# Vegeta2020/SE-SSD

Measured on NVIDIA H100. Metric: frames_per_sec, higher is better.
Workload: dtype f32

## Files before the change

### include/sessd_b200.h

```cpp
#ifndef SESSD_B200_H
#define SESSD_B200_H

#include <stddef.h>
#include <stdint.h>

#ifdef __cplusplus
extern "C" {
#endif

#define SESSD_OK 0
#define SESSD_EINVAL (-1)
#define SESSD_ECAPACITY (-2)
#define SESSD_EWORKSPACE (-3)

const char *sessd_version(void);
long long sessd_launch_count(void);

typedef struct {
    float voxel_size[3];
    float range_min[3];
    float range_max[3];
    int grid[3];
    int max_points;
    int max_voxels;
    int num_feat;
} sessd_voxel_cfg;

size_t sessd_voxelize_workspace_bytes(int max_total_points, int batch, const sessd_voxel_cfg *cfg);

int sessd_voxelize(const float *d_points, const int *d_frame_off, int batch, int max_total_points,
                   const sessd_voxel_cfg *cfg, float *d_voxels, int *d_coors, int *d_num_points, float *d_mean,
                   int *d_num_voxels, void *workspace, size_t workspace_bytes, void *stream);

int sessd_voxelize_host(const float *h_points, int num_points, const sessd_voxel_cfg *cfg, float *h_voxels,
                        int *h_coors_zyx , int *h_num_points);

typedef struct {
    int batch;
    int shape[3];
} sessd_grid;

size_t sessd_hash_bytes(int max_rows, int *capacity_out);
int sessd_hash_build(const int *d_coors , const int *d_n, int max_rows, sessd_grid grid,
                     uint64_t *d_table, int capacity, void *stream);

size_t sessd_bitmap_words(sessd_grid grid);
size_t sessd_scan_scratch_bytes(size_t n_items);

int sessd_subm_rulebook(const int *d_coors, const int *d_n, int max_rows, sessd_grid grid, const int ksize[3],
                        int index_kind , const void *d_index, int hash_capacity,
                        int *d_nbr, void *stream);

int sessd_strided_rulebook(const int *d_in_coors, const int *d_n_in, int max_in, sessd_grid in_grid,
                           int in_index_kind, const void *d_in_index, int in_hash_capacity,
                           const int ksize[3], const int stride[3], const int padding[3],
                           sessd_grid out_grid, void *d_out_bitmap , void *d_scan_scratch,
                           int *d_out_coors, int *d_n_out, int max_out, int *d_nbr, int *d_status, void *stream);

int sessd_tile_list_stride(int kvol);
int sessd_rulebook_tile_lists(const int *d_nbr, int kvol, const int *d_n_out, int max_out, void *d_tiles, void *stream);

int sessd_spconv_forward(const float *d_in_feat, int cin, const int *d_nbr, int kvol, const int *d_n_out,
                         int max_out, const float *d_weight, int cout, const float *d_scale, const float *d_shift,
                         int relu, float *d_out_feat, void *stream);

int sessd_sparse_to_dense(const float *d_feat, const int *d_coors, const int *d_n, int max_rows, int channels,
                          sessd_grid grid, float *d_out, void *stream);
int sessd_sparse_to_dense_indexed(const float *d_feat, int max_rows, const void *d_bitmap_index, int channels, sessd_grid grid,
                                  float *d_out, void *stream);

int sessd_spconv_forward_rows(const float *d_in_feat, int cin, const int *d_nbr, int kvol, const int *d_n_out, int max_out,
                              const float *d_weight, int cout, const float *d_scale, const float *d_shift, int relu,
                              float *d_out_feat, float *d_amax_out, void *stream);
int sessd_spconv_forward_rows_planes(const float *d_in_feat, int cin, const int *d_nbr, int kvol, const int *d_n_out, int max_out,
                                     const float *d_weight, int cout, const float *d_scale, const float *d_shift, int relu,
                                     const float *d_amax_in, float gain, float shift_max, float *d_out_feat, void *d_out_planes, int cpo,
                                     float *d_out_info, void *stream);
int sessd_spconv_forward_cg(const void *d_in_planes, int cp, int plane_rows, const float *d_in_info, const void *d_tiles, int kvol,
                            const int *d_n_out, int max_out, const void *d_weight_h2, int cout, const float *d_scale, const float *d_shift,
                            int relu, float gain, float shift_max, float *d_out_f32, void *d_out_planes, float *d_out_info, void *stream);
void sessd_set_sp_cg_deep(int on);
int sessd_spconv_cg_blocks_per_sm(int cp, int cout, int deep);
int sessd_absmax_rows(const float *d_feat, const int *d_n, int max_rows, int channels, float *d_amax, void *stream);

int sessd_rulebook_transpose(const int *d_nbr, int kvol, const int *d_n_out, int max_out, int max_in, int *d_nbr_t, void *stream);
int sessd_sparse_split_planes(const float *d_x, const int *d_n, int max_rows, int channels, float *d_info, void *d_planes, int cp, void *stream);
int sessd_dense_grad_gather(const float *d_grad, const int *d_coors, const int *d_n, int max_rows, int channels, sessd_grid grid,
                            float *d_out, void *stream);
int sessd_spconv_wgrad_items(int max_out, int kvol);
size_t sessd_spconv_wgrad_workspace_bytes(int max_out, int kvol, int cin, int cout);
int sessd_spconv_wgrad_rows(const float *d_in_feat, int cin, const float *d_gout, int cout, const void *d_tiles, int kvol,
                            const int *d_n_out, int max_out, float *d_gw, void *d_ws, size_t ws_bytes, void *stream);
int sessd_spconv_wgrad_cg(const void *d_in_planes, int cp, const float *d_in_info, const void *d_g_planes, int cout, const float *d_g_info,
                          const void *d_tiles, int kvol, const int *d_n_out, int max_out, float *d_gw, void *d_ws, size_t ws_bytes,
                          void *stream);

typedef struct {
    int batch, in_h, in_w, cin;
    int out_h, out_w, cout;
    int grid_h, grid_w;
    int in_stride;
    int out_stride, out_off_y, out_off_x;
    int ntaps;
    int tap_dy[16], tap_dx[16];
    int relu;
} sessd_conv_desc;

int sessd_bev_conv_p2(const void *d_in_planes, const float *d_in_info, const void *d_weight_h2, int cout_pad, const float *d_scale,
                      const float *d_shift, const float *d_residual, const float *d_resid_info, float gain, float shift_max,
                      float *d_out_f32, void *d_out_planes, float *d_out_info, const sessd_conv_desc *desc, const int *d_items,
                      void *stream);
int sessd_bev_deconv_p2(const void *d_in_planes, const float *d_in_info, const void *d_weight_h2, int cout_pad, const float *d_scale,
                        const float *d_shift, const float *d_residual, const float *d_resid_info, float gain, float shift_max,
                        float *d_out_f32, void *d_out_planes, float *d_out_info, int batch, int in_h, int in_w, int cin, int cout,
                        int relu, const int *d_items, void *stream);
long long sessd_bev_skip_plan_words(int batch, int h, int w, int *offsets);
int sessd_bev_skip_plan(const void *d_bitmap_index, sessd_grid grid, int *d_plan, void *stream);
int sessd_bev_skip_fill(const int *d_record, float *d_out_f32, void *d_out_planes, int cout, void *stream);
int sessd_bev_wgrad_items(const sessd_conv_desc *desc);
size_t sessd_bev_wgrad_workspace_bytes(const sessd_conv_desc *desc);
int sessd_bev_wgrad(const void *d_in_planes, const float *d_in_info, const void *d_g_planes, const float *d_g_info,
                    const sessd_conv_desc *desc, float *d_gw, void *d_ws, size_t ws_bytes, void *stream);
int sessd_bev_split_planes(const float *d_x, long long n, float *d_info, void *d_planes, void *stream);
int sessd_sparse_to_dense_planes(const float *d_feat, int max_rows, const void *d_bitmap_index, int channels, sessd_grid grid,
                                 const float *d_amax, float *d_info, void *d_planes, void *stream);
int sessd_ssfa_fuse_planes(const float *d_x0, const float *d_x1, const float *d_w0, const float *d_w1, float s0, float t0, float s1,
                           float t1, int num_pixels, int channels, float *d_out, const float *d_info0, const float *d_info1,
                           float *d_out_info, void *d_planes, void *stream);

int sessd_absmax(const float *d_x, long long n, float *d_amax, void *stream);


typedef struct {
    float cnt_thresh;
    float dist_edge[4];
    float sigma2[3];
    float suppressed_thresh;
    float centerness_pow;
    int centerness;
} sessd_dinms_cfg;

#define SESSD_DINMS_MAX_PRE 4096

typedef struct {
    int batch;
    int num_anchors;
    int anchors_per_loc;
    int head_stride;
    float score_thresh;
    int nms_pre_max;
    int nms_post_max;
    float nms_iou_thresh;
    int nms_ge;
    float post_range[6];
    float direction_offset;
    int use_frustum;
    int nms_mode;
    sessd_dinms_cfg dinms;
} sessd_post_cfg;

size_t sessd_postprocess_workspace_bytes(const sessd_post_cfg *cfg);

int sessd_postprocess(const float *d_head, const float *d_anchors, const float *d_frustum,
                      const sessd_post_cfg *cfg, float *d_boxes, float *d_scores, int *d_labels, int *d_count,
                      int *d_aux, int *d_sel_anchor, void *workspace, size_t workspace_bytes, void *stream);

int sessd_postprocess_packed(const float *d_head, const float *d_anchors, const float *d_frustum,
                             const sessd_post_cfg *cfg, float *d_boxes, float *d_scores, int *d_labels, int *d_count,
                             int *d_aux, int *d_sel_anchor, float *d_packed, int *d_meta, const int *d_num_voxels,
                             const int *d_status, void *workspace, size_t workspace_bytes, void *stream);

size_t sessd_rotate_nms_workspace_bytes(int max_boxes, int pre_max);
int sessd_rotate_nms(const float *d_boxes5, const float *d_scores, const int *d_n, int max_boxes, int pre_max,
                     int post_max, float iou_thresh, int ge, int *d_keep, int *d_num_keep, void *workspace,
                     size_t workspace_bytes, void *stream);

size_t sessd_rotate_weighted_nms_workspace_bytes(int max_boxes, int pre_max);
int sessd_rotate_weighted_nms(const float *d_boxes7, const float *d_boxes5, const float *d_scores, const float *d_iou_preds,
                              const int *d_labels, const int *d_dirs, const float *d_anchors, const int *d_n, int max_boxes,
                              int pre_max, const sessd_dinms_cfg *cfg, float *d_out_boxes, float *d_out_scores, int *d_out_labels,
                              int *d_out_dirs, int *d_keep, int *d_selected, int *d_count, void *workspace, size_t workspace_bytes,
                              void *stream);

int sessd_boxes_overlap_bev(const float *d_a, int n, const float *d_b, int m, float *d_out, void *stream);
int sessd_boxes_aligned_overlap_bev(const float *d_a, const float *d_b, int n, float *d_out, void *stream);
int sessd_boxes_iou_bev(const float *d_a, int n, const float *d_b, int m, float *d_out, void *stream);
int sessd_boxes_iou3d(const float *d_a, int n, const float *d_b, int m, float *d_out, void *stream);
size_t sessd_nms_workspace_bytes(int n);
int sessd_nms_sorted(const float *d_boxes, int n, float thresh, int mode, long long *d_keep, int *d_num_keep,
                     void *workspace, size_t workspace_bytes, void *stream);

size_t sessd_assign_workspace_bytes(int num_anchors, int batch, int max_gt);
int sessd_assign_targets(const float *d_anchors, int num_anchors, const float *d_gt_boxes, const int *d_num_gt, int batch,
                         int max_gt, float matched_thr, float unmatched_thr, int *d_labels, float *d_bbox_targets,
                         float *d_bbox_outside_weights, int *d_pos_anchor, int *d_pos_gt_id, int *d_num_pos,
                         void *workspace, size_t workspace_bytes, void *stream);

#define SESSD_AUGMENT_MAX_GT 256
#define SESSD_AUGMENT_MAX_TRY 128
int sessd_box_collision(const double *d_boxes, int n, const double *d_qboxes, int k, uint8_t *d_out, void *stream);
int sessd_noise_per_box(const float *d_gt_boxes, const int *d_num_gt, const uint8_t *d_valid, int batch, int max_gt,
                        const double *d_loc_noise, const double *d_rot_noise, int num_try, double context, int *d_selected,
                        void *stream);
int sessd_points_in_boxes(const float *d_points, int n, int point_stride, const float *d_boxes, int m, double context, uint8_t *d_mask,
                          void *stream);
int sessd_augment_points(const float *d_points, const int *d_frame_off, int batch, int max_frame_points, const float *d_gt_boxes,
                         const int *d_num_gt, const uint8_t *d_valid, int max_gt, const double *d_loc_noise, const double *d_rot_noise,
                         int num_try, const int *d_selected, double context, const float *d_global, const int *d_perm,
                         const uint8_t *d_labeled, float *d_points_raw, float *d_points_out, void *stream);
int sessd_augment_boxes(const float *d_gt_boxes, const int *d_num_gt, const uint8_t *d_valid, const uint8_t *d_target, int batch,
                        int max_gt, const double *d_loc_noise, const double *d_rot_noise, int num_try, const int *d_selected,
                        const float *d_global, const float *range_bev, float *d_boxes_raw, int *d_num_raw, float *d_boxes_out,
                        int *d_num_out, float *d_boxes_global, int *d_num_global, void *stream);

int sessd_gtaug_select_host(const double *h_corners, int num_boxes, int num_cand, uint8_t *h_accepted);
size_t sessd_gtaug_paste_workspace_bytes(int batch, int num_points, int num_objects);
int sessd_gtaug_paste(const float *d_points, const int *d_frame_off, int batch, int num_points, const int *d_obj_off, const int *d_obj_ids,
                      int num_objects, int max_paste_points, const float *d_db_points, const int *d_db_off, const int *d_db_count,
                      const double *d_db_boxes, int db_size, void *d_workspace, size_t workspace_bytes, float *d_points_out, int capacity,
                      int *d_frame_off_out, void *stream);

#define SESSD_SADA_MAX_IDS (6 * SESSD_AUGMENT_MAX_GT)
int sessd_sada_pyramids(const float *d_boxes, int num_boxes, float *d_pyramids, float *d_planes, void *stream);
int sessd_sada_membership(const float *d_points, int n, const int *d_n, const float *d_planes, int num_pyramids, const int *d_ids, int num_ids,
                          uint32_t *d_bits, int *d_counts, void *stream);
size_t sessd_sada_compact_workspace_bytes(int n);
int sessd_sada_compact(const float *d_points, int n, const int *d_n, const uint32_t *d_bits, int num_ids, const int *d_counts, int min_count,
                       void *d_workspace, size_t workspace_bytes, float *d_out, int capacity, int *d_num_out, void *stream);
size_t sessd_sada_fps_workspace_bytes(int n, int num_ids);
int sessd_sada_fps(const float *d_points, int n, const int *d_n, const uint32_t *d_bits, int num_ids, const int *d_counts, int min_count, int k,
                   void *d_workspace, size_t workspace_bytes, float *d_out, int capacity, int *d_num, void *stream);
int sessd_sada_swap(const float *d_points, int n, const int *d_n, const uint32_t *d_bits, int num_pairs, const int *d_counts, const float *d_pyramids,
                    int num_pyramids, const int *d_ids, int max_swap_points, float *d_out, int capacity, const int *d_num_in,
                    int *d_num_out, void *stream);
int sessd_sada_shuffle(const float *d_points, const int *d_frame_off, int batch, int max_frame_points, const int *d_perm, float *d_out,
                       void *stream);

size_t sessd_prep_frustum_compact_workspace_bytes(int num_points);
int sessd_prep_frustum_compact(const float *d_points, const int *d_frame_off, int batch, int num_points, const double *d_planes,
                               void *d_workspace, size_t workspace_bytes, float *d_points_out, int capacity, int *d_frame_off_out, void *stream);
int sessd_prep_box_count(const float *d_points, const int *d_frame_off, int batch, int num_points, const double *d_box_planes,
                         const int *d_box_off, int num_boxes, int *d_counts, void *stream);
size_t sessd_prep_box_gather_workspace_bytes(int num_boxes);
int sessd_prep_box_gather(const float *d_points, const int *d_frame_off, int batch, int num_points, const double *d_box_planes,
                          const double *d_centres, const int *d_box_off, int num_boxes, const int *d_counts, int num_rows, void *d_workspace,
                          size_t workspace_bytes, float *d_rows_out, int capacity, int *d_obj_off, void *stream);

size_t sessd_head_loss_workspace_bytes(int batch);
size_t sessd_odiou_loss_workspace_bytes(int batch);
int sessd_odiou_loss(const float *d_head, const float *d_anchors, const int *d_labels, const float *d_reg_targets, int batch,
                     int num_anchors, int anchors_per_loc, int head_stride, float w_odiou, const float *d_losses, float *d_odiou_sum,
                     float *d_grad_head, void *workspace, size_t workspace_bytes, void *stream);
int sessd_odiou_pairs_host(const float *h_gboxes, const float *h_qboxes, int n, float *h_odiou, float *h_grad_q);
size_t sessd_iou_pred_loss_workspace_bytes(int batch);
int sessd_iou_pred_loss(const float *d_head, const float *d_anchors, const int *d_labels, const float *d_reg_targets, int batch,
                        int num_anchors, int anchors_per_loc, int head_stride, float sigma, float w_iou, float *d_losses,
                        float *d_grad_head, void *workspace, size_t workspace_bytes, void *stream);
int sessd_head_loss(const float *d_head, const float *d_anchors, const int *d_labels, const float *d_reg_targets, int batch,
                    int num_anchors, int anchors_per_loc, int head_stride, float alpha, float sigma, float dir_offset,
                    float pos_cls_weight, float neg_cls_weight, float w_cls, float w_loc, float w_dir, float *d_losses,
                    float *d_grad_head, void *workspace, size_t workspace_bytes, void *stream);

int sessd_axpby(float *d_y, const float *d_x, float a, float b, long long n, void *stream);
int sessd_adamw_step(float *d_param, const float *d_grad, float *d_exp_avg, float *d_exp_avg_sq, long long n, float lr, float beta1,
                     float beta2, float eps, float weight_decay, int step, void *stream);
size_t sessd_grad_sqnorm_workspace_bytes(long long n);
int sessd_grad_sqnorm(const float *d_x, long long n, float max_norm, float *d_out, void *d_workspace, void *stream);
int sessd_adamw_clip_ema_step(float *d_param, float *d_grad, float *d_exp_avg, float *d_exp_avg_sq, long long n, float lr, float beta1,
                              float beta2, float eps, float weight_decay, int step, const float *d_clip_coef, float *d_ema, double ema_alpha,
                              void *stream);

#define SESSD_KITTI_REC 13
#define SESSD_KITTI_PERSON_SITTING 11
#define SESSD_KITTI_VAN 12
typedef struct {
    int num_frames;
    const int *gt_off;
    const double *gt;
    const int *gt_code;
    const int *gt_occluded;
    const int *dc_off;
    const double *dc;
    const int *dt_off;
    const int *dt_cnt;
    const double *dt;
    const int *dt_code;
    const long long *ov_off;
} SessdKittiFrames;
size_t sessd_kitti_convert_workspace_bytes(long long capacity);
int sessd_kitti_convert_detections(const float *d_boxes7, const float *d_scores, const int *d_labels, const int *d_off, int num_frames,
                                   long long capacity, const double *d_calib, const int *d_image_hw, const int *d_label_code,
                                   int num_labels, double *d_rec, int *d_label, int *d_code, int *d_cnt, void *workspace,
                                   size_t workspace_bytes, void *stream);
int sessd_kitti_overlaps(const SessdKittiFrames *frames, int metric, int z_axis, double z_center, double *d_overlaps, void *stream);
size_t sessd_kitti_eval_workspace_bytes(int num_frames, long long total_gt, long long overlap_elems, int num_configs, int compute_aos);
int sessd_kitti_eval(const SessdKittiFrames *frames, int max_frame_dt, int metric, int z_axis, double z_center, int num_configs,
                     const int *d_cfg, const double *d_min_overlap, int compute_aos, long long total_gt, long long overlap_elems,
                     double *d_thresholds, int *d_num_thresholds, double *d_precision, double *d_aos, double *d_map, void *workspace,
                     size_t workspace_bytes, void *stream);

#ifdef __cplusplus
}
#endif
#endif
```

### se-ssd_b200/csrc/bevconv.cu

```cuda
#include <cuda_fp16.h>

#include "common.cuh"

namespace sessd {

__global__ void __launch_bounds__(256) ssfa_fuse_kernel(const float *__restrict__ x0, const float *__restrict__ x1,
                                                        const float *__restrict__ w0, const float *__restrict__ w1, float s0, float t0,
                                                        float s1, float t1, int num_pixels, int C, float *__restrict__ out,
                                                        const float *__restrict__ info0, const float *__restrict__ info1,
                                                        float *__restrict__ out_info, __half *__restrict__ planes, long long plane_stride) {
    const int lane = threadIdx.x & 31;
    const int warps_per_block = blockDim.x >> 5;
    const float am = fmaxf(__ldg(info0), __ldg(info1));
    const float sp = pow2_scale_for_bound(am);
    if (blockIdx.x == 0 && threadIdx.x == 0) { out_info[0] = am; out_info[1] = sp; }
    for (int p = blockIdx.x * warps_per_block + (threadIdx.x >> 5); p < num_pixels; p += gridDim.x * warps_per_block) {
        float d0 = 0.f, d1 = 0.f;
        for (int c = lane * 4; c < C; c += 128) {
            const float4 a = *reinterpret_cast<const float4 *>(x0 + (size_t)p * C + c);
            const float4 b = *reinterpret_cast<const float4 *>(x1 + (size_t)p * C + c);
            const float4 u = *reinterpret_cast<const float4 *>(w0 + c);
            const float4 v = *reinterpret_cast<const float4 *>(w1 + c);
            d0 += a.x * u.x + a.y * u.y + a.z * u.z + a.w * u.w;
            d1 += b.x * v.x + b.y * v.y + b.z * v.z + b.w * v.w;
        }
#pragma unroll
        for (int o = 16; o > 0; o >>= 1) { d0 += __shfl_xor_sync(0xffffffffu, d0, o); d1 += __shfl_xor_sync(0xffffffffu, d1, o); }
        const float l0 = fmaf(d0, s0, t0), l1 = fmaf(d1, s1, t1);
        const float mx = fmaxf(l0, l1);
        const float e0 = expf(l0 - mx), e1 = expf(l1 - mx);
        const float inv = 1.0f / (e0 + e1);
        const float a0 = e0 * inv, a1 = e1 * inv;
        for (int c = lane * 4; c < C; c += 128) {
            const float4 a = *reinterpret_cast<const float4 *>(x0 + (size_t)p * C + c);
            const float4 b = *reinterpret_cast<const float4 *>(x1 + (size_t)p * C + c);
            float4 r;
            r.x = a.x * a0 + b.x * a1; r.y = a.y * a0 + b.y * a1; r.z = a.z * a0 + b.z * a1; r.w = a.w * a0 + b.w * a1;
            if (out) *reinterpret_cast<float4 *>(out + (size_t)p * C + c) = r;
            const float q[4] = {r.x * sp, r.y * sp, r.z * sp, r.w * sp};
            __align__(8) __half hi[4], lo[4];
#pragma unroll
            for (int e = 0; e < 4; ++e) {
                hi[e] = __float2half_rn(q[e]);
                lo[e] = __float2half_rn(q[e] - __half2float(hi[e]));
            }
            *reinterpret_cast<uint2 *>(planes + (size_t)p * C + c) = *reinterpret_cast<const uint2 *>(hi);
            *reinterpret_cast<uint2 *>(planes + plane_stride + (size_t)p * C + c) = *reinterpret_cast<const uint2 *>(lo);
        }
    }
}

__global__ void absmax_kernel(const float4 *__restrict__ x, long long n4, const float *__restrict__ tail, int ntail, float *__restrict__ amax) {
    float m = 0.f;
    for (long long i = blockIdx.x * (long long)blockDim.x + threadIdx.x; i < n4; i += (long long)gridDim.x * blockDim.x) {
        const float4 v = __ldg(x + i);
        m = fmaxf(m, fmaxf(fmaxf(fabsf(v.x), fabsf(v.y)), fmaxf(fabsf(v.z), fabsf(v.w))));
    }
    if (blockIdx.x == 0 && (int)threadIdx.x < ntail) m = fmaxf(m, fabsf(tail[threadIdx.x]));
    const unsigned w = __reduce_max_sync(0xFFFFFFFFu, __float_as_uint(m));
    __shared__ unsigned s_m[32];
    if ((threadIdx.x & 31) == 0) s_m[threadIdx.x >> 5] = w;
    __syncthreads();
    if (threadIdx.x < 32) {
        const unsigned v = threadIdx.x < (blockDim.x >> 5) ? s_m[threadIdx.x] : 0u;
        const unsigned r = __reduce_max_sync(0xFFFFFFFFu, v);
        if (threadIdx.x == 0 && r != 0u) atomicMax(reinterpret_cast<unsigned *>(amax), r);
    }
}

}

using namespace sessd;

extern "C" int sessd_absmax(const float *d_x, long long n, float *d_amax, void *stream) {
    if (!d_x || !d_amax || n < 0 || ((uintptr_t)d_x & 15)) return SESSD_EINVAL;
    if (n == 0) return 0;
    const long long n4 = n / 4;
    const int blocks = (int)max(1LL, min((long long)kNumSMs * 8, (n4 + 255) / 256));
    absmax_kernel<<<blocks, 256, 0, (cudaStream_t)stream>>>(reinterpret_cast<const float4 *>(d_x), n4, d_x + n4 * 4, (int)(n - n4 * 4), d_amax);
    ++g_launches;
    return last_error();
}

extern "C" int sessd_ssfa_fuse_planes(const float *d_x0, const float *d_x1, const float *d_w0, const float *d_w1, float s0, float t0, float s1,
                                      float t1, int num_pixels, int channels, float *d_out, const float *d_info0, const float *d_info1,
                                      float *d_out_info, void *d_planes, void *stream) {
    if (!d_x0 || !d_x1 || !d_w0 || !d_w1 || !d_planes || !d_info0 || !d_info1 || !d_out_info || num_pixels < 1 || channels < 4 || channels % 4)
        return SESSD_EINVAL;
    SESSD_LAUNCH(ssfa_fuse_kernel, persistent_grid((long long)num_pixels * 32, 256), 256, 0, stream, d_x0, d_x1, d_w0, d_w1, s0, t0, s1, t1,
                 num_pixels, channels, d_out, d_info0, d_info1, d_out_info, (__half *)d_planes, (long long)num_pixels * channels);
    return last_error();
}
```

### se-ssd_b200/csrc/bevconv_p2.cu

```cuda
#include "bevconv_p2.cuh"

namespace sessd {

__global__ void __launch_bounds__(256) bev_split_planes_kernel(const float4 *__restrict__ x, long long n4, float *__restrict__ info,
                                                               __half *__restrict__ planes, long long plane_stride) {
    const float s = pow2_scale_for_bound(__ldg(info));
    if (blockIdx.x == 0 && threadIdx.x == 0) info[1] = s;
    for (long long i = blockIdx.x * (long long)blockDim.x + threadIdx.x; i < n4; i += (long long)gridDim.x * blockDim.x) {
        const float4 v = __ldg(x + i);
        const float a[4] = {v.x * s, v.y * s, v.z * s, v.w * s};
        __align__(8) __half hi[4], lo[4];
#pragma unroll
        for (int t = 0; t < 4; ++t) {
            hi[t] = __float2half_rn(a[t]);
            lo[t] = __float2half_rn(a[t] - __half2float(hi[t]));
        }
        *reinterpret_cast<uint2 *>(planes + 4 * i) = *reinterpret_cast<const uint2 *>(hi);
        *reinterpret_cast<uint2 *>(planes + plane_stride + 4 * i) = *reinterpret_cast<const uint2 *>(lo);
    }
}

}

using namespace sessd;

extern "C" int sessd_bev_conv_p2(const void *d_in_planes, const float *d_in_info, const void *d_weight_h2, int cout_pad, const float *d_scale,
                                 const float *d_shift, const float *d_residual, const float *d_resid_info, float gain, float shift_max,
                                 float *d_out_f32, void *d_out_planes, float *d_out_info, const sessd_conv_desc *desc, const int *d_items,
                                 void *stream) {
    return p2_conv<kP2Planes>(d_in_planes, d_in_info, d_weight_h2, cout_pad, d_scale, d_shift, d_residual, d_resid_info, gain, shift_max,
                              d_out_f32, d_out_planes, d_out_info, desc, stream, d_items);
}

extern "C" int sessd_bev_deconv_p2(const void *d_in_planes, const float *d_in_info, const void *d_weight_h2, int cout_pad, const float *d_scale,
                                   const float *d_shift, const float *d_residual, const float *d_resid_info, float gain, float shift_max,
                                   float *d_out_f32, void *d_out_planes, float *d_out_info, int batch, int in_h, int in_w, int cin, int cout,
                                   int relu, const int *d_items, void *stream) {
    return p2_deconv<kP2Planes>(d_in_planes, d_in_info, d_weight_h2, cout_pad, d_scale, d_shift, d_residual, d_resid_info, gain, shift_max,
                                d_out_f32, d_out_planes, d_out_info, batch, in_h, in_w, cin, cout, relu, stream, d_items);
}

extern "C" int sessd_bev_split_planes(const float *d_x, long long n, float *d_info, void *d_planes, void *stream) {
    if (!d_x || !d_info || !d_planes || n < 4 || (n & 3) || ((uintptr_t)d_x & 15)) return SESSD_EINVAL;
    SESSD_LAUNCH(bev_split_planes_kernel, persistent_grid(n / 4, 256), 256, 0, stream, reinterpret_cast<const float4 *>(d_x), n / 4, d_info,
                 (__half *)d_planes, n);
    return last_error();
}
```

### se-ssd_b200/csrc/bevconv_p2.cuh

```cuda
#pragma once
#include <cuda_fp16.h>

#include "tc_common.cuh"

namespace sessd {

constexpr int kP2TileU = 8, kP2TileV = 16;
constexpr int kP2MaxCopies = 6, kP2MaxRowsV = 18;
constexpr int kP2BStages = 6, kP2MaxBStages = 12;
constexpr int kP2MmaWarps = 8;
constexpr int kP2PatchWarp = 8, kP2WeightWarp = 9;
constexpr int kP2Threads = 320;
constexpr int kP2ThreadsRegA = 384, kP2RegsConsumer = 232, kP2RegsProducer = 40;
static_assert(2 * (kP2RegsConsumer - 168) <= 168 - kP2RegsProducer, "the consumers take what the producers release");
constexpr int kP2MaxSmem = 227 * 1024;
constexpr int kP2Chunk = 32;
constexpr int kP2ItemsHeader = 32;
enum { kP2Planes = 0, kP2SplitF16 = 1 };
enum { kP2NoProbe = 0, kP2ProbeClocks = 1, kP2ProbeLoads = 2 };

struct P2Params {
    int batch, cin, cout;
    int in_stride;
    int out_h, out_w;
    int grid_u, grid_v;
    int u_is_x;
    int out_stride, nclass;
    int cls_ntaps[4], cls_off_u[4], cls_off_v[4];
    int tap_copy[4][9], tap_row[4][9], tap_w[4][9];
    int ncopies, rows_v, pitch_u;
    int copy_u[kP2MaxCopies], copy_v[kP2MaxCopies];
    int copy_bytes, patch_bytes, npatch;
    int load_bytes, staging_bytes;
    int bring_bytes;
    int out_info_scale;
    const float *in_amax;
    int relu, n_tile, nblocks;
    int bstages, bstage_bytes;
    int tiles_u, tiles_v, tiles, total;
    int cls_order[4];
    const float *in_info;
    const float *resid_info;
    float gain, shift_max;
    float *out_info;
    long long out_plane_stride;
    const int *items;
    long long *prof;
};

enum P2Prof {
    kProfCta,
    kProfItems,
    kProfSteps,
    kProfItemClk,
    kProfBFull,
    kProfPatchFull,
    kProfMmaWait,
    kProfEpilogue,
    kProfPatchEmpty,
    kProfPatchTotal,
    kProfBEmpty,
    kProfBTotal,
    kP2ProfWords = 16
};

__device__ __forceinline__ int p2_item_count(const P2Params &p) { return p.items ? __ldg(p.items) : p.total; }
__device__ __forceinline__ int p2_item(const P2Params &p, int k) { return p.items ? __ldg(p.items + kP2ItemsHeader + k) : k; }

struct P2ItemIndex { int rank, nb, t; };
__host__ __device__ __forceinline__ P2ItemIndex p2_item_index(int g, int nblocks, int tiles) {
    const int rank = g / (nblocks * tiles), rem = g - rank * (nblocks * tiles), nb = rem / tiles;
    return {rank, nb, rem - nb * tiles};
}

struct P2Item { int cls, n0, b, u0, v0, ntaps; };

__device__ __forceinline__ P2Item p2_decode(const P2Params &p, int g) {
    P2Item it;
    const P2ItemIndex ix = p2_item_index(g, p.nblocks, p.tiles);
    int t = ix.t;
    it.cls = p.cls_order[ix.rank];
    it.n0 = ix.nb * p.n_tile;
    const int tu = t % p.tiles_u; t /= p.tiles_u;
    const int tv = t % p.tiles_v;
    it.b = t / p.tiles_v;
    it.u0 = tu * kP2TileU; it.v0 = tv * kP2TileV;
    it.ntaps = p.cls_ntaps[it.cls];
    return it;
}

template <int N>
__device__ __forceinline__ void p2_wgmma(float *d, uint64_t da, uint64_t db, uint32_t accumulate) {
    if constexpr (N == 32) wgmma_f16_n32(d, da, db, accumulate);
    else if constexpr (N == 64) wgmma_f16_n64(d, da, db, accumulate);
    else if constexpr (N == 128) wgmma_f16_n128(d, da, db, accumulate);
    else wgmma_f16_n256(d, da, db, accumulate);
}

template <int N>
__device__ __forceinline__ void p2_wgmma_ra(float *d, const uint32_t *a, uint64_t db, uint32_t accumulate) {
    if constexpr (N == 32) wgmma_f16_ra_n32(d, a, db, accumulate);
    else if constexpr (N == 64) wgmma_f16_ra_n64(d, a, db, accumulate);
    else if constexpr (N == 128) wgmma_f16_ra_n128(d, a, db, accumulate);
    else wgmma_f16_ra_n256(d, a, db, accumulate);
}

template <bool PROFILE>
__device__ __forceinline__ long long p2_tick() {
    if constexpr (PROFILE) return clock64();
    return 0;
}
template <bool PROFILE>
__device__ __forceinline__ void p2_tock(long long &clk, long long t0) {
    if constexpr (PROFILE) clk += clock64() - t0;
}

__device__ __forceinline__ void p2_split_patch(const P2Params &p, const unsigned char *staging, unsigned char *planes, float s_in, int ctid) {
    const int rows = p.rows_v * kP2TileU;
    const int copy_in = p.staging_bytes / p.ncopies;
    const int items = p.ncopies * rows * 4;
    for (int i = ctid; i < items; i += kP2MmaWarps * 32) {
        const int j = i & 3, r = (i >> 2) % rows, c = (i >> 2) / rows;
        unsigned char *hi = planes + 2 * c * p.copy_bytes + r * 64 + ((j ^ ((r >> 1) & 3)) << 4);
        const float4 *src = reinterpret_cast<const float4 *>(staging + c * copy_in + r * 128 + j * 32);
        const float4 a = src[0], b = src[1];
        const float x[8] = {a.x * s_in, a.y * s_in, a.z * s_in, a.w * s_in, b.x * s_in, b.y * s_in, b.z * s_in, b.w * s_in};
        __align__(16) __half h[8], l[8];
#pragma unroll
        for (int t = 0; t < 8; ++t) { h[t] = __float2half_rn(x[t]); l[t] = __float2half_rn(x[t] - __half2float(h[t])); }
        *reinterpret_cast<uint4 *>(hi) = *reinterpret_cast<const uint4 *>(h);
        *reinterpret_cast<uint4 *>(hi + p.copy_bytes) = *reinterpret_cast<const uint4 *>(l);
    }
    asm volatile("fence.proxy.async.shared::cta;\n" ::: "memory");
    asm volatile("bar.sync 1, %0;\n" ::"n"(kP2MmaWarps * 32) : "memory");
}

template <int NT, int MODE, bool REGA = false, int PROBE = kP2NoProbe>
__global__ void __launch_bounds__(REGA ? kP2ThreadsRegA : kP2Threads, 1) bev_conv_p2_kernel(const __grid_constant__ CUtensorMap map_a,
                                                                   const __grid_constant__ CUtensorMap map_b,
                                                                   const float *__restrict__ scale, const float *__restrict__ shift,
                                                                   const float *__restrict__ resid, float *__restrict__ out_f32,
                                                                   __half *__restrict__ out_planes, P2Params p) {
    static_assert(!REGA || MODE == kP2Planes, "register-fed A reads the TMA-written planes");
    constexpr bool PROFILE = PROBE != kP2NoProbe, LOADS_ONLY = PROBE == kP2ProbeLoads;
    extern __shared__ unsigned char smem_raw[];
    unsigned char *tiles = (unsigned char *)(((uintptr_t)smem_raw + 1023) & ~(uintptr_t)1023);
    unsigned char *patches = tiles + p.bring_bytes;
    unsigned char *staging = patches + p.npatch * p.patch_bytes;
    uint64_t *bars = (uint64_t *)(staging + p.npatch * p.staging_bytes);
    uint64_t *patch_full = bars, *patch_empty = bars + 2, *b_full = bars + 4, *b_empty = bars + 4 + kP2MaxBStages;
    uint32_t *s_aoff = (uint32_t *)(b_empty + kP2MaxBStages);
    float *s_scale = (float *)(((uintptr_t)(s_aoff + 4 * 9) + 15) & ~(uintptr_t)15), *s_shift = s_scale + p.cout;

    const int warp = threadIdx.x >> 5, lane = threadIdx.x & 31;
    if (threadIdx.x == kP2PatchWarp * 32) prefetch_tensormap(&map_a);
    if (threadIdx.x == kP2WeightWarp * 32) prefetch_tensormap(&map_b);
    const int nchunks = p.cin / kP2Chunk;
    const int nitems = p2_item_count(p);
    const uint32_t b_plane_bytes = (uint32_t)p.n_tile * 64u;

    if (threadIdx.x == 0) {
        for (int s = 0; s < 2; ++s) { mbar_init(&patch_full[s], 1); mbar_init(&patch_empty[s], kP2MmaWarps); }
        for (int s = 0; s < p.bstages; ++s) { mbar_init(&b_full[s], 1); mbar_init(&b_empty[s], kP2MmaWarps); }
        asm volatile("fence.mbarrier_init.release.cluster;\n" ::: "memory");
    }
    for (int idx = threadIdx.x; idx < p.nclass * 9; idx += blockDim.x) {
        const int c = idx / 9, t = idx - c * 9;
        s_aoff[idx] = REGA ? (uint32_t)p.tap_row[c][t] : (uint32_t)((2 * p.tap_copy[c][t] * p.copy_bytes + p.tap_row[c][t] * 512) >> 4);
    }
    for (int n = threadIdx.x; n < p.cout; n += blockDim.x) {
        s_scale[n] = scale ? __ldg(scale + n) : 1.f;
        s_shift[n] = shift ? __ldg(shift + n) : 0.f;
    }
    __syncthreads();
    long long clk[kP2ProfWords] = {};
    const long long t_start = p2_tick<PROFILE>();
    long long *prof_rec = PROFILE ? p.prof + (size_t)blockIdx.x * kP2ProfWords : nullptr;

    if (warp >= kP2MmaWarps) {
        if constexpr (REGA) setmaxnreg_dec<kP2RegsProducer>();
        if (warp == kP2PatchWarp) {
            int pb = 0;
            uint32_t pph = 0;
            const uint32_t patches_u32 = smem_u32(patches);
            for (int k = blockIdx.x; k < nitems; k += gridDim.x) {
                const P2Item it = p2_decode(p, p2_item(p, k));
                const int bu = it.u0 * p.in_stride, bv = it.v0 * p.in_stride;
                for (int cc = 0; cc < nchunks; ++cc) {
                    { const long long t0 = p2_tick<PROFILE>(); mbar_wait<REGA>(&patch_empty[pb], pph ^ 1u); p2_tock<PROFILE>(clk[kProfPatchEmpty], t0); }
                    if (elect_one()) {
                        mbar_expect_tx(&patch_full[pb], (uint32_t)p.load_bytes);
                        if constexpr (MODE == kP2Planes) {
                            uint32_t dst = patches_u32 + (uint32_t)(pb * p.patch_bytes);
                            for (int c = 0; c < p.ncopies; ++c, dst += 2u * (uint32_t)p.copy_bytes) {
                                const int cu = bu + p.copy_u[c], cv = bv + p.copy_v[c];
                                tma_load_5d(dst, &map_a, &patch_full[pb], cc * kP2Chunk, cu, cv, it.b, 0);
                                tma_load_5d(dst + (uint32_t)p.copy_bytes, &map_a, &patch_full[pb], cc * kP2Chunk, cu, cv, it.b, 1);
                            }
                        } else {
                            const uint32_t copy_in = (uint32_t)(p.staging_bytes / p.ncopies);
                            uint32_t dst = smem_u32(staging) + (uint32_t)(pb * p.staging_bytes);
                            for (int c = 0; c < p.ncopies; ++c, dst += copy_in)
                                tma_load_5d(dst, &map_a, &patch_full[pb], cc * kP2Chunk, bu + p.copy_u[c], bv + p.copy_v[c], it.b, 0);
                        }
                    }
                    __syncwarp();
                    if (++pb == p.npatch) { pb = 0; pph ^= 1u; }
                }
            }
            if constexpr (PROFILE)
                if (lane == 0) {
                    prof_rec[kProfPatchEmpty] = clk[kProfPatchEmpty];
                    prof_rec[kProfPatchTotal] = clock64() - t_start;
                }
        } else if (warp == kP2WeightWarp) {
            int S = 0;
            uint32_t bph = 0;
            for (int k = blockIdx.x; k < nitems; k += gridDim.x) {
                const P2Item it = p2_decode(p, p2_item(p, k));
                for (int cc = 0; cc < nchunks; ++cc)
                    for (int tap = 0; tap < it.ntaps; ++tap) {
                        { const long long t0 = p2_tick<PROFILE>(); mbar_wait<REGA>(&b_empty[S], bph ^ 1u); p2_tock<PROFILE>(clk[kProfBEmpty], t0); }
                        if (elect_one()) {
                            unsigned char *st = tiles + S * p.bstage_bytes;
                            const int wtap = p.tap_w[it.cls][tap];
                            mbar_expect_tx(&b_full[S], 2 * b_plane_bytes);
                            tma_load_4d(st + b_plane_bytes, &map_b, &b_full[S], cc * kP2Chunk, it.n0, wtap, 0);
                            tma_load_4d(st, &map_b, &b_full[S], cc * kP2Chunk, it.n0, wtap, 1);
                        }
                        __syncwarp();
                        if (++S == p.bstages) { S = 0; bph ^= 1u; }
                    }
            }
            if constexpr (PROFILE)
                if (lane == 0) {
                    prof_rec[kProfBEmpty] = clk[kProfBEmpty];
                    prof_rec[kProfBTotal] = clock64() - t_start;
                }
        }
    } else {
        if constexpr (REGA) setmaxnreg_inc<kP2RegsConsumer>();
        const int wg = warp >> 2, wq = warp & 3;
        constexpr int kAcc = NT / 2;
        const uint32_t a_rows = (uint32_t)(wg * 64 * 64) >> 4;
        const uint32_t tiles_lo = desc_lo(smem_u32(tiles));
        const uint32_t patch_lo = desc_lo(smem_u32(patches)) + a_rows;
        const uint32_t plane_lo = b_plane_bytes >> 4;
        const uint32_t copy_lo = (uint32_t)(p.copy_bytes >> 4), patch_sz = (uint32_t)(p.patch_bytes >> 4);
        const uint32_t a_row = (uint32_t)((wg * 8 + wq * 2 + ((lane >> 3) & 1)) * p.pitch_u + (lane & 7)), a_chunk = (uint32_t)(lane >> 4);
        const uint32_t patches_u32 = smem_u32(patches);
        float amax_in = 0.f, s_in = 1.f;
        if constexpr (MODE == kP2Planes) { amax_in = __ldg(p.in_info); s_in = __ldg(p.in_info + 1); }
        if constexpr (MODE == kP2SplitF16) if (p.in_amax) { amax_in = __ldg(p.in_amax); s_in = pow2_scale_for_bound(amax_in); }
        const float inv_sa = 1.f / s_in;
        float bound = amax_in * p.gain + p.shift_max;
        if (p.resid_info) bound += __ldg(p.resid_info);
        const float s_out = pow2_scale_for_bound(bound);
        if (blockIdx.x == 0 && threadIdx.x == 0 && p.out_info && p.out_info_scale) p.out_info[1] = s_out;
        float vmax = 0.f;
        const int per_cls = p.nblocks * p.tiles;
        int S = 0, pb = 0;
        uint32_t bph = 0, pph = 0;
        for (int k = blockIdx.x; k < nitems; k += gridDim.x) {
            const long long t_item = p2_tick<PROFILE>();
            const int g = p2_item(p, k);
            const int cls = p.cls_order[g / per_cls];
            const int ntaps = p.cls_ntaps[cls];
            const uint32_t *aoff = s_aoff + cls * 9;
            float acc[NT];
#pragma unroll
            for (int i = 0; i < NT; ++i) acc[i] = 0.f;
            int prevS = -1, prev_pb = -1;
            bool first = true;
            if constexpr (REGA) {
                uint32_t frag[2][16];
                int tap = 0;
                uint32_t pbase = 0;
                auto load_frags = [&](uint32_t *fa) {
                    if (tap == 0) {
                        { const long long t0 = p2_tick<PROFILE>(); mbar_wait<REGA>(&patch_full[pb], pph); p2_tock<PROFILE>(clk[kProfPatchFull], t0); }
                        pbase = patches_u32 + (uint32_t)(pb * p.patch_bytes);
                    }
                    if constexpr (!LOADS_ONLY) {
                        const uint32_t r = a_row + aoff[tap];
                        const uint32_t a_hi = pbase + r * 64u + ((a_chunk ^ ((r >> 1) & 3u)) << 4), a_lo = a_hi + (uint32_t)p.copy_bytes;
                        ldsm_x4(fa, a_hi);
                        ldsm_x4(fa + 4, a_hi ^ 32u);
                        ldsm_x4(fa + 8, a_lo);
                        ldsm_x4(fa + 12, a_lo ^ 32u);
                    }
                };
                auto step_ra = [&](const uint32_t *fa, uint32_t *fn, bool more) {
                    { const long long t0 = p2_tick<PROFILE>(); mbar_wait<REGA>(&b_full[S], bph); p2_tock<PROFILE>(clk[kProfBFull], t0); }
                    const uint64_t db_lo = kDescSw64Hi | (uint64_t)(tiles_lo + (uint32_t)(S * (p.bstage_bytes >> 4)));
                    const uint64_t db_hi = db_lo + (uint64_t)plane_lo;
                    if constexpr (!LOADS_ONLY) {
                        wgmma_fence();
                        p2_wgmma_ra<2 * NT>(acc, fa, db_lo, first ? 0u : 1u);
                        p2_wgmma_ra<2 * NT>(acc, fa + 4, db_lo + 2, 1u);
                        wgmma_commit();
                    }
                    first = false;
                    if constexpr (PROFILE) ++clk[kProfSteps];
                    { const long long t0 = p2_tick<PROFILE>(); wgmma_wait<1>(); p2_tock<PROFILE>(clk[kProfMmaWait], t0); }
                    if (lane == 0 && prevS >= 0) mbar_arrive(&b_empty[prevS]);
                    prevS = S;
                    if (++S == p.bstages) { S = 0; bph ^= 1u; }
                    if (++tap == ntaps) {
                        tap = 0;
                        if (lane == 0) mbar_arrive(&patch_empty[pb]);
                        if (++pb == p.npatch) { pb = 0; pph ^= 1u; }
                    }
                    if (more) load_frags(fn);
                    if constexpr (!LOADS_ONLY) {
                        wgmma_fence();
                        p2_wgmma_ra<NT>(acc, fa + 8, db_hi, 1u);
                        p2_wgmma_ra<NT>(acc, fa + 12, db_hi + 2, 1u);
                        wgmma_commit();
                    }
                };
                const int nsteps = nchunks * ntaps;
                load_frags(frag[0]);
#pragma unroll 1
                for (int st = 0; st + 1 < nsteps; st += 2) { step_ra(frag[0], frag[1], true); step_ra(frag[1], frag[0], st + 2 < nsteps); }
                if (nsteps & 1) step_ra(frag[0], frag[1], false);
            } else {
                for (int cc = 0; cc < nchunks; ++cc) {
                    { const long long t0 = p2_tick<PROFILE>(); mbar_wait(&patch_full[pb], pph); p2_tock<PROFILE>(clk[kProfPatchFull], t0); }
                    if constexpr (MODE == kP2SplitF16)
                        p2_split_patch(p, staging + pb * p.staging_bytes, patches + pb * p.patch_bytes, s_in, threadIdx.x);
                    const uint32_t pbase = patch_lo + (uint32_t)pb * patch_sz;
#pragma unroll 1
                    for (int tap = 0; tap < ntaps; ++tap) {
                        { const long long t0 = p2_tick<PROFILE>(); mbar_wait(&b_full[S], bph); p2_tock<PROFILE>(clk[kProfBFull], t0); }
                        if constexpr (!LOADS_ONLY) {
                            const uint64_t da_hi = kDescSw64Hi | (uint64_t)(pbase + aoff[tap]);
                            const uint64_t da_lo = da_hi + (uint64_t)copy_lo;
                            const uint64_t db_lo = kDescSw64Hi | (uint64_t)(tiles_lo + (uint32_t)(S * (p.bstage_bytes >> 4)));
                            const uint64_t db_hi = db_lo + (uint64_t)plane_lo;
                            const uint32_t accum = first ? 0u : 1u;
                            wgmma_fence();
                            if constexpr (MODE == kP2Planes) {
                                p2_wgmma<2 * NT>(acc, da_hi, db_lo, accum);
                                p2_wgmma<2 * NT>(acc, da_hi + 2, db_lo + 2, 1u);
                            } else {
                                p2_wgmma<NT>(acc + kAcc, da_hi, db_hi, accum);
                                p2_wgmma<NT>(acc + kAcc, da_hi + 2, db_hi + 2, 1u);
                                p2_wgmma<NT>(acc, da_hi, db_lo, accum);
                                p2_wgmma<NT>(acc, da_hi + 2, db_lo + 2, 1u);
                            }
                            p2_wgmma<NT>(acc, da_lo, db_hi, 1u);
                            p2_wgmma<NT>(acc, da_lo + 2, db_hi + 2, 1u);
                            wgmma_commit();
                        }
                        first = false;
                        if constexpr (PROFILE) ++clk[kProfSteps];
                        { const long long t0 = p2_tick<PROFILE>(); wgmma_wait<1>(); p2_tock<PROFILE>(clk[kProfMmaWait], t0); }
                        if (lane == 0) {
                            if (prevS >= 0) mbar_arrive(&b_empty[prevS]);
                            if (prev_pb >= 0) mbar_arrive(&patch_empty[prev_pb]);
                        }
                        prevS = S;
                        prev_pb = (tap == ntaps - 1) ? pb : -1;
                        if (++S == p.bstages) { S = 0; bph ^= 1u; }
                    }
                    if (p.npatch == 1) {
                        { const long long t0 = p2_tick<PROFILE>(); wgmma_wait<0>(); p2_tock<PROFILE>(clk[kProfMmaWait], t0); }
                        if (lane == 0) {
                            mbar_arrive(&b_empty[prevS]);
                            mbar_arrive(&patch_empty[pb]);
                        }
                        prevS = prev_pb = -1;
                    }
                    if (++pb == p.npatch) { pb = 0; pph ^= 1u; }
                }
            }
            { const long long t0 = p2_tick<PROFILE>(); wgmma_wait<0>(); p2_tock<PROFILE>(clk[kProfMmaWait], t0); }
            const long long t_epi = p2_tick<PROFILE>();
            wgmma_fence_regs<NT>(acc);
            if (lane == 0) {
                if (prevS >= 0) mbar_arrive(&b_empty[prevS]);
                if (prev_pb >= 0) mbar_arrive(&patch_empty[prev_pb]);
            }
#pragma unroll
            for (int i = 0; i < kAcc; ++i) acc[i] = acc[kAcc + i] + acc[i];
            const P2Item it = p2_decode(p, g);
            const int q = lane & 3;
            const int r0 = wg * 64 + wq * 16 + (lane >> 2);
            bool rows_ok[2];
            size_t opixs[2];
#pragma unroll
            for (int h = 0; h < 2; ++h) {
                const int r = r0 + 8 * h;
                const int lv = r / kP2TileU, lu = r % kP2TileU;
                const int gu = it.u0 + lu, gv = it.v0 + lv;
                rows_ok[h] = it.b < p.batch && gu < p.grid_u && gv < p.grid_v;
                const int ou = gu * p.out_stride + p.cls_off_u[it.cls], ov = gv * p.out_stride + p.cls_off_v[it.cls];
                const int oy = p.u_is_x ? ov : ou, ox = p.u_is_x ? ou : ov;
                opixs[h] = ((size_t)it.b * p.out_h + (size_t)oy) * p.out_w + (size_t)ox;
            }
#pragma unroll
            for (int j = 0; j < (LOADS_ONLY ? 0 : NT / 32); ++j)
#pragma unroll
                for (int h = 0; h < 2; ++h) {
                    const bool row_ok = rows_ok[h];
                    const size_t opix = opixs[h];
                    float v[8], o[8] = {};
                    quad_transpose8(acc + 16 * j + 2 * h, q, v);
                    const int n = it.n0 + 32 * j + 8 * q;
                    const size_t off = opix * p.cout + n;
                    if (row_ok && n < p.cout) {
                        float sc[8], sh[8];
#pragma unroll
                        for (int t = 0; t < 8; t += 4) {
                            const float4 a = *reinterpret_cast<const float4 *>(s_scale + n + t);
                            const float4 b = *reinterpret_cast<const float4 *>(s_shift + n + t);
                            sc[t] = a.x; sc[t + 1] = a.y; sc[t + 2] = a.z; sc[t + 3] = a.w;
                            sh[t] = b.x; sh[t + 1] = b.y; sh[t + 2] = b.z; sh[t + 3] = b.w;
                        }
#pragma unroll
                        for (int t = 0; t < 8; ++t) {
                            o[t] = fmaf(v[t] * inv_sa, sc[t], sh[t]);
                            if (p.relu) o[t] = fmaxf(o[t], 0.f);
                        }
                        if (resid) {
#pragma unroll
                            for (int t = 0; t < 8; t += 4) {
                                const float4 rr = __ldg(reinterpret_cast<const float4 *>(resid + off + t));
                                o[t] += rr.x; o[t + 1] += rr.y; o[t + 2] += rr.z; o[t + 3] += rr.w;
                            }
                        }
#pragma unroll
                        for (int t = 0; t < 8; ++t) vmax = fmaxf(vmax, fabsf(o[t]));
                        if (out_planes) {
                            __align__(16) __half2 hi[4], lo[4];
#pragma unroll
                            for (int t = 0; t < 4; ++t) {
                                const float x0 = o[2 * t] * s_out, x1 = o[2 * t + 1] * s_out;
                                hi[t] = __floats2half2_rn(x0, x1);
                                const float2 f = __half22float2(hi[t]);
                                lo[t] = __floats2half2_rn(x0 - f.x, x1 - f.y);
                            }
                            *reinterpret_cast<uint4 *>(out_planes + off) = *reinterpret_cast<const uint4 *>(hi);
                            *reinterpret_cast<uint4 *>(out_planes + p.out_plane_stride + off) = *reinterpret_cast<const uint4 *>(lo);
                        }
                    }
                    if (out_f32) {
                        const bool up = q & 2;
                        float keep[4], recv[4];
#pragma unroll
                        for (int t = 0; t < 4; ++t) {
                            keep[t] = up ? o[4 + t] : o[t];
                            recv[t] = __shfl_xor_sync(0xFFFFFFFFu, up ? o[t] : o[4 + t], 2);
                        }
                        const int n_lo = it.n0 + 32 * j + 8 * (q & 1), c_lo = n_lo + 4 * (q >> 1);
                        const float4 w_lo = up ? make_float4(recv[0], recv[1], recv[2], recv[3]) : make_float4(keep[0], keep[1], keep[2], keep[3]);
                        const float4 w_hi = up ? make_float4(keep[0], keep[1], keep[2], keep[3]) : make_float4(recv[0], recv[1], recv[2], recv[3]);
                        if (row_ok && n_lo < p.cout) *reinterpret_cast<float4 *>(out_f32 + opix * p.cout + c_lo) = w_lo;
                        if (row_ok && n_lo + 16 < p.cout) *reinterpret_cast<float4 *>(out_f32 + opix * p.cout + c_lo + 16) = w_hi;
                    }
                }
            if constexpr (PROFILE) {
                const long long t_end = clock64();
                clk[kProfEpilogue] += t_end - t_epi;
                clk[kProfItemClk] += t_end - t_item;
                ++clk[kProfItems];
            }
        }
        if constexpr (PROFILE)
            if (threadIdx.x == 0) {
                clk[kProfCta] = clock64() - t_start;
                for (int w = kProfCta; w <= kProfEpilogue; ++w) prof_rec[w] = clk[w];
            }
        if (p.out_info) {
            const unsigned m = __reduce_max_sync(0xFFFFFFFFu, __float_as_uint(vmax));
            if (lane == 0 && m != 0u) atomicMax(reinterpret_cast<unsigned *>(p.out_info), m);
        }
    }
}

static int encode_map_nd(CUtensorMap *m, const void *base, int rank, const cuuint64_t *dims, const cuuint64_t *strides_bytes ,
                         const cuuint32_t *box, const cuuint32_t *estr, CUtensorMapSwizzle swz,
                         CUtensorMapDataType dtype = CU_TENSOR_MAP_DATA_TYPE_FLOAT16) {
    EncodeTiledFn enc = get_tensor_map_encoder();
    if (!enc) return SESSD_EINVAL;
    CUresult r = enc(m, dtype, (cuuint32_t)rank, const_cast<void *>(base), dims, strides_bytes, box, estr,
                     CU_TENSOR_MAP_INTERLEAVE_NONE, swz, CU_TENSOR_MAP_L2_PROMOTION_L2_256B, CU_TENSOR_MAP_FLOAT_OOB_FILL_NONE);
    return r == CUDA_SUCCESS ? 0 : 700 + (int)r;
}

struct P2Taps { int n, dy[9], dx[9], w[9], off_y, off_x; };

static void p2_deconv_classes(P2Taps cls[4]) {
    for (int c = 0; c < 4; ++c) {
        P2Taps &k = cls[c];
        k = {};
        k.off_y = c >> 1; k.off_x = c & 1;
        for (int dy = k.off_y; dy >= 0; --dy)
            for (int dx = k.off_x; dx >= 0; --dx, ++k.n) {
                k.dy[k.n] = dy; k.dx[k.n] = dx; k.w[k.n] = (k.off_y + 1 - 2 * dy) * 3 + (k.off_x + 1 - 2 * dx);
            }
    }
}

constexpr int p2_n_tile(int cout) { return cout <= 32 ? 32 : 128; }

struct P2Geometry {
    int u_is_x, grid_u, grid_v, tiles_u, tiles_v, tiles;
    int n_tile, nblocks, nclass, total;
    int ntaps[4], off_u[4], off_v[4], order[4];
};

static int p2_geometry(P2Geometry &g, int batch, int grid_h, int grid_w, int cout, int cout_pad, const P2Taps *cls, int nclass) {
    g = {};
    if (batch < 1 || grid_h < 1 || grid_w < 1 || cout < 8 || cout % 8) return SESSD_EINVAL;
    g.n_tile = p2_n_tile(cout);
    if (cout_pad % g.n_tile || cout_pad < cout) return SESSD_EINVAL;
    g.u_is_x = div_up(grid_w, kP2TileU) * div_up(grid_h, kP2TileV) <= div_up(grid_h, kP2TileU) * div_up(grid_w, kP2TileV);
    g.grid_u = g.u_is_x ? grid_w : grid_h; g.grid_v = g.u_is_x ? grid_h : grid_w;
    g.tiles_u = div_up(g.grid_u, kP2TileU); g.tiles_v = div_up(g.grid_v, kP2TileV);
    g.tiles = g.tiles_u * g.tiles_v * batch;
    g.nblocks = cout_pad / g.n_tile;
    g.nclass = nclass; g.total = nclass * g.nblocks * g.tiles;
    for (int c = 0; c < nclass; ++c) {
        g.ntaps[c] = cls[c].n;
        g.off_u[c] = g.u_is_x ? cls[c].off_x : cls[c].off_y;
        g.off_v[c] = g.u_is_x ? cls[c].off_y : cls[c].off_x;
        g.order[c] = c;
    }
    for (int i = 1; i < nclass; ++i)
        for (int k = i; k > 0 && g.ntaps[g.order[k]] > g.ntaps[g.order[k - 1]]; --k) {
            const int tmp = g.order[k]; g.order[k] = g.order[k - 1]; g.order[k - 1] = tmp;
        }
    return 0;
}

static int p2_plan(P2Params &p, const P2Taps *cls, int nclass, int grid_h, int grid_w, int cout_pad, int mode, bool reg_a, int *smem) {
    if (reg_a && (mode != kP2Planes || p.in_stride != 1)) return SESSD_EINVAL;
    if (p.cin < 64 || p.cin % 64) return SESSD_EINVAL;
    P2Geometry g;
    if (p2_geometry(g, p.batch, grid_h, grid_w, p.cout, cout_pad, cls, nclass)) return SESSD_EINVAL;
    p.u_is_x = g.u_is_x; p.grid_u = g.grid_u; p.grid_v = g.grid_v;
    p.tiles_u = g.tiles_u; p.tiles_v = g.tiles_v; p.tiles = g.tiles;
    p.n_tile = g.n_tile; p.nblocks = g.nblocks; p.nclass = g.nclass; p.total = g.total;
    for (int c = 0; c < 4; ++c) {
        p.cls_ntaps[c] = g.ntaps[c]; p.cls_off_u[c] = g.off_u[c]; p.cls_off_v[c] = g.off_v[c]; p.cls_order[c] = g.order[c];
    }
    const int s = p.in_stride;
    p.ncopies = 0;
    int key_u[kP2MaxCopies], key_vm[kP2MaxCopies], vmin[kP2MaxCopies], vmax[kP2MaxCopies];
    for (int c = 0; c < p.nclass; ++c)
        for (int t = 0; t < cls[c].n; ++t) {
            const int tu = p.u_is_x ? cls[c].dx[t] : cls[c].dy[t], tv = p.u_is_x ? cls[c].dy[t] : cls[c].dx[t];
            const int vm = ((tv % s) + s) % s;
            int k = 0;
            for (; k < p.ncopies; ++k)
                if (key_u[k] == tu && key_vm[k] == vm) break;
            if (k == p.ncopies) {
                if (p.ncopies == kP2MaxCopies) return SESSD_EINVAL;
                key_u[k] = tu; key_vm[k] = vm; vmin[k] = tv; vmax[k] = tv;
                ++p.ncopies;
            }
            vmin[k] = min(vmin[k], tv); vmax[k] = max(vmax[k], tv);
        }
    p.rows_v = 0;
    p.pitch_u = kP2TileU;
    for (int k = 0; k < p.ncopies; ++k) p.rows_v = max(p.rows_v, kP2TileV + (vmax[k] - vmin[k]) / s);
    if (p.rows_v > kP2MaxRowsV) return SESSD_EINVAL;
    for (int k = 0; k < p.ncopies; ++k) { p.copy_u[k] = key_u[k]; p.copy_v[k] = vmin[k]; }
    if (reg_a) {
        int umin = key_u[0], umax = key_u[0];
        for (int k = 1; k < p.ncopies; ++k) {
            umin = min(umin, key_u[k]); umax = max(umax, key_u[k]);
            vmin[0] = min(vmin[0], vmin[k]); vmax[0] = max(vmax[0], vmax[k]);
        }
        p.ncopies = 1;
        p.copy_u[0] = umin; p.copy_v[0] = vmin[0];
        p.pitch_u = kP2TileU + umax - umin; p.rows_v = kP2TileV + vmax[0] - vmin[0];
        if (p.pitch_u > 256 || p.rows_v > 256) return SESSD_EINVAL;
    }
    for (int c = 0; c < p.nclass; ++c) {
        for (int t = 0; t < cls[c].n; ++t) {
            const int tu = p.u_is_x ? cls[c].dx[t] : cls[c].dy[t], tv = p.u_is_x ? cls[c].dy[t] : cls[c].dx[t];
            const int vm = ((tv % s) + s) % s;
            int k = 0;
            for (; k < p.ncopies; ++k)
                if (key_u[k] == tu && key_vm[k] == vm) break;
            p.tap_copy[c][t] = reg_a ? 0 : k;
            p.tap_row[c][t] = reg_a ? (tv - p.copy_v[0]) * p.pitch_u + (tu - p.copy_u[0]) : (tv - vmin[k]) / s;
            p.tap_w[c][t] = cls[c].w[t];
        }
    }
    p.copy_bytes = (p.rows_v * p.pitch_u * 64 + 511) & ~511;
    p.patch_bytes = p.ncopies * 2 * p.copy_bytes;
    p.staging_bytes = mode == kP2Planes ? 0 : p.ncopies * p.rows_v * kP2TileU * kP2Chunk * 4;
    p.load_bytes = mode == kP2Planes ? p.ncopies * 2 * p.rows_v * p.pitch_u * 64 : p.staging_bytes;
    const int per_buf = p.patch_bytes + p.staging_bytes, bstage = 2 * p.n_tile * 64;
    const int tail = 1536 + 16 + 2 * 4 * p.cout;
    p.npatch = (kP2BStages * bstage + tail + 2 * per_buf <= kP2MaxSmem) ? 2 : 1;
    p.bstage_bytes = bstage;
    p.bstages = min((kP2MaxSmem - tail - p.npatch * per_buf) / bstage, kP2MaxBStages);
    if (p.bstages < 2) return SESSD_EINVAL;
    p.bring_bytes = p.bstages * bstage;
    *smem = p.bring_bytes + tail + p.npatch * per_buf;
    return 0;
}

template <int MODE, int PROBE = kP2NoProbe>
static int launch_p2(const void *d_in_planes, int in_h, int in_w, const float *d_in_info, const void *d_w, int w_taps, int cout_pad,
                     const float *d_scale, const float *d_shift, const float *d_residual, const float *d_resid_info, float gain,
                     float shift_max, float *d_out_f32, void *d_out_planes, float *d_out_info, P2Params &p, const P2Taps *cls, int nclass,
                     int grid_h, int grid_w, bool reg_a, void *stream) {
    if (!d_in_planes || !d_w || (!d_out_f32 && !d_out_planes)) return SESSD_EINVAL;
    if (MODE == kP2Planes && (!d_in_info || !d_scale)) return SESSD_EINVAL;
    if (MODE != kP2Planes && d_out_planes) return SESSD_EINVAL;
    if (((uintptr_t)d_scale | (uintptr_t)d_shift | (uintptr_t)d_residual | (uintptr_t)d_out_f32 | (uintptr_t)d_out_planes) & 15)
        return SESSD_EINVAL;
    int smem = 0;
    if (p2_plan(p, cls, nclass, grid_h, grid_w, cout_pad, MODE, reg_a, &smem)) return SESSD_EINVAL;
    if (p.items && cout_pad != div_up(p.cout, p.n_tile) * p.n_tile) return SESSD_EINVAL;
    const int s = p.in_stride;
    CUtensorMap map_a, map_b;
    if (MODE != kP2Planes) {
        const cuuint64_t row_w = (cuuint64_t)p.cin * 4, row_h = (cuuint64_t)in_w * p.cin * 4;
        const cuuint64_t dims[5] = {(cuuint64_t)p.cin, (cuuint64_t)(p.u_is_x ? in_w : in_h), (cuuint64_t)(p.u_is_x ? in_h : in_w),
                                    (cuuint64_t)p.batch, 1};
        const cuuint64_t strides[4] = {p.u_is_x ? row_w : row_h, p.u_is_x ? row_h : row_w, (cuuint64_t)in_h * in_w * p.cin * 4,
                                       (cuuint64_t)p.batch * in_h * in_w * p.cin * 4};
        const cuuint32_t box[5] = {(cuuint32_t)kP2Chunk, (cuuint32_t)(kP2TileU * s), (cuuint32_t)(p.rows_v * s), 1, 1};
        const cuuint32_t estr[5] = {1, (cuuint32_t)s, (cuuint32_t)s, 1, 1};
        int rc = encode_map_nd(&map_a, d_in_planes, 5, dims, strides, box, estr, CU_TENSOR_MAP_SWIZZLE_NONE, CU_TENSOR_MAP_DATA_TYPE_FLOAT32);
        if (rc) return rc;
    } else {
        const cuuint64_t row_w = (cuuint64_t)p.cin * 2, row_h = (cuuint64_t)in_w * p.cin * 2;
        const cuuint64_t dims[5] = {(cuuint64_t)p.cin, (cuuint64_t)(p.u_is_x ? in_w : in_h), (cuuint64_t)(p.u_is_x ? in_h : in_w),
                                    (cuuint64_t)p.batch, 2};
        const cuuint64_t strides[4] = {p.u_is_x ? row_w : row_h, p.u_is_x ? row_h : row_w, (cuuint64_t)in_h * in_w * p.cin * 2,
                                       (cuuint64_t)p.batch * in_h * in_w * p.cin * 2};
        const cuuint32_t box[5] = {(cuuint32_t)kP2Chunk, (cuuint32_t)(p.pitch_u * s), (cuuint32_t)(p.rows_v * s), 1, 1};
        const cuuint32_t estr[5] = {1, (cuuint32_t)s, (cuuint32_t)s, 1, 1};
        int rc = encode_map_nd(&map_a, d_in_planes, 5, dims, strides, box, estr, CU_TENSOR_MAP_SWIZZLE_64B);
        if (rc) return rc;
    }
    {
        const cuuint64_t dims[4] = {(cuuint64_t)p.cin, (cuuint64_t)cout_pad, (cuuint64_t)w_taps, 2};
        const cuuint64_t strides[3] = {(cuuint64_t)p.cin * 2, (cuuint64_t)cout_pad * p.cin * 2, (cuuint64_t)w_taps * cout_pad * p.cin * 2};
        const cuuint32_t box[4] = {(cuuint32_t)kP2Chunk, (cuuint32_t)p.n_tile, 1, 1};
        const cuuint32_t estr[4] = {1, 1, 1, 1};
        int rc = encode_map_nd(&map_b, d_w, 4, dims, strides, box, estr, CU_TENSOR_MAP_SWIZZLE_64B);
        if (rc) return rc;
    }
    constexpr bool kRegA = MODE == kP2Planes;
    auto kernel = bev_conv_p2_kernel<128, MODE, false, PROBE>;
    if (p.n_tile == 32) kernel = reg_a ? bev_conv_p2_kernel<32, MODE, kRegA, PROBE> : bev_conv_p2_kernel<32, MODE, false, PROBE>;
    else if (reg_a) kernel = bev_conv_p2_kernel<128, MODE, kRegA, PROBE>;
    static bool attr_done[2][2] = {};
    if (!attr_done[p.n_tile == 32][reg_a]) {
        SESSD_CUDA_TRY(cudaFuncSetAttribute(kernel, cudaFuncAttributeMaxDynamicSharedMemorySize, kP2MaxSmem));
        attr_done[p.n_tile == 32][reg_a] = true;
    }
    p.in_info = MODE == kP2Planes ? d_in_info : nullptr;
    p.in_amax = MODE == kP2SplitF16 ? d_in_info : nullptr;
    p.resid_info = d_residual ? d_resid_info : nullptr;
    if (d_residual && d_out_planes && !d_resid_info) return SESSD_EINVAL;
    p.gain = gain; p.shift_max = shift_max; p.out_info = d_out_info;
    p.out_info_scale = MODE == kP2Planes ? 1 : 0;
    if (d_out_planes && !d_out_info) return SESSD_EINVAL;
    p.out_plane_stride = (long long)p.batch * p.out_h * p.out_w * p.cout;
    static int num_sms = 0;
    if (!num_sms) {
        int dev = 0;
        SESSD_CUDA_TRY(cudaGetDevice(&dev));
        SESSD_CUDA_TRY(cudaDeviceGetAttribute(&num_sms, cudaDevAttrMultiProcessorCount, dev));
    }
    const int grid = p.total < num_sms ? p.total : num_sms;
    SESSD_LAUNCH(kernel, grid, reg_a ? kP2ThreadsRegA : kP2Threads, smem, (cudaStream_t)stream, map_a, map_b, d_scale, d_shift, d_residual, d_out_f32,
                 (__half *)d_out_planes, p);
    return last_error();
}


static int p2_conv_params(const sessd_conv_desc &d, P2Params &p, P2Taps &t) {
    if (d.ntaps < 1 || d.ntaps > 9 || (d.in_stride != 1 && d.in_stride != 2) || d.out_stride < 1) return SESSD_EINVAL;
    if ((d.grid_h - 1) * d.out_stride + d.out_off_y >= d.out_h || (d.grid_w - 1) * d.out_stride + d.out_off_x >= d.out_w) return SESSD_EINVAL;
    p = {};
    p.batch = d.batch; p.cin = d.cin; p.cout = d.cout; p.in_stride = d.in_stride;
    p.out_h = d.out_h; p.out_w = d.out_w; p.out_stride = d.out_stride; p.relu = d.relu;
    t = {};
    t.n = d.ntaps; t.off_y = d.out_off_y; t.off_x = d.out_off_x;
    for (int i = 0; i < d.ntaps; ++i) { t.dy[i] = d.tap_dy[i]; t.dx[i] = d.tap_dx[i]; t.w[i] = i; }
    return 0;
}

static void p2_deconv_params(int batch, int in_h, int in_w, int cin, int cout, int relu, P2Params &p, P2Taps cls[4]) {
    p = {};
    p.batch = batch; p.cin = cin; p.cout = cout; p.in_stride = 1;
    p.out_h = 2 * in_h; p.out_w = 2 * in_w; p.out_stride = 2; p.relu = relu;
    p2_deconv_classes(cls);
}

template <int MODE, int PROBE = kP2NoProbe>
static int p2_conv(const void *d_in_planes, const float *d_in_info, const void *d_weight_h2, int cout_pad, const float *d_scale,
                   const float *d_shift, const float *d_residual, const float *d_resid_info, float gain, float shift_max,
                   float *d_out_f32, void *d_out_planes, float *d_out_info, const sessd_conv_desc *desc, void *stream,
                   const int *d_items = nullptr, long long *d_prof = nullptr, bool smem_a = false) {
    if (!desc || (PROBE != kP2NoProbe && !d_prof)) return SESSD_EINVAL;
    const sessd_conv_desc &d = *desc;
    P2Params p;
    P2Taps t;
    if (p2_conv_params(d, p, t)) return SESSD_EINVAL;
    p.items = d_items;
    p.prof = d_prof;
    return launch_p2<MODE, PROBE>(d_in_planes, d.in_h, d.in_w, d_in_info, d_weight_h2, d.ntaps, cout_pad, d_scale, d_shift, d_residual, d_resid_info, gain,
                     shift_max, d_out_f32, d_out_planes, d_out_info, p, &t, 1, d.grid_h, d.grid_w, MODE == kP2Planes && d.in_stride == 1 && !smem_a,
                     stream);
}

template <int MODE, int PROBE = kP2NoProbe>
static int p2_deconv(const void *d_in_planes, const float *d_in_info, const void *d_weight_h2, int cout_pad, const float *d_scale,
                     const float *d_shift, const float *d_residual, const float *d_resid_info, float gain, float shift_max,
                     float *d_out_f32, void *d_out_planes, float *d_out_info, int batch, int in_h, int in_w, int cin, int cout,
                     int relu, void *stream, const int *d_items = nullptr, long long *d_prof = nullptr) {
    if (PROBE != kP2NoProbe && !d_prof) return SESSD_EINVAL;
    P2Params p;
    P2Taps cls[4];
    p2_deconv_params(batch, in_h, in_w, cin, cout, relu, p, cls);
    p.items = d_items;
    p.prof = d_prof;
    return launch_p2<MODE, PROBE>(d_in_planes, in_h, in_w, d_in_info, d_weight_h2, 9, cout_pad, d_scale, d_shift, d_residual, d_resid_info, gain, shift_max,
                     d_out_f32, d_out_planes, d_out_info, p, cls, 4, in_h, in_w, MODE == kP2Planes, stream);
}

}
```

### se-ssd_b200/csrc/bevconv_split.cu

```cuda
#include "bevconv_p2.cuh"

#include "../../include/sessd_b200_lab.h"

using namespace sessd;

extern "C" int sessd_bev_conv_h2(const float *d_in, const void *d_weight_h2, int cout_pad, const float *d_scale, const float *d_shift,
                                 const float *d_residual, float *d_out, const sessd_conv_desc *desc, const float *d_amax_in,
                                 float *d_amax_out, void *stream) {
    if (!d_in || !d_out || !d_scale) return SESSD_EINVAL;
    return p2_conv<kP2SplitF16>(d_in, d_amax_in, d_weight_h2, cout_pad, d_scale, d_shift, d_residual, nullptr, 0.f, 0.f, d_out, nullptr,
                                d_amax_out, desc, stream);
}

extern "C" int sessd_bev_deconv_h2(const float *d_in, const void *d_weight_h2, int cout_pad, const float *d_scale, const float *d_shift,
                                   const float *d_residual, float *d_out, int batch, int in_h, int in_w, int cin, int cout, int relu,
                                   const float *d_amax_in, float *d_amax_out, void *stream) {
    if (!d_in || !d_out || !d_scale) return SESSD_EINVAL;
    return p2_deconv<kP2SplitF16>(d_in, d_amax_in, d_weight_h2, cout_pad, d_scale, d_shift, d_residual, nullptr, 0.f, 0.f, d_out, nullptr,
                                  d_amax_out, batch, in_h, in_w, cin, cout, relu, stream);
}

extern "C" int sessd_bev_conv_p2_profile(const void *d_in_planes, const float *d_in_info, const void *d_weight_h2, int cout_pad,
                                         const float *d_scale, const float *d_shift, const float *d_residual, const float *d_resid_info,
                                         float gain, float shift_max, float *d_out_f32, void *d_out_planes, float *d_out_info,
                                         const sessd_conv_desc *desc, const int *d_items, long long *d_prof, void *stream) {
    return p2_conv<kP2Planes, kP2ProbeClocks>(d_in_planes, d_in_info, d_weight_h2, cout_pad, d_scale, d_shift, d_residual, d_resid_info, gain,
                                              shift_max, d_out_f32, d_out_planes, d_out_info, desc, stream, d_items, d_prof);
}

extern "C" int sessd_bev_deconv_p2_profile(const void *d_in_planes, const float *d_in_info, const void *d_weight_h2, int cout_pad,
                                           const float *d_scale, const float *d_shift, const float *d_residual, const float *d_resid_info,
                                           float gain, float shift_max, float *d_out_f32, void *d_out_planes, float *d_out_info, int batch,
                                           int in_h, int in_w, int cin, int cout, int relu, const int *d_items, long long *d_prof,
                                           void *stream) {
    return p2_deconv<kP2Planes, kP2ProbeClocks>(d_in_planes, d_in_info, d_weight_h2, cout_pad, d_scale, d_shift, d_residual, d_resid_info, gain,
                                                shift_max, d_out_f32, d_out_planes, d_out_info, batch, in_h, in_w, cin, cout, relu, stream,
                                                d_items, d_prof);
}

extern "C" int sessd_bev_conv_p2_loads(const void *d_in_planes, const float *d_in_info, const void *d_weight_h2, int cout_pad,
                                       const float *d_scale, const float *d_shift, const float *d_residual, const float *d_resid_info,
                                       float gain, float shift_max, float *d_out_f32, void *d_out_planes, float *d_out_info,
                                       const sessd_conv_desc *desc, const int *d_items, int smem_a, long long *d_prof, void *stream) {
    return p2_conv<kP2Planes, kP2ProbeLoads>(d_in_planes, d_in_info, d_weight_h2, cout_pad, d_scale, d_shift, d_residual, d_resid_info, gain,
                                             shift_max, d_out_f32, d_out_planes, d_out_info, desc, stream, d_items, d_prof, smem_a != 0);
}

extern "C" int sessd_bev_p2_plan(const sessd_conv_desc *desc, int deconv, int cout_pad, int split, int smem_a, int *plan) {
    if (!desc || !plan) return SESSD_EINVAL;
    const sessd_conv_desc &d = *desc;
    P2Params p;
    P2Taps cls[4];
    if (deconv) p2_deconv_params(d.batch, d.in_h, d.in_w, d.cin, d.cout, d.relu, p, cls);
    else if (p2_conv_params(d, p, cls[0])) return SESSD_EINVAL;
    const int mode = split ? kP2SplitF16 : kP2Planes;
    const bool reg_a = mode == kP2Planes && (deconv || (d.in_stride == 1 && !smem_a));
    int smem = 0;
    if (p2_plan(p, cls, deconv ? 4 : 1, deconv ? d.in_h : d.grid_h, deconv ? d.in_w : d.grid_w, cout_pad, mode, reg_a, &smem))
        return SESSD_EINVAL;
    const int rec[11] = {p.u_is_x, p.n_tile, p.nblocks, p.tiles, p.total, p.ncopies, p.rows_v, p.pitch_u, p.npatch, p.bstages, smem};
    for (int i = 0; i < 11; ++i) plan[i] = rec[i];
    for (int c = 0; c < 4; ++c) { plan[11 + c] = p.cls_ntaps[c]; plan[15 + c] = p.cls_order[c]; }
    return 0;
}
```

### se-ssd_b200/sessd_b200/_lib.py

```python
import ctypes as C
import os

_HERE = os.path.dirname(os.path.abspath(__file__))
LIB_PATH = os.path.join(os.path.dirname(_HERE), "libsessd_b200.so")
LAB_PATH = os.path.join(os.path.dirname(_HERE), "libsessd_b200_lab.so")


class SessdError(RuntimeError):
    pass


class VoxelCfg(C.Structure):
    _fields_ = [("voxel_size", C.c_float * 3), ("range_min", C.c_float * 3), ("range_max", C.c_float * 3),
                ("grid", C.c_int * 3), ("max_points", C.c_int), ("max_voxels", C.c_int), ("num_feat", C.c_int)]


class Grid(C.Structure):
    _fields_ = [("batch", C.c_int), ("shape", C.c_int * 3)]


class ConvDesc(C.Structure):
    _fields_ = [("batch", C.c_int), ("in_h", C.c_int), ("in_w", C.c_int), ("cin", C.c_int),
                ("out_h", C.c_int), ("out_w", C.c_int), ("cout", C.c_int),
                ("grid_h", C.c_int), ("grid_w", C.c_int), ("in_stride", C.c_int),
                ("out_stride", C.c_int), ("out_off_y", C.c_int), ("out_off_x", C.c_int),
                ("ntaps", C.c_int), ("tap_dy", C.c_int * 16), ("tap_dx", C.c_int * 16), ("relu", C.c_int)]


class DinmsCfg(C.Structure):
    _fields_ = [("cnt_thresh", C.c_float), ("dist_edge", C.c_float * 4), ("sigma2", C.c_float * 3), ("suppressed_thresh", C.c_float),
                ("centerness_pow", C.c_float), ("centerness", C.c_int)]


class PostCfg(C.Structure):
    _fields_ = [("batch", C.c_int), ("num_anchors", C.c_int), ("anchors_per_loc", C.c_int), ("head_stride", C.c_int),
                ("score_thresh", C.c_float), ("nms_pre_max", C.c_int), ("nms_post_max", C.c_int),
                ("nms_iou_thresh", C.c_float), ("nms_ge", C.c_int), ("post_range", C.c_float * 6),
                ("direction_offset", C.c_float), ("use_frustum", C.c_int), ("nms_mode", C.c_int), ("dinms", DinmsCfg)]


class KittiFrames(C.Structure):
    _fields_ = [("num_frames", C.c_int), ("gt_off", C.c_void_p), ("gt", C.c_void_p), ("gt_code", C.c_void_p),
                ("gt_occluded", C.c_void_p), ("dc_off", C.c_void_p), ("dc", C.c_void_p), ("dt_off", C.c_void_p),
                ("dt_cnt", C.c_void_p), ("dt", C.c_void_p), ("dt_code", C.c_void_p), ("ov_off", C.c_void_p)]


_vp, _i, _f, _sz, _ll = C.c_void_p, C.c_int, C.c_float, C.c_size_t, C.c_longlong
_I3 = C.POINTER(C.c_int)

SIGNATURES = {
    "sessd_version": (C.c_char_p, []),
    "sessd_launch_count": (_ll, []),
    "sessd_voxelize_workspace_bytes": (_sz, [_i, _i, C.POINTER(VoxelCfg)]),
    "sessd_voxelize": (_i, [_vp, _vp, _i, _i, C.POINTER(VoxelCfg), _vp, _vp, _vp, _vp, _vp, _vp, _sz, _vp]),
    "sessd_voxelize_host": (_i, [_vp, _i, C.POINTER(VoxelCfg), _vp, _vp, _vp]),
    "sessd_hash_bytes": (_sz, [_i, _I3]),
    "sessd_hash_build": (_i, [_vp, _vp, _i, Grid, _vp, _i, _vp]),
    "sessd_bitmap_words": (_sz, [Grid]),
    "sessd_scan_scratch_bytes": (_sz, [_sz]),
    "sessd_subm_rulebook": (_i, [_vp, _vp, _i, Grid, _I3, _i, _vp, _i, _vp, _vp]),
    "sessd_strided_rulebook": (_i, [_vp, _vp, _i, Grid, _i, _vp, _i, _I3, _I3, _I3, Grid, _vp, _vp, _vp, _vp, _i, _vp, _vp, _vp]),
    "sessd_tile_list_stride": (_i, [_i]),
    "sessd_rulebook_tile_lists": (_i, [_vp, _i, _vp, _i, _vp, _vp]),
    "sessd_spconv_forward": (_i, [_vp, _i, _vp, _i, _vp, _i, _vp, _i, _vp, _vp, _i, _vp, _vp]),
    "sessd_spconv_forward_rows": (_i, [_vp, _i, _vp, _i, _vp, _i, _vp, _i, _vp, _vp, _i, _vp, _vp, _vp]),
    "sessd_spconv_forward_rows_planes": (_i, [_vp, _i, _vp, _i, _vp, _i, _vp, _i, _vp, _vp, _i, _vp, _f, _f, _vp, _vp, _i, _vp, _vp]),
    "sessd_spconv_forward_cg": (_i, [_vp, _i, _i, _vp, _vp, _i, _vp, _i, _vp, _i, _vp, _vp, _i, _f, _f, _vp, _vp, _vp, _vp]),
    "sessd_set_sp_cg_deep": (None, [_i]),
    "sessd_spconv_cg_blocks_per_sm": (_i, [_i, _i, _i]),
    "sessd_absmax_rows": (_i, [_vp, _vp, _i, _i, _vp, _vp]),
    "sessd_rulebook_transpose": (_i, [_vp, _i, _vp, _i, _i, _vp, _vp]),
    "sessd_sparse_split_planes": (_i, [_vp, _vp, _i, _i, _vp, _vp, _i, _vp]),
    "sessd_dense_grad_gather": (_i, [_vp, _vp, _vp, _i, _i, Grid, _vp, _vp]),
    "sessd_spconv_wgrad_items": (_i, [_i, _i]),
    "sessd_spconv_wgrad_workspace_bytes": (_sz, [_i, _i, _i, _i]),
    "sessd_spconv_wgrad_rows": (_i, [_vp, _i, _vp, _i, _vp, _i, _vp, _i, _vp, _vp, _sz, _vp]),
    "sessd_spconv_wgrad_cg": (_i, [_vp, _i, _vp, _vp, _i, _vp, _vp, _i, _vp, _i, _vp, _vp, _sz, _vp]),
    "sessd_sparse_to_dense_indexed": (_i, [_vp, _i, _vp, _i, Grid, _vp, _vp]),
    "sessd_sparse_to_dense": (_i, [_vp, _vp, _vp, _i, _i, Grid, _vp, _vp]),
    "sessd_bev_conv_p2": (_i, [_vp, _vp, _vp, _i, _vp, _vp, _vp, _vp, _f, _f, _vp, _vp, _vp, C.POINTER(ConvDesc), _vp, _vp]),
    "sessd_bev_deconv_p2": (_i, [_vp, _vp, _vp, _i, _vp, _vp, _vp, _vp, _f, _f, _vp, _vp, _vp, _i, _i, _i, _i, _i, _i, _vp, _vp]),
    "sessd_bev_skip_plan_words": (_ll, [_i, _i, _i, _I3]),
    "sessd_bev_skip_plan": (_i, [_vp, Grid, _vp, _vp]),
    "sessd_bev_skip_fill": (_i, [_vp, _vp, _vp, _i, _vp]),
    "sessd_bev_wgrad_items": (_i, [C.POINTER(ConvDesc)]),
    "sessd_bev_wgrad_workspace_bytes": (_sz, [C.POINTER(ConvDesc)]),
    "sessd_bev_wgrad": (_i, [_vp, _vp, _vp, _vp, C.POINTER(ConvDesc), _vp, _vp, _sz, _vp]),
    "sessd_bev_split_planes": (_i, [_vp, _ll, _vp, _vp, _vp]),
    "sessd_sparse_to_dense_planes": (_i, [_vp, _i, _vp, _i, Grid, _vp, _vp, _vp, _vp]),
    "sessd_ssfa_fuse_planes": (_i, [_vp, _vp, _vp, _vp, _f, _f, _f, _f, _i, _i, _vp, _vp, _vp, _vp, _vp, _vp]),
    "sessd_absmax": (_i, [_vp, C.c_longlong, _vp, _vp]),
    "sessd_postprocess_workspace_bytes": (_sz, [C.POINTER(PostCfg)]),
    "sessd_postprocess": (_i, [_vp, _vp, _vp, C.POINTER(PostCfg), _vp, _vp, _vp, _vp, _vp, _vp, _vp, _sz, _vp]),
    "sessd_postprocess_packed": (_i, [_vp, _vp, _vp, C.POINTER(PostCfg), _vp, _vp, _vp, _vp, _vp, _vp, _vp, _vp, _vp, _vp, _vp, _sz, _vp]),
    "sessd_rotate_nms_workspace_bytes": (_sz, [_i, _i]),
    "sessd_rotate_nms": (_i, [_vp, _vp, _vp, _i, _i, _i, _f, _i, _vp, _vp, _vp, _sz, _vp]),
    "sessd_rotate_weighted_nms_workspace_bytes": (_sz, [_i, _i]),
    "sessd_rotate_weighted_nms": (_i, [_vp, _vp, _vp, _vp, _vp, _vp, _vp, _vp, _i, _i, C.POINTER(DinmsCfg), _vp, _vp, _vp, _vp, _vp, _vp, _vp,
                                       _vp, _sz, _vp]),
    "sessd_boxes_overlap_bev": (_i, [_vp, _i, _vp, _i, _vp, _vp]),
    "sessd_boxes_aligned_overlap_bev": (_i, [_vp, _vp, _i, _vp, _vp]),
    "sessd_boxes_iou_bev": (_i, [_vp, _i, _vp, _i, _vp, _vp]),
    "sessd_boxes_iou3d": (_i, [_vp, _i, _vp, _i, _vp, _vp]),
    "sessd_nms_workspace_bytes": (_sz, [_i]),
    "sessd_nms_sorted": (_i, [_vp, _i, _f, _i, _vp, _vp, _vp, _sz, _vp]),
    "sessd_head_loss_workspace_bytes": (_sz, [_i]),
    "sessd_head_loss": (_i, [_vp, _vp, _vp, _vp, _i, _i, _i, _i, _f, _f, _f, _f, _f, _f, _f, _f, _vp, _vp, _vp, _sz, _vp]),
    "sessd_odiou_loss_workspace_bytes": (_sz, [_i]),
    "sessd_odiou_loss": (_i, [_vp, _vp, _vp, _vp, _i, _i, _i, _i, _f, _vp, _vp, _vp, _vp, _sz, _vp]),
    "sessd_odiou_pairs_host": (_i, [_vp, _vp, _i, _vp, _vp]),
    "sessd_iou_pred_loss_workspace_bytes": (_sz, [_i]),
    "sessd_iou_pred_loss": (_i, [_vp, _vp, _vp, _vp, _i, _i, _i, _i, _f, _f, _vp, _vp, _vp, _sz, _vp]),
    "sessd_axpby": (_i, [_vp, _vp, _f, _f, _ll, _vp]),
    "sessd_adamw_step": (_i, [_vp, _vp, _vp, _vp, _ll, _f, _f, _f, _f, _f, _i, _vp]),
    "sessd_grad_sqnorm_workspace_bytes": (_sz, [_ll]),
    "sessd_grad_sqnorm": (_i, [_vp, _ll, _f, _vp, _vp, _vp]),
    "sessd_adamw_clip_ema_step": (_i, [_vp, _vp, _vp, _vp, _ll, _f, _f, _f, _f, _f, _i, _vp, _vp, C.c_double, _vp]),
    "sessd_assign_workspace_bytes": (_sz, [_i, _i, _i]),
    "sessd_assign_targets": (_i, [_vp, _i, _vp, _vp, _i, _i, _f, _f, _vp, _vp, _vp, _vp, _vp, _vp, _vp, _sz, _vp]),
    "sessd_box_collision": (_i, [_vp, _i, _vp, _i, _vp, _vp]),
    "sessd_noise_per_box": (_i, [_vp, _vp, _vp, _i, _i, _vp, _vp, _i, C.c_double, _vp, _vp]),
    "sessd_points_in_boxes": (_i, [_vp, _i, _i, _vp, _i, C.c_double, _vp, _vp]),
    "sessd_augment_points": (_i, [_vp, _vp, _i, _i, _vp, _vp, _vp, _i, _vp, _vp, _i, _vp, C.c_double, _vp, _vp, _vp, _vp, _vp, _vp]),
    "sessd_augment_boxes": (_i, [_vp, _vp, _vp, _vp, _i, _i, _vp, _vp, _i, _vp, _vp, C.POINTER(C.c_float), _vp, _vp, _vp, _vp, _vp, _vp, _vp]),
    "sessd_gtaug_select_host": (_i, [_vp, _i, _i, _vp]),
    "sessd_gtaug_paste_workspace_bytes": (_sz, [_i, _i, _i]),
    "sessd_gtaug_paste": (_i, [_vp, _vp, _i, _i, _vp, _vp, _i, _i, _vp, _vp, _vp, _vp, _i, _vp, _sz, _vp, _i, _vp, _vp]),
    "sessd_sada_pyramids": (_i, [_vp, _i, _vp, _vp, _vp]),
    "sessd_sada_membership": (_i, [_vp, _i, _vp, _vp, _i, _vp, _i, _vp, _vp, _vp]),
    "sessd_sada_compact_workspace_bytes": (_sz, [_i]),
    "sessd_sada_compact": (_i, [_vp, _i, _vp, _vp, _i, _vp, _i, _vp, _sz, _vp, _i, _vp, _vp]),
    "sessd_sada_fps_workspace_bytes": (_sz, [_i, _i]),
    "sessd_sada_fps": (_i, [_vp, _i, _vp, _vp, _i, _vp, _i, _i, _vp, _sz, _vp, _i, _vp, _vp]),
    "sessd_sada_swap": (_i, [_vp, _i, _vp, _vp, _i, _vp, _vp, _i, _vp, _i, _vp, _i, _vp, _vp, _vp]),
    "sessd_sada_shuffle": (_i, [_vp, _vp, _i, _i, _vp, _vp, _vp]),
    "sessd_prep_frustum_compact_workspace_bytes": (_sz, [_i]),
    "sessd_prep_frustum_compact": (_i, [_vp, _vp, _i, _i, _vp, _vp, _sz, _vp, _i, _vp, _vp]),
    "sessd_prep_box_count": (_i, [_vp, _vp, _i, _i, _vp, _vp, _i, _vp, _vp]),
    "sessd_prep_box_gather_workspace_bytes": (_sz, [_i]),
    "sessd_prep_box_gather": (_i, [_vp, _vp, _i, _i, _vp, _vp, _vp, _i, _vp, _i, _vp, _sz, _vp, _i, _vp, _vp]),
    "sessd_kitti_convert_workspace_bytes": (_sz, [_ll]),
    "sessd_kitti_convert_detections": (_i, [_vp, _vp, _vp, _vp, _i, _ll, _vp, _vp, _vp, _i, _vp, _vp, _vp, _vp, _vp, _sz, _vp]),
    "sessd_kitti_overlaps": (_i, [C.POINTER(KittiFrames), _i, _i, C.c_double, _vp, _vp]),
    "sessd_kitti_eval_workspace_bytes": (_sz, [_i, _ll, _ll, _i, _i]),
    "sessd_kitti_eval": (_i, [C.POINTER(KittiFrames), _i, _i, _i, C.c_double, _i, _vp, _vp, _i, _ll, _ll, _vp, _vp, _vp, _vp, _vp, _vp,
                              _sz, _vp]),
}


LAB_SIGNATURES = {
    "sessd_bev_conv_h2": (_i, [_vp, _vp, _i, _vp, _vp, _vp, _vp, C.POINTER(ConvDesc), _vp, _vp, _vp]),
    "sessd_bev_deconv_h2": (_i, [_vp, _vp, _i, _vp, _vp, _vp, _vp, _i, _i, _i, _i, _i, _i, _vp, _vp, _vp]),
    "sessd_bev_conv_p2_profile": (_i, [_vp, _vp, _vp, _i, _vp, _vp, _vp, _vp, _f, _f, _vp, _vp, _vp, C.POINTER(ConvDesc), _vp, _vp, _vp]),
    "sessd_bev_deconv_p2_profile": (_i, [_vp, _vp, _vp, _i, _vp, _vp, _vp, _vp, _f, _f, _vp, _vp, _vp, _i, _i, _i, _i, _i, _i, _vp, _vp,
                                         _vp]),
    "sessd_bev_conv_p2_loads": (_i, [_vp, _vp, _vp, _i, _vp, _vp, _vp, _vp, _f, _f, _vp, _vp, _vp, C.POINTER(ConvDesc), _vp, _i, _vp, _vp]),
    "sessd_bev_p2_plan": (_i, [C.POINTER(ConvDesc), _i, _i, _i, _i, _I3]),
}


def _load(path, signatures, mode=C.DEFAULT_MODE):
    if not os.path.exists(path):
        raise ImportError(
            "sessd_b200: %s is missing -- the CUDA library has not been built (run `python se-ssd_b200/build.py`). "
            "There is no CPU fallback." % path)
    lib = C.CDLL(path, mode=mode)
    for name, (res, args) in signatures.items():
        fn = getattr(lib, name)
        fn.restype = res
        fn.argtypes = args
    return lib


class _Libs:

    def __init__(self):
        self._prod = _load(LIB_PATH, SIGNATURES, C.RTLD_GLOBAL)
        self._lab = None

    def lab(self):
        if self._lab is None:
            self._lab = _load(LAB_PATH, LAB_SIGNATURES)
        return self._lab

    @property
    def lab_loaded(self):
        return self._lab is not None

    def __getattr__(self, name):
        if name in LAB_SIGNATURES:
            return getattr(self.lab(), name)
        return getattr(self._prod, name)


lib = _Libs()


def check(rc, what):
    if rc != 0:
        kind = {-1: "invalid argument", -2: "capacity exceeded", -3: "workspace too small"}.get(rc, "cudaError %d" % rc)
        raise SessdError("%s failed: %s" % (what, kind))


def version():
    return lib.sessd_version().decode()


def launch_count():
    return int(lib.sessd_launch_count())
```

### se-ssd_b200/sessd_b200/engine.py

```python
import numpy as np
import torch

from . import ops, synth
from .runners import SpMiddleRunner, SSFAPlanesRunner


class FrameEngine:
    def __init__(self, batch=1, max_points_per_frame=32768, voxel_size=synth.VOXEL_SIZE, pc_range=synth.PC_RANGE,
                 max_points_per_voxel=5, max_voxels=20000, device="cuda", post_kwargs=None, growth=None, skip_constant=True):
        self.batch, self.device = int(batch), torch.device(device)
        self.max_points = int(max_points_per_frame) * self.batch
        self.vcfg = ops.make_voxel_cfg(voxel_size, pc_range, max_points_per_voxel, max_voxels)
        self.grid_xyz = [int(self.vcfg.grid[j]) for j in range(3)]
        dev = self.device
        self.h_points = torch.zeros((self.max_points, 4), dtype=torch.float32).pin_memory()
        self.h_off = torch.zeros((self.batch + 1,), dtype=torch.int32).pin_memory()
        self.d_points = torch.zeros((self.max_points, 4), dtype=torch.float32, device=dev)
        self.d_off = torch.zeros((self.batch + 1,), dtype=torch.int32, device=dev)
        self.vox = ops.VoxelBuffers(self.vcfg, self.batch, self.max_points, dev, with_mean=True)
        self.middle = SpMiddleRunner(self.batch, self.batch * max_voxels, self.grid_xyz, 4, dev, growth=growth)
        self.neck = SSFAPlanesRunner(self.batch, (self.grid_xyz[1] // 8, self.grid_xyz[0] // 8), dev, skip_constant=skip_constant)
        self.anchors = None
        pk = dict(batch=self.batch, head_stride=SSFAPlanesRunner.HEAD_STRIDE)
        pk.update(post_kwargs or {})
        self.pcfg = ops.make_post_cfg(**pk)
        self.post = ops.PostBuffers(self.pcfg, dev)
        P = ops.post_capacity(self.pcfg)
        self.d_result = torch.zeros((self.batch, P, 8), dtype=torch.float32, device=dev)
        self.h_result = torch.zeros((self.batch, P, 8), dtype=torch.float32).pin_memory()
        self.d_meta = torch.zeros((self.batch, 8 + P), dtype=torch.int32, device=dev)
        self.h_meta = torch.zeros((self.batch, 8 + P), dtype=torch.int32).pin_memory()
        self.frustum = None
        self.graph = None
        self.graph_dev = None
        self.stream = torch.cuda.Stream(device=dev)

    def load_weights(self, middle_layers, ssfa_state, head_state, anchors, head_prefix="tasks.0."):
        self.middle.load_weights(middle_layers)
        self.neck.load_state(ssfa_state, head_state, head_prefix)
        self.anchors = torch.as_tensor(np.asarray(anchors, np.float32).reshape(-1, 7)).to(self.device).contiguous()
        assert self.anchors.shape[0] == self.pcfg.num_anchors
        self.graph = None

    def _device_pipeline(self):
        ops.voxelize(self.d_points, self.d_off, self.vox)
        head = self.sparse_and_neck()
        ops.postprocess_packed(head, self.anchors, self.frustum, self.post, self.d_result, self.d_meta,
                               self.vox.num_voxels[:self.batch], self.middle.status)

    def sparse_and_neck(self, mark=None):
        n0 = self.vox.num_voxels[self.batch:self.batch + 1]
        self.neck.info.zero_()
        self.middle.forward(self.vox.mean, self.vox.coors, n0, mark=mark, dense_planes=(self.neck.planes["x"], self.neck.info[0]))
        last = self.middle.levels[-1]
        _, head = self.neck.forward(None, mark=mark, occupancy=(last["index"], last["grid"]))
        return head

    def _step_body(self):
        self.d_points.copy_(self.h_points, non_blocking=True)
        self.d_off.copy_(self.h_off, non_blocking=True)
        self._device_pipeline()
        self.h_result.copy_(self.d_result, non_blocking=True)
        self.h_meta.copy_(self.d_meta, non_blocking=True)

    def capture(self):
        with torch.cuda.stream(self.stream):
            self._step_body()
            self.stream.synchronize()
            g = torch.cuda.CUDAGraph()
            with torch.cuda.graph(g, stream=self.stream):
                self._step_body()
        self.graph = g
        return g

    def capture_device_only(self):
        with torch.cuda.stream(self.stream):
            self._device_pipeline()
            self.stream.synchronize()
            g = torch.cuda.CUDAGraph()
            with torch.cuda.graph(g, stream=self.stream):
                self._device_pipeline()
        self.graph_dev = g
        return g

    def stage(self, clouds):
        assert len(clouds) == self.batch
        off = 0
        hp = self.h_points.numpy()
        ho = self.h_off.numpy()
        for f, c in enumerate(clouds):
            n = c.shape[0]
            if off + n > self.max_points:
                raise ValueError("point capacity exceeded")
            hp[off:off + n] = c
            ho[f] = off
            off += n
        ho[self.batch] = off
        return off

    def launch(self):
        if self.graph is not None:
            with torch.cuda.stream(self.stream):
                self.graph.replay()
        else:
            with torch.cuda.stream(self.stream):
                self._step_body()

    def results(self):
        self.stream.synchronize()
        meta = self.h_meta.numpy()
        if int(meta[:, 5].max()) != 0:
            raise RuntimeError("sparse active-site capacity exceeded (status=%d); raise `growth`" % int(meta[:, 5].max()))
        out = []
        res = self.h_result.numpy()
        for f in range(self.batch):
            k = int(meta[f, 0])
            out.append(dict(box3d_lidar=res[f, :k, :7].copy(), scores=res[f, :k, 7].copy(),
                            label_preds=np.zeros((k,), np.int64), num_voxels=int(meta[f, 4]), num_candidates=int(meta[f, 1]),
                            anchor_index=meta[f, 8:8 + k].astype(np.int64)))
        return out

    def infer(self, clouds):
        self.stage(clouds)
        self.launch()
        return self.results()
```

### se-ssd_b200/sessd_b200/ops.py

```python
import ctypes as C

import numpy as np
import torch

from . import _lib
from ._lib import ConvDesc, DinmsCfg, Grid, PostCfg, VoxelCfg, check, lib


def _p(t):
    return C.c_void_p(t.data_ptr()) if t is not None else C.c_void_p(0)


def _st():
    return C.c_void_p(torch.cuda.current_stream().cuda_stream)


def _cuda(t, dtype, name):
    if not (isinstance(t, torch.Tensor) and t.is_cuda and t.dtype == dtype and t.is_contiguous()):
        raise ValueError("%s must be a contiguous CUDA %s tensor" % (name, dtype))
    return t


def _i3(v):
    return (C.c_int * 3)(*[int(x) for x in v])


def make_grid(batch, shape_dhw):
    g = Grid()
    g.batch = int(batch)
    g.shape[0], g.shape[1], g.shape[2] = [int(v) for v in shape_dhw]
    return g


def make_voxel_cfg(voxel_size, pc_range, max_points, max_voxels, num_feat=4):
    cfg = VoxelCfg()
    vs = np.asarray(voxel_size, np.float32)
    rg = np.asarray(pc_range, np.float32)
    grid = np.round((rg[3:] - rg[:3]) / vs).astype(np.int64)
    for j in range(3):
        cfg.voxel_size[j] = float(vs[j])
        cfg.range_min[j] = float(rg[j])
        cfg.range_max[j] = float(rg[3 + j])
        cfg.grid[j] = int(grid[j])
    cfg.max_points, cfg.max_voxels, cfg.num_feat = int(max_points), int(max_voxels), int(num_feat)
    return cfg


class VoxelBuffers:

    def __init__(self, cfg, batch, max_total_points, device, with_mean=True):
        self.cfg, self.batch, self.max_total_points = cfg, batch, max_total_points
        nv = batch * cfg.max_voxels
        self.voxels = torch.empty((nv, cfg.max_points, cfg.num_feat), dtype=torch.float32, device=device)
        self.coors = torch.empty((nv, 4), dtype=torch.int32, device=device)
        self.num_points = torch.empty((nv,), dtype=torch.int32, device=device)
        self.mean = torch.empty((nv, cfg.num_feat), dtype=torch.float32, device=device) if with_mean else None
        self.num_voxels = torch.zeros((batch + 1,), dtype=torch.int32, device=device)
        ws = lib.sessd_voxelize_workspace_bytes(max_total_points, batch, C.byref(cfg))
        self.ws = torch.empty((ws,), dtype=torch.uint8, device=device)


def voxelize(points, frame_off, buf):
    _cuda(points, torch.float32, "points")
    _cuda(frame_off, torch.int32, "frame_off")
    if points.shape[0] > buf.max_total_points or points.shape[1] != buf.cfg.num_feat or frame_off.numel() != buf.batch + 1:
        raise ValueError("voxelize: shape/capacity mismatch")
    rc = lib.sessd_voxelize(_p(points), _p(frame_off), buf.batch, buf.max_total_points, C.byref(buf.cfg), _p(buf.voxels),
                            _p(buf.coors), _p(buf.num_points), _p(buf.mean), _p(buf.num_voxels), _p(buf.ws), buf.ws.numel(), _st())
    check(rc, "sessd_voxelize")
    return buf


def voxelize_host(points_np, cfg):
    pts = np.ascontiguousarray(points_np, np.float32)
    if pts.ndim != 2 or pts.shape[1] != cfg.num_feat:
        raise ValueError("points must be [N,%d]" % cfg.num_feat)
    voxels = np.zeros((cfg.max_voxels, cfg.max_points, cfg.num_feat), np.float32)
    coors = np.zeros((cfg.max_voxels, 3), np.int32)
    num = np.zeros((cfg.max_voxels,), np.int32)
    m = lib.sessd_voxelize_host(pts.ctypes.data_as(C.c_void_p), pts.shape[0], C.byref(cfg), voxels.ctypes.data_as(C.c_void_p),
                                coors.ctypes.data_as(C.c_void_p), num.ctypes.data_as(C.c_void_p))
    if m < 0:
        raise _lib.SessdError("sessd_voxelize_host failed (%d)" % m)
    return voxels[:m].copy(), coors[:m].copy(), num[:m].copy()


def hash_capacity(max_rows):
    cap = C.c_int(0)
    lib.sessd_hash_bytes(int(max_rows), C.byref(cap))
    return cap.value


def hash_build(coors, n, max_rows, grid, table=None):
    cap = hash_capacity(max_rows)
    if table is None:
        table = torch.empty((cap,), dtype=torch.int64, device=coors.device)
    check(lib.sessd_hash_build(_p(coors), _p(n), int(max_rows), grid, _p(table), cap, _st()), "sessd_hash_build")
    return table


def bitmap_alloc(grid, device):
    words = lib.sessd_bitmap_words(grid)
    bitmap = torch.empty((words, 2), dtype=torch.int32, device=device)
    scratch = torch.empty((lib.sessd_scan_scratch_bytes(words),), dtype=torch.uint8, device=device)
    return bitmap, scratch


def subm_rulebook(coors, n, max_rows, grid, ksize, index_kind, index, nbr=None):
    kvol = int(ksize[0] * ksize[1] * ksize[2])
    if nbr is None:
        nbr = torch.empty((max_rows, kvol), dtype=torch.int32, device=coors.device)
    cap = index.numel() if index_kind == 0 else 0
    check(lib.sessd_subm_rulebook(_p(coors), _p(n), int(max_rows), grid, _i3(ksize), int(index_kind), _p(index), cap, _p(nbr), _st()),
          "sessd_subm_rulebook")
    return nbr


def strided_rulebook(in_coors, n_in, max_in, in_grid, in_index_kind, in_index, ksize, stride, padding, out_grid, bitmap,
                     scratch, out_coors, n_out, max_out, nbr, status):
    cap = in_index.numel() if in_index_kind == 0 else 0
    check(lib.sessd_strided_rulebook(_p(in_coors), _p(n_in), int(max_in), in_grid, int(in_index_kind), _p(in_index), cap, _i3(ksize),
                                     _i3(stride), _i3(padding), out_grid, _p(bitmap), _p(scratch), _p(out_coors), _p(n_out),
                                     int(max_out), _p(nbr), _p(status), _st()), "sessd_strided_rulebook")


def spconv_forward(in_feat, nbr, n_out, max_out, weight, scale, shift, relu, out=None):
    kvol, cin, cout = weight.shape
    if out is None:
        out = torch.empty((max_out, cout), dtype=torch.float32, device=in_feat.device)
    check(lib.sessd_spconv_forward(_p(in_feat), int(cin), _p(nbr), int(kvol), _p(n_out), int(max_out), _p(weight), int(cout),
                                   _p(scale), _p(shift), int(bool(relu)), _p(out), _st()), "sessd_spconv_forward")
    return out


def spconv_forward_rows(in_feat, nbr, n_out, max_out, weight, scale, shift, relu, out, amax_out=None):
    kvol, cin, cout = weight.shape
    check(lib.sessd_spconv_forward_rows(_p(in_feat), int(cin), _p(nbr), int(kvol), _p(n_out), int(max_out), _p(weight), int(cout),
                                        _p(scale), _p(shift), int(bool(relu)), _p(out), _p(amax_out), _st()), "sessd_spconv_forward_rows")
    return out


def _fp16_split(wt):
    amax = wt.abs().amax(dim=(0, 2))
    _, ex = torch.frexp(amax)
    e = torch.where(amax > 0, 11 - ex, torch.zeros_like(ex)).clamp(-100, 100).to(torch.float32)
    ws = wt * torch.exp2(e)[None, :, None]
    hi = ws.to(torch.float16)
    return hi, (ws - hi.to(torch.float32)).to(torch.float16), torch.exp2(-e).contiguous()


def pack_weight_sp_h2(wp, cp):
    kvol, cin, cout = wp.shape
    assert cp in (32, 64) and cin == cp
    hi, lo, inv = _fp16_split(wp.permute(0, 2, 1).contiguous().to(torch.float32))
    return torch.stack([hi, lo], 1).contiguous(), inv


def alloc_planes(max_rows, cp, device):
    return torch.zeros((max_rows + 1, 2 * cp), dtype=torch.float16, device=device)


def absmax_rows(feat, n, max_rows, amax):
    check(lib.sessd_absmax_rows(_p(feat), _p(n), int(max_rows), int(feat.shape[1]), _p(amax), _st()), "sessd_absmax_rows")
    return amax


def spconv_forward_rows_planes(in_feat, nbr, n_out, max_out, weight, scale, shift, relu, amax_in, gain, shift_max, out, out_planes, out_info):
    kvol, cin, cout = weight.shape
    check(lib.sessd_spconv_forward_rows_planes(_p(in_feat), int(cin), _p(nbr), int(kvol), _p(n_out), int(max_out), _p(weight), int(cout),
                                               _p(scale), _p(shift), int(bool(relu)), _p(amax_in), float(gain), float(shift_max), _p(out),
                                               _p(out_planes), int(out_planes.shape[1] // 2), _p(out_info), _st()),
          "sessd_spconv_forward_rows_planes")
    return out_planes


def alloc_tile_lists(max_out, kvol, device):
    return torch.zeros((-(-int(max_out) // 128), int(lib.sessd_tile_list_stride(int(kvol)))), dtype=torch.int32, device=device)


def rulebook_tile_lists(nbr, n_out, max_out, tiles):
    check(lib.sessd_rulebook_tile_lists(_p(nbr), int(nbr.shape[1]), _p(n_out), int(max_out), _p(tiles), _st()), "sessd_rulebook_tile_lists")
    return tiles


def spconv_forward_cg(in_planes, in_info, tiles, n_out, max_out, weight_h2, scale, shift, relu, gain, shift_max, out, out_planes, out_info):
    cp = in_planes.shape[1] // 2
    kvol = weight_h2.shape[0]
    cout = weight_h2.shape[2]
    check(lib.sessd_spconv_forward_cg(_p(in_planes), int(cp), int(in_planes.shape[0]), _p(in_info), _p(tiles), int(kvol), _p(n_out), int(max_out),
                                      _p(weight_h2), int(cout), _p(scale), _p(shift), int(bool(relu)), float(gain), float(shift_max), _p(out),
                                      _p(out_planes), _p(out_info), _st()), "sessd_spconv_forward_cg")
    return out if out is not None else out_planes


def set_sp_cg_deep(on):
    lib.sessd_set_sp_cg_deep(int(on))


def spconv_cg_blocks_per_sm(cp, cout, deep=0):
    n = int(lib.sessd_spconv_cg_blocks_per_sm(int(cp), int(cout), int(deep)))
    check(min(n, 0), "sessd_spconv_cg_blocks_per_sm")
    return n


def rulebook_transpose(nbr, n_out, max_out, max_in, nbr_t=None):
    kvol = int(nbr.shape[1])
    if nbr_t is None:
        nbr_t = torch.empty((int(max_in), kvol), dtype=torch.int32, device=nbr.device)
    check(lib.sessd_rulebook_transpose(_p(nbr), kvol, _p(n_out), int(max_out), int(max_in), _p(nbr_t), _st()), "sessd_rulebook_transpose")
    return nbr_t


def sparse_split_planes(x, n, max_rows, info, planes):
    check(lib.sessd_sparse_split_planes(_p(x), _p(n), int(max_rows), int(x.shape[1]), _p(info), _p(planes), int(planes.shape[1] // 2), _st()),
          "sessd_sparse_split_planes")
    return planes


def dense_grad_gather(grad, coors, n, max_rows, grid, channels, out=None):
    if out is None:
        out = torch.empty((int(max_rows), int(channels)), dtype=torch.float32, device=grad.device)
    check(lib.sessd_dense_grad_gather(_p(grad), _p(coors), _p(n), int(max_rows), int(channels), grid, _p(out), _st()), "sessd_dense_grad_gather")
    return out


def wgrad_items(max_out, kvol):
    return int(lib.sessd_spconv_wgrad_items(int(max_out), int(kvol)))


def wgrad_workspace(max_out, kvol, cin, cout, device):
    return torch.empty((int(lib.sessd_spconv_wgrad_workspace_bytes(int(max_out), int(kvol), int(cin), int(cout))),), dtype=torch.uint8,
                       device=device)


def spconv_wgrad_rows(in_feat, gout, tiles, n_out, max_out, kvol, gw=None, ws=None):
    cin, cout = int(in_feat.shape[1]), int(gout.shape[1])
    if gw is None:
        gw = torch.empty((int(kvol), cin, cout), dtype=torch.float32, device=gout.device)
    if ws is None:
        ws = wgrad_workspace(max_out, kvol, cin, cout, gout.device)
    check(lib.sessd_spconv_wgrad_rows(_p(in_feat), cin, _p(gout), cout, _p(tiles), int(kvol), _p(n_out), int(max_out), _p(gw), _p(ws), ws.numel(),
                                      _st()), "sessd_spconv_wgrad_rows")
    return gw


def spconv_wgrad_cg(in_planes, in_info, g_planes, g_info, tiles, n_out, max_out, kvol, gw=None, ws=None):
    cp, cout = int(in_planes.shape[1] // 2), int(g_planes.shape[1] // 2)
    if gw is None:
        gw = torch.empty((int(kvol), cp, cout), dtype=torch.float32, device=g_planes.device)
    if ws is None:
        ws = wgrad_workspace(max_out, kvol, cp, cout, g_planes.device)
    check(lib.sessd_spconv_wgrad_cg(_p(in_planes), cp, _p(in_info), _p(g_planes), cout, _p(g_info), _p(tiles), int(kvol), _p(n_out), int(max_out),
                                    _p(gw), _p(ws), ws.numel(), _st()), "sessd_spconv_wgrad_cg")
    return gw


def sparse_planes_to_float(planes, info, channels):
    cp = planes.shape[1] // 2
    return (planes[:, :channels].float() + planes[:, cp:cp + channels].float()) / info[1]


def sparse_to_dense(feat, coors, n, max_rows, grid, out=None):
    c = feat.shape[1]
    d, h, w = grid.shape[0], grid.shape[1], grid.shape[2]
    if out is None:
        out = torch.empty((grid.batch, h, w, c * d), dtype=torch.float32, device=feat.device)
    check(lib.sessd_sparse_to_dense(_p(feat), _p(coors), _p(n), int(max_rows), int(c), grid, _p(out), _st()), "sessd_sparse_to_dense")
    return out


def sparse_to_dense_indexed(feat, bitmap_index, grid, out):
    check(lib.sessd_sparse_to_dense_indexed(_p(feat), int(feat.shape[0]), _p(bitmap_index), int(feat.shape[1]), grid, _p(out), _st()),
          "sessd_sparse_to_dense_indexed")
    return out


def conv_desc(batch, in_hw, cin, out_hw, cout, grid_hw, taps, in_stride=1, out_stride=1, out_off=(0, 0), relu=True):
    d = ConvDesc()
    d.batch, d.in_h, d.in_w, d.cin = int(batch), int(in_hw[0]), int(in_hw[1]), int(cin)
    d.out_h, d.out_w, d.cout = int(out_hw[0]), int(out_hw[1]), int(cout)
    d.grid_h, d.grid_w = int(grid_hw[0]), int(grid_hw[1])
    d.in_stride, d.out_stride, d.out_off_y, d.out_off_x = int(in_stride), int(out_stride), int(out_off[0]), int(out_off[1])
    d.ntaps = len(taps)
    for t, (dy, dx) in enumerate(taps):
        d.tap_dy[t], d.tap_dx[t] = int(dy), int(dx)
    d.relu = int(bool(relu))
    return d


def pack_weight_h2(wp, cout_pad):
    taps, cin, cout = wp.shape
    wt = torch.zeros((taps, cout_pad, cin), dtype=torch.float32, device=wp.device)
    wt[:, :cout] = wp.permute(0, 2, 1)
    hi, lo, inv = _fp16_split(wt)
    return torch.stack([hi, lo], 0).contiguous(), inv


def bev_conv_h2(x, weight_h2, scale, shift, residual, out, desc, amax_in=None, amax_out=None):
    check(lib.sessd_bev_conv_h2(_p(x), _p(weight_h2), int(weight_h2.shape[2]), _p(scale), _p(shift), _p(residual), _p(out), C.byref(desc),
                                _p(amax_in), _p(amax_out), _st()), "sessd_bev_conv_h2")
    return out


def bev_deconv_h2(x, weight_h2, scale, shift, residual, out, relu=True, amax_in=None, amax_out=None):
    b, h, w, cin = x.shape
    check(lib.sessd_bev_deconv_h2(_p(x), _p(weight_h2), int(weight_h2.shape[2]), _p(scale), _p(shift), _p(residual), _p(out),
                                  int(b), int(h), int(w), int(cin), int(out.shape[-1]), int(bool(relu)), _p(amax_in), _p(amax_out), _st()),
          "sessd_bev_deconv_h2")
    return out


def alloc_bev_planes(batch, h, w, c, device):
    return torch.zeros((2, batch, h, w, c), dtype=torch.float16, device=device)


def conv_gain(wp, scale):
    g = wp.abs().sum(dim=(0, 1)) * scale.abs().to(wp.device)[: wp.shape[2]]
    return float(g.max()) * (1.0 + 1e-5)


def bev_conv_p2(in_planes, in_info, weight_h2, scale, shift, residual, resid_info, gain, shift_max, out_f32, out_planes, out_info, desc,
                items=None):
    check(lib.sessd_bev_conv_p2(_p(in_planes), _p(in_info), _p(weight_h2), int(weight_h2.shape[2]), _p(scale), _p(shift), _p(residual),
                                _p(resid_info), float(gain), float(shift_max), _p(out_f32), _p(out_planes), _p(out_info), C.byref(desc),
                                _p(items), _st()), "sessd_bev_conv_p2")


def bev_deconv_p2(in_planes, in_info, weight_h2, scale, shift, residual, resid_info, gain, shift_max, out_f32, out_planes, out_info, relu=True,
                  items=None):
    _two, b, h, w, cin = in_planes.shape
    cout = (out_f32 if out_f32 is not None else out_planes).shape[-1]
    check(lib.sessd_bev_deconv_p2(_p(in_planes), _p(in_info), _p(weight_h2), int(weight_h2.shape[2]), _p(scale), _p(shift), _p(residual),
                                  _p(resid_info), float(gain), float(shift_max), _p(out_f32), _p(out_planes), _p(out_info), int(b), int(h),
                                  int(w), int(cin), int(cout), int(bool(relu)), _p(items), _st()), "sessd_bev_deconv_p2")


class BevSkipPlan:

    LAUNCHES = 13

    def __init__(self, batch, h, w, device):
        offs = (C.c_int * self.LAUNCHES)()
        words = lib.sessd_bev_skip_plan_words(int(batch), int(h), int(w), offs)
        if words <= 0:
            raise ValueError("no skip plan for a [%d, %d, %d] neck" % (batch, h, w))
        self.offsets = list(offs)
        self.buf = torch.zeros((int(words),), dtype=torch.int32, device=device)

    def record(self, i):
        return self.buf[self.offsets[i]:]

    def build(self, bitmap_index, grid):
        check(lib.sessd_bev_skip_plan(_p(bitmap_index), grid, _p(self.buf), _st()), "sessd_bev_skip_plan")

    def fill(self, i, out_f32, out_planes, cout):
        check(lib.sessd_bev_skip_fill(_p(self.record(i)), _p(out_f32), _p(out_planes), int(cout), _st()), "sessd_bev_skip_fill")


def bev_split_planes(x, info, planes):
    check(lib.sessd_bev_split_planes(_p(x), int(x.numel()), _p(info), _p(planes), _st()), "sessd_bev_split_planes")
    return planes


def bev_wgrad_workspace(desc, device):
    n = int(lib.sessd_bev_wgrad_workspace_bytes(C.byref(desc)))
    if n == 0:
        raise ValueError("sessd_bev_wgrad: no weight gradient for this descriptor")
    return torch.empty((n,), dtype=torch.uint8, device=device)


def bev_wgrad(in_planes, in_info, g_planes, g_info, desc, gw=None, ws=None):
    if gw is None:
        gw = torch.empty((desc.ntaps, desc.cin, desc.cout), dtype=torch.float32, device=g_planes.device)
    if ws is None:
        ws = bev_wgrad_workspace(desc, g_planes.device)
    check(lib.sessd_bev_wgrad(_p(in_planes), _p(in_info), _p(g_planes), _p(g_info), C.byref(desc), _p(gw), _p(ws), ws.numel(), _st()),
          "sessd_bev_wgrad")
    return gw


def planes_to_float(planes, info):
    return (planes[0].float() + planes[1].float()) / info[1]


def sparse_to_dense_planes(feat, bitmap_index, grid, amax, info, planes):
    check(lib.sessd_sparse_to_dense_planes(_p(feat), int(feat.shape[0]), _p(bitmap_index), int(feat.shape[1]), grid, _p(amax), _p(info),
                                           _p(planes), _st()), "sessd_sparse_to_dense_planes")
    return planes


def ssfa_fuse_planes(x0, x1, w0, w1, s0, t0, s1, t1, out, info0, info1, out_info, planes):
    npix = x0.numel() // x0.shape[-1]
    check(lib.sessd_ssfa_fuse_planes(_p(x0), _p(x1), _p(w0), _p(w1), float(s0), float(t0), float(s1), float(t1), int(npix), int(x0.shape[-1]),
                                     _p(out), _p(info0), _p(info1), _p(out_info), _p(planes), _st()), "sessd_ssfa_fuse_planes")
    return out


def absmax(x, amax):
    check(lib.sessd_absmax(_p(x), int(x.numel()), _p(amax), _st()), "sessd_absmax")
    return amax


NMS_TYPES = ("rotate_nms", "rotate_weighted_nms")
DINMS_MAX_PRE = 4096


def make_dinms_cfg(nms_cnt_thresh=2.6, nms_sigma_dist_interval=(0, 20, 40, 60), nms_sigma_square=(0.0009, 0.009, 0.1, 1),
                   suppressed_thresh=0.3, centerness_pow=2, enable_centerness=True):
    if len(nms_sigma_dist_interval) != 4 or len(nms_sigma_square) < 3:
        raise ValueError("DI-NMS takes four distance edges (three bands) and their three sigma^2")
    d = DinmsCfg()
    d.cnt_thresh, d.suppressed_thresh, d.centerness_pow = float(nms_cnt_thresh), float(suppressed_thresh), float(centerness_pow)
    for j in range(4):
        d.dist_edge[j] = float(nms_sigma_dist_interval[j])
    for j in range(3):
        d.sigma2[j] = float(nms_sigma_square[j])
    d.centerness = int(bool(enable_centerness))
    return d


def make_post_cfg(batch, num_anchors=70400, anchors_per_loc=2, head_stride=24, score_thresh=0.3, nms_pre_max=1000, nms_post_max=100,
                  nms_iou_thresh=0.01, nms_ge=True, post_range=(0, -40.0, -5.0, 70.4, 40.0, 5.0), direction_offset=0.0,
                  use_frustum=False, nms_type="rotate_nms"):
    if nms_type not in NMS_TYPES:
        raise ValueError("nms_type must be one of %s, not %r" % (NMS_TYPES, nms_type))
    c = PostCfg()
    c.batch, c.num_anchors, c.anchors_per_loc, c.head_stride = int(batch), int(num_anchors), int(anchors_per_loc), int(head_stride)
    c.score_thresh, c.nms_pre_max, c.nms_post_max = float(score_thresh), int(nms_pre_max), int(nms_post_max)
    c.nms_iou_thresh, c.nms_ge = float(nms_iou_thresh), int(bool(nms_ge))
    for j in range(6):
        c.post_range[j] = float(post_range[j])
    c.direction_offset, c.use_frustum = float(direction_offset), int(bool(use_frustum))
    if nms_type == "rotate_weighted_nms":
        c.nms_mode, c.dinms = 1, make_dinms_cfg()
    return c


def post_capacity(cfg):
    return cfg.nms_pre_max if cfg.nms_mode == 1 else cfg.nms_post_max


class PostBuffers:
    def __init__(self, cfg, device):
        self.cfg = cfg
        b, p = cfg.batch, post_capacity(cfg)
        self.boxes = torch.zeros((b, p, 7), dtype=torch.float32, device=device)
        self.scores = torch.zeros((b, p), dtype=torch.float32, device=device)
        self.labels = torch.zeros((b, p), dtype=torch.int32, device=device)
        self.count = torch.zeros((b,), dtype=torch.int32, device=device)
        self.aux = torch.zeros((b, 4), dtype=torch.int32, device=device)
        self.sel_anchor = torch.zeros((b, p), dtype=torch.int32, device=device)
        self.ws = torch.empty((lib.sessd_postprocess_workspace_bytes(C.byref(cfg)),), dtype=torch.uint8, device=device)


def postprocess(head, anchors, frustum_planes, buf):
    check(lib.sessd_postprocess(_p(head), _p(anchors), _p(frustum_planes), C.byref(buf.cfg), _p(buf.boxes), _p(buf.scores), _p(buf.labels),
                                _p(buf.count), _p(buf.aux), _p(buf.sel_anchor), _p(buf.ws), buf.ws.numel(), _st()), "sessd_postprocess")
    return buf


def postprocess_packed(head, anchors, frustum_planes, buf, packed, meta, num_voxels=None, status=None):
    check(lib.sessd_postprocess_packed(_p(head), _p(anchors), _p(frustum_planes), C.byref(buf.cfg), _p(buf.boxes), _p(buf.scores),
                                       _p(buf.labels), _p(buf.count), _p(buf.aux), _p(buf.sel_anchor), _p(packed), _p(meta),
                                       _p(num_voxels), _p(status), _p(buf.ws), buf.ws.numel(), _st()), "sessd_postprocess_packed")
    return buf


def rotate_nms(boxes5, scores, n, max_boxes, pre_max, post_max, iou_thresh, ge=True):
    dev = boxes5.device
    keep = torch.empty((post_max,), dtype=torch.int32, device=dev)
    num = torch.zeros((1,), dtype=torch.int32, device=dev)
    ws = torch.empty((lib.sessd_rotate_nms_workspace_bytes(int(max_boxes), int(pre_max)),), dtype=torch.uint8, device=dev)
    check(lib.sessd_rotate_nms(_p(boxes5), _p(scores), _p(n), int(max_boxes), int(pre_max), int(post_max), float(iou_thresh),
                               int(bool(ge)), _p(keep), _p(num), _p(ws), ws.numel(), _st()), "sessd_rotate_nms")
    return keep, num


def rotate_weighted_nms(boxes7, boxes5, scores, iou_preds, labels, dirs, anchors, n, max_boxes, pre_max, dinms_cfg, ws=None):
    dev = scores.device
    for t, dt, name in ((boxes7, torch.float32, "boxes7"), (boxes5, torch.float32, "boxes5"), (scores, torch.float32, "scores"),
                        (iou_preds, torch.float32, "iou_preds"), (labels, torch.int32, "labels"), (dirs, torch.int32, "dirs"),
                        (n, torch.int32, "n")):
        _cuda(t, dt, name)
    if anchors is not None:
        _cuda(anchors, torch.float32, "anchors")
    p = int(pre_max)
    out = dict(boxes=torch.empty((p, 7), dtype=torch.float32, device=dev), scores=torch.empty((p,), dtype=torch.float32, device=dev),
               labels=torch.empty((p,), dtype=torch.int32, device=dev), dirs=torch.empty((p,), dtype=torch.int32, device=dev),
               keep=torch.empty((p,), dtype=torch.int32, device=dev), selected=torch.empty((p,), dtype=torch.int32, device=dev),
               count=torch.zeros((2,), dtype=torch.int32, device=dev))
    if ws is None:
        ws = torch.empty((max(lib.sessd_rotate_weighted_nms_workspace_bytes(int(max_boxes), p), 1),), dtype=torch.uint8, device=dev)
    check(lib.sessd_rotate_weighted_nms(_p(boxes7), _p(boxes5), _p(scores), _p(iou_preds), _p(labels), _p(dirs), _p(anchors), _p(n),
                                        int(max_boxes), p, C.byref(dinms_cfg), _p(out["boxes"]), _p(out["scores"]), _p(out["labels"]),
                                        _p(out["dirs"]), _p(out["keep"]), _p(out["selected"]), _p(out["count"]), _p(ws), ws.numel(),
                                        _st()), "sessd_rotate_weighted_nms")
    return out


def boxes_overlap_bev(a, b, out):
    check(lib.sessd_boxes_overlap_bev(_p(a), a.shape[0], _p(b), b.shape[0], _p(out), _st()), "sessd_boxes_overlap_bev")
    return out


def boxes_aligned_overlap_bev(a, b, out):
    check(lib.sessd_boxes_aligned_overlap_bev(_p(a), _p(b), a.shape[0], _p(out), _st()), "sessd_boxes_aligned_overlap_bev")
    return out


def boxes_iou_bev(a, b, out):
    check(lib.sessd_boxes_iou_bev(_p(a), a.shape[0], _p(b), b.shape[0], _p(out), _st()), "sessd_boxes_iou_bev")
    return out


def boxes_iou3d(a, b, out):
    check(lib.sessd_boxes_iou3d(_p(a), a.shape[0], _p(b), b.shape[0], _p(out), _st()), "sessd_boxes_iou3d")
    return out


def nms_sorted(boxes, thresh, mode):
    n = boxes.shape[0]
    dev = boxes.device
    keep = torch.empty((max(n, 1),), dtype=torch.int64, device=dev)
    num = torch.zeros((1,), dtype=torch.int32, device=dev)
    ws = torch.empty((lib.sessd_nms_workspace_bytes(n),), dtype=torch.uint8, device=dev)
    check(lib.sessd_nms_sorted(_p(boxes), n, float(thresh), int(mode), _p(keep), _p(num), _p(ws), ws.numel(), _st()), "sessd_nms_sorted")
    return keep, num


class AssignBuffers:

    def __init__(self, num_anchors, batch, max_gt, device):
        self.num_anchors, self.batch, self.max_gt = int(num_anchors), int(batch), int(max_gt)
        z = lambda shape, dt: torch.zeros(shape, dtype=dt, device=device)
        self.labels = z((batch, num_anchors), torch.int32)
        self.bbox_targets = z((batch, num_anchors, 7), torch.float32)
        self.bbox_outside_weights = z((batch, num_anchors), torch.float32)
        self.pos_anchor = z((batch, num_anchors), torch.int32)
        self.pos_gt_id = z((batch, num_anchors), torch.int32)
        self.num_pos = z((batch,), torch.int32)
        self.ws = torch.empty((lib.sessd_assign_workspace_bytes(self.num_anchors, self.batch, self.max_gt),), dtype=torch.uint8,
                              device=device)


def assign_targets(anchors, gt_boxes, num_gt, buf, matched_thr=0.6, unmatched_thr=0.45):
    _cuda(anchors, torch.float32, "anchors"); _cuda(gt_boxes, torch.float32, "gt_boxes"); _cuda(num_gt, torch.int32, "num_gt")
    assert anchors.shape == (buf.num_anchors, 7) and tuple(gt_boxes.shape) == (buf.batch, buf.max_gt, 7) and num_gt.numel() == buf.batch
    check(lib.sessd_assign_targets(_p(anchors), buf.num_anchors, _p(gt_boxes), _p(num_gt), buf.batch, buf.max_gt, float(matched_thr),
                                   float(unmatched_thr), _p(buf.labels), _p(buf.bbox_targets), _p(buf.bbox_outside_weights),
                                   _p(buf.pos_anchor), _p(buf.pos_gt_id), _p(buf.num_pos), _p(buf.ws), buf.ws.numel(), _st()),
          "sessd_assign_targets")
    return buf


def head_loss(head, anchors, labels, reg_targets, alpha=0.25, sigma=3.0, dir_offset=0.0, pos_cls_weight=1.0, neg_cls_weight=1.0,
              w_cls=1.0, w_loc=2.0, w_dir=0.2, w_iou=None, with_grad=True):
    _cuda(head, torch.float32, "head"); _cuda(anchors, torch.float32, "anchors"); _cuda(labels, torch.int32, "labels")
    _cuda(reg_targets, torch.float32, "reg_targets")
    B, A = labels.shape
    assert head.shape[0] == B and head.shape[1] * 2 == A and anchors.shape == (A, 7) and tuple(reg_targets.shape) == (B, A, 7)
    losses = torch.empty((B, 8), dtype=torch.float32, device=head.device)
    grad = torch.empty_like(head) if with_grad else None
    ws = torch.empty((lib.sessd_head_loss_workspace_bytes(int(B)),), dtype=torch.uint8, device=head.device)
    check(lib.sessd_head_loss(_p(head), _p(anchors), _p(labels), _p(reg_targets), int(B), int(A), 2, int(head.shape[2]), float(alpha), float(sigma),
                              float(dir_offset), float(pos_cls_weight), float(neg_cls_weight), float(w_cls), float(w_loc), float(w_dir),
                              _p(losses), _p(grad), _p(ws), ws.numel(), _st()), "sessd_head_loss")
    if w_iou is not None:
        ws2 = torch.empty((lib.sessd_iou_pred_loss_workspace_bytes(int(B)),), dtype=torch.uint8, device=head.device)
        check(lib.sessd_iou_pred_loss(_p(head), _p(anchors), _p(labels), _p(reg_targets), int(B), int(A), 2, int(head.shape[2]), float(sigma),
                                      float(w_iou), _p(losses), _p(grad), _p(ws2), ws2.numel(), _st()), "sessd_iou_pred_loss")
    return losses, grad


def odiou_pairs_host(gboxes, qboxes, with_grad=True):
    g = np.ascontiguousarray(gboxes, np.float32).reshape(-1, 7)
    q = np.ascontiguousarray(qboxes, np.float32).reshape(-1, 7)
    assert g.shape == q.shape
    out = np.zeros((g.shape[0],), np.float32)
    grad = np.zeros_like(q) if with_grad else None
    check(lib.sessd_odiou_pairs_host(g.ctypes.data_as(C.c_void_p), q.ctypes.data_as(C.c_void_p), int(g.shape[0]), out.ctypes.data_as(C.c_void_p),
                                     grad.ctypes.data_as(C.c_void_p) if with_grad else C.c_void_p(0)), "sessd_odiou_pairs_host")
    return out, grad


def odiou_loss(head, anchors, labels, reg_targets, losses, grad_head=None, w_odiou=2.0):
    B, A = labels.shape
    out = torch.empty((B,), dtype=torch.float32, device=head.device)
    ws = torch.empty((lib.sessd_odiou_loss_workspace_bytes(int(B)),), dtype=torch.uint8, device=head.device)
    check(lib.sessd_odiou_loss(_p(head), _p(anchors), _p(labels), _p(reg_targets), int(B), int(A), 2, int(head.shape[2]), float(w_odiou),
                               _p(losses), _p(out), _p(grad_head), _p(ws), ws.numel(), _st()), "sessd_odiou_loss")
    return out


def box_collision(boxes, qboxes, out=None):
    _cuda(boxes, torch.float64, "boxes"); _cuda(qboxes, torch.float64, "qboxes")
    n, k = boxes.shape[0], qboxes.shape[0]
    if out is None:
        out = torch.empty((n, k), dtype=torch.uint8, device=boxes.device)
    check(lib.sessd_box_collision(_p(boxes), int(n), _p(qboxes), int(k), _p(out), _st()), "sessd_box_collision")
    return out


def _aug_inputs(gt_boxes, num_gt, valid, loc_noise, rot_noise, selected=None):
    _cuda(gt_boxes, torch.float32, "gt_boxes"); _cuda(num_gt, torch.int32, "num_gt"); _cuda(valid, torch.uint8, "valid")
    _cuda(loc_noise, torch.float64, "loc_noise"); _cuda(rot_noise, torch.float64, "rot_noise")
    B, M = valid.shape
    T = rot_noise.shape[2]
    if (tuple(gt_boxes.shape) != (B, M, 7) or num_gt.numel() != B or tuple(loc_noise.shape) != (B, M, T, 3)
            or tuple(rot_noise.shape) != (B, M, T)):
        raise ValueError("augmentation inputs: shape mismatch")
    if selected is not None:
        _cuda(selected, torch.int32, "selected")
        if tuple(selected.shape) != (B, M):
            raise ValueError("selected must be [B, M]")
    return B, M, T


def points_in_boxes(points, boxes, context=-1.0, mask=None):
    _cuda(points, torch.float32, "points"); _cuda(boxes, torch.float32, "boxes")
    if points.dim() != 2 or points.shape[1] < 3 or boxes.dim() != 2 or boxes.shape[1] != 7:
        raise ValueError("points_in_boxes: points [N, >=3], boxes [M, 7]")
    n, m = points.shape[0], boxes.shape[0]
    if mask is None:
        mask = torch.empty((n, m), dtype=torch.uint8, device=points.device)
    check(lib.sessd_points_in_boxes(_p(points), int(n), int(points.shape[1]), _p(boxes), int(m), float(context), _p(mask), _st()),
          "sessd_points_in_boxes")
    return mask


def noise_per_box(gt_boxes, num_gt, valid, loc_noise, rot_noise, context=-1.0, selected=None):
    B, M, T = _aug_inputs(gt_boxes, num_gt, valid, loc_noise, rot_noise)
    if selected is None:
        selected = torch.empty((B, M), dtype=torch.int32, device=gt_boxes.device)
    _cuda(selected, torch.int32, "selected")
    check(lib.sessd_noise_per_box(_p(gt_boxes), _p(num_gt), _p(valid), int(B), int(M), _p(loc_noise), _p(rot_noise), int(T),
                                  float(context), _p(selected), _st()), "sessd_noise_per_box")
    return selected


def augment_points(points, frame_off, max_frame_points, gt_boxes, num_gt, valid, loc_noise, rot_noise, selected, glob, perm, labeled=None,
                   context=-1.0, points_raw=None, points_out=None, with_raw=True):
    B, M, T = _aug_inputs(gt_boxes, num_gt, valid, loc_noise, rot_noise, selected)
    _cuda(points, torch.float32, "points"); _cuda(frame_off, torch.int32, "frame_off"); _cuda(glob, torch.float32, "glob")
    _cuda(perm, torch.int32, "perm")
    if labeled is not None:
        _cuda(labeled, torch.uint8, "labeled")
        if labeled.numel() != B:
            raise ValueError("labeled must be [B]")
    if points.dim() != 2 or points.shape[1] != 4 or frame_off.numel() != B + 1 or perm.numel() != points.shape[0] or tuple(glob.shape) != (B, 5):
        raise ValueError("augment_points: shape mismatch")
    if not with_raw:
        points_raw = None
    elif points_raw is None:
        points_raw = torch.empty_like(points)
    if points_out is None:
        points_out = torch.empty_like(points)
    written = (("points_raw", points_raw), ("points_out", points_out)) if with_raw else (("points_out", points_out),)
    for name, t in written:
        _cuda(t, torch.float32, name)
        if t.shape != points.shape:
            raise ValueError("%s must be shaped like points" % name)
    if any(t.data_ptr() % 16 for t in (points, points_out) + ((points_raw,) if with_raw else ())):
        raise ValueError("augment_points: point rows are read and written as float4 and must be 16-byte aligned")
    check(lib.sessd_augment_points(_p(points), _p(frame_off), int(B), int(max_frame_points), _p(gt_boxes), _p(num_gt), _p(valid), int(M),
                                   _p(loc_noise), _p(rot_noise), int(T), _p(selected), float(context), _p(glob), _p(perm), _p(labeled),
                                   _p(points_raw), _p(points_out), _st()), "sessd_augment_points")
    return points_raw, points_out


def augment_boxes(gt_boxes, num_gt, valid, target, loc_noise, rot_noise, selected, glob, range_bev, global_boxes=False):
    B, M, T = _aug_inputs(gt_boxes, num_gt, valid, loc_noise, rot_noise, selected)
    _cuda(glob, torch.float32, "glob")
    if tuple(glob.shape) != (B, 5):
        raise ValueError("glob must be [B, 5]")
    if target is not None:
        _cuda(target, torch.uint8, "target")
        if tuple(target.shape) != (B, M):
            raise ValueError("target must be [B, M]")
    dev = gt_boxes.device
    boxes_raw = torch.empty((B, M, 7), dtype=torch.float32, device=dev)
    boxes_out = torch.empty((B, M, 7), dtype=torch.float32, device=dev)
    num_raw = torch.empty((B,), dtype=torch.int32, device=dev)
    num_out = torch.empty((B,), dtype=torch.int32, device=dev)
    boxes_glob = torch.empty((B, M, 7), dtype=torch.float32, device=dev) if global_boxes else None
    num_glob = torch.empty((B,), dtype=torch.int32, device=dev) if global_boxes else None
    rg = (C.c_float * 4)(*[float(v) for v in range_bev])
    check(lib.sessd_augment_boxes(_p(gt_boxes), _p(num_gt), _p(valid), _p(target), int(B), int(M), _p(loc_noise), _p(rot_noise), int(T),
                                  _p(selected), _p(glob), rg, _p(boxes_raw), _p(num_raw), _p(boxes_out), _p(num_out), _p(boxes_glob),
                                  _p(num_glob), _st()), "sessd_augment_boxes")
    res = (boxes_raw, num_raw, boxes_out, num_out)
    return res + (boxes_glob, num_glob) if global_boxes else res


def gtaug_select_host(corners, num_boxes):
    corners = np.ascontiguousarray(corners, np.float64)
    if corners.ndim != 3 or corners.shape[1:] != (4, 2) or not 0 <= num_boxes <= corners.shape[0]:
        raise ValueError("gtaug_select_host: corners [num_boxes + K, 4, 2], 0 <= num_boxes <= rows")
    k = corners.shape[0] - int(num_boxes)
    acc = np.zeros(max(k, 1), np.uint8)
    rc = lib.sessd_gtaug_select_host(corners.ctypes.data_as(C.c_void_p), int(num_boxes), int(k), acc.ctypes.data_as(C.c_void_p))
    if rc < 0:
        check(rc, "sessd_gtaug_select_host")
    return acc[:k].astype(bool)


def gtaug_paste(points, frame_off, obj_off, obj_ids, db_points, db_off, db_count, db_boxes, max_paste_points, out=None,
                frame_off_out=None):
    _cuda(points, torch.float32, "points"); _cuda(frame_off, torch.int32, "frame_off"); _cuda(db_points, torch.float32, "db_points")
    _cuda(db_off, torch.int32, "db_off"); _cuda(db_count, torch.int32, "db_count"); _cuda(db_boxes, torch.float64, "db_boxes")
    B = frame_off.numel() - 1
    N = db_count.numel()
    if isinstance(obj_ids, np.ndarray) or isinstance(obj_off, np.ndarray):
        ids = np.asarray(obj_ids).reshape(-1); off = np.asarray(obj_off).reshape(-1)
        if ids.size and (ids.min() < 0 or ids.max() >= N):
            raise ValueError("gtaug_paste: object id out of range [0, %d)" % N)
        if off.size != B + 1 or off[0] != 0 or off[-1] != ids.size or (np.diff(off) < 0).any():
            raise ValueError("gtaug_paste: obj_off must be a CSR offset array [B+1] over the ids")
        host = np.concatenate([off.astype(np.int32), ids.astype(np.int32)])
        dev_ids = torch.from_numpy(host).to(points.device)
        obj_off, obj_ids = dev_ids[:B + 1], dev_ids[B + 1:]
    _cuda(obj_off, torch.int32, "obj_off"); _cuda(obj_ids, torch.int32, "obj_ids")
    if (B < 1 or points.dim() != 2 or points.shape[1] != 4 or obj_off.numel() != B + 1 or db_points.dim() != 2 or db_points.shape[1] != 4
            or db_off.numel() != N or tuple(db_boxes.shape) != (N, 7)):
        raise ValueError("gtaug_paste: shape mismatch")
    cap = int(points.shape[0]) + int(max_paste_points)
    dev = points.device
    if out is None:
        out = torch.empty((max(cap, 1), 4), dtype=torch.float32, device=dev)
    if frame_off_out is None:
        frame_off_out = torch.empty((B + 1,), dtype=torch.int32, device=dev)
    _cuda(out, torch.float32, "out"); _cuda(frame_off_out, torch.int32, "frame_off_out")
    if out.dim() != 2 or out.shape[1] != 4 or frame_off_out.numel() != B + 1:
        raise ValueError("gtaug_paste: out [capacity, 4], frame_off_out [B+1]")
    if any(t.data_ptr() % 16 for t in (points, db_points, out)):
        raise ValueError("gtaug_paste: point rows are read and written as float4 and must be 16-byte aligned")
    K = obj_ids.numel()
    ws = torch.empty((int(lib.sessd_gtaug_paste_workspace_bytes(B, int(points.shape[0]), K)),), dtype=torch.uint8, device=dev)
    check(lib.sessd_gtaug_paste(_p(points), _p(frame_off), int(B), int(points.shape[0]), _p(obj_off), _p(obj_ids), int(K),
                                int(max_paste_points), _p(db_points), _p(db_off), _p(db_count), _p(db_boxes), int(N), _p(ws),
                                ws.numel(), _p(out), int(out.shape[0]), _p(frame_off_out), _st()), "sessd_gtaug_paste")
    return out, frame_off_out


SADA_MAX_IDS = 6 * 256


def _rows4(points, name):
    _cuda(points, torch.float32, name)
    if points.dim() != 2 or points.shape[1] != 4:
        raise ValueError("%s must be [N, 4]" % name)
    if points.data_ptr() % 16:
        raise ValueError("%s: point rows are read and written as float4 and must be 16-byte aligned" % name)
    return points


def _count(d_n, name="n"):
    if d_n is not None:
        _cuda(d_n, torch.int32, name)
        if d_n.numel() < 1:
            raise ValueError("%s must hold one count" % name)
    return d_n


def _ids(ids, num_pyramids, device):
    if not isinstance(ids, torch.Tensor):
        ids = np.asarray(ids, np.int64).reshape(-1)
        if ids.size and (ids.min() < 0 or ids.max() >= num_pyramids):
            raise ValueError("pyramid id out of range [0, %d)" % num_pyramids)
        if ids.size > SADA_MAX_IDS:
            raise ValueError("at most %d listed pyramids" % SADA_MAX_IDS)
        ids = torch.from_numpy(ids.astype(np.int32)).to(device)
    return _cuda(ids, torch.int32, "ids")


def sada_pyramids(boxes):
    _cuda(boxes, torch.float32, "boxes")
    if boxes.dim() != 2 or boxes.shape[1] != 7:
        raise ValueError("sada_pyramids: boxes [K, 7]")
    K = boxes.shape[0]
    pyr = torch.empty((6 * K, 15), dtype=torch.float32, device=boxes.device)
    planes = torch.empty((6 * K, 5, 4), dtype=torch.float32, device=boxes.device)
    if K == 0:
        return pyr, planes
    check(lib.sessd_sada_pyramids(_p(boxes), int(K), _p(pyr), _p(planes), _st()), "sessd_sada_pyramids")
    return pyr, planes


def sada_membership(points, planes, ids, n=None, with_bits=True):
    _rows4(points, "points"); _cuda(planes, torch.float32, "planes"); _count(n)
    if planes.dim() != 3 or tuple(planes.shape[1:]) != (5, 4):
        raise ValueError("planes must be [P, 5, 4]")
    dev = points.device
    ids = _ids(ids, planes.shape[0], dev)
    A, N = ids.numel(), points.shape[0]
    bits = torch.empty((N, max(-(-A // 32), 1)), dtype=torch.int32, device=dev) if with_bits else None
    counts = torch.zeros((max(A, 1),), dtype=torch.int32, device=dev)
    check(lib.sessd_sada_membership(_p(points), int(N), _p(n), _p(planes), int(planes.shape[0]), _p(ids), int(A), _p(bits), _p(counts),
                                    _st()), "sessd_sada_membership")
    return bits, counts[:A], ids


def sada_compact(points, bits, counts, min_count=-1, n=None, out=None):
    _rows4(points, "points"); _cuda(bits, torch.int32, "bits"); _cuda(counts, torch.int32, "counts"); _count(n)
    N, A = points.shape[0], counts.numel()
    if bits.shape[0] != N or bits.shape[1] * 32 < A:
        raise ValueError("sada_compact: bits [N, ceil(A / 32)]")
    dev = points.device
    out = _rows4(torch.empty((max(N, 1), 4), dtype=torch.float32, device=dev) if out is None else out, "out")
    num = torch.empty((1,), dtype=torch.int32, device=dev)
    ws = torch.empty((max(int(lib.sessd_sada_compact_workspace_bytes(int(N))), 16),), dtype=torch.uint8, device=dev)
    check(lib.sessd_sada_compact(_p(points), int(N), _p(n), _p(bits), int(A), _p(counts), int(min_count), _p(ws), ws.numel(), _p(out),
                                 int(out.shape[0]), _p(num), _st()), "sessd_sada_compact")
    return out, num


def sada_fps(points, bits, counts, min_count, k, out, num, n=None):
    _rows4(points, "points"); _cuda(bits, torch.int32, "bits"); _cuda(counts, torch.int32, "counts"); _rows4(out, "out")
    _count(num, "num"); _count(n)
    N, A = points.shape[0], counts.numel()
    if bits.shape[0] != N or bits.shape[1] * 32 < A:
        raise ValueError("sada_fps: bits [N, ceil(A / 32)]")
    ws = torch.empty((max(int(lib.sessd_sada_fps_workspace_bytes(int(N), int(A))), 16),), dtype=torch.uint8, device=points.device)
    check(lib.sessd_sada_fps(_p(points), int(N), _p(n), _p(bits), int(A), _p(counts), int(min_count), int(k), _p(ws), ws.numel(), _p(out),
                             int(out.shape[0]), _p(num), _st()), "sessd_sada_fps")
    return out, num


def sada_swap(points, bits, counts, pyramids, ids, max_swap_points, out, num_in, n=None):
    _rows4(points, "points"); _cuda(bits, torch.int32, "bits"); _cuda(counts, torch.int32, "counts"); _rows4(out, "out")
    _cuda(pyramids, torch.float32, "pyramids"); _cuda(ids, torch.int32, "ids"); _count(num_in, "num_in"); _count(n)
    N, A = points.shape[0], ids.numel()
    if A % 2 or counts.numel() != A or bits.shape[0] != N or bits.shape[1] * 32 < A or pyramids.dim() != 2 or pyramids.shape[1] != 15:
        raise ValueError("sada_swap: shape mismatch")
    num_out = torch.empty((1,), dtype=torch.int32, device=points.device)
    check(lib.sessd_sada_swap(_p(points), int(N), _p(n), _p(bits), int(A // 2), _p(counts), _p(pyramids), int(pyramids.shape[0]), _p(ids),
                              int(max_swap_points), _p(out), int(out.shape[0]), _p(num_in), _p(num_out), _st()), "sessd_sada_swap")
    return out, num_out


def sada_shuffle(points, frame_off, max_frame_points, perm, out=None):
    _rows4(points, "points"); _cuda(frame_off, torch.int32, "frame_off"); _cuda(perm, torch.int32, "perm")
    if perm.numel() != points.shape[0]:
        raise ValueError("sada_shuffle: perm [P]")
    out = _rows4(torch.empty_like(points) if out is None else out, "out")
    if out.shape != points.shape:
        raise ValueError("sada_shuffle: out must be shaped like points")
    check(lib.sessd_sada_shuffle(_p(points), _p(frame_off), int(frame_off.numel() - 1), int(max_frame_points), _p(perm), _p(out), _st()),
          "sessd_sada_shuffle")
    return out


def _rows16(name, *ts):
    if any(t is not None and t.data_ptr() % 16 for t in ts):
        raise ValueError("%s: point rows are read and written as float4 and must be 16-byte aligned" % name)


def prep_frustum_compact(points, frame_off, planes, out=None, frame_off_out=None):
    _cuda(points, torch.float32, "points"); _cuda(frame_off, torch.int32, "frame_off"); _cuda(planes, torch.float64, "planes")
    B = frame_off.numel() - 1
    P = int(points.shape[0])
    if B < 1 or points.dim() != 2 or points.shape[1] != 4 or tuple(planes.shape) != (B, 6, 4):
        raise ValueError("prep_frustum_compact: points [P, 4], frame_off [B+1], planes [B, 6, 4]")
    dev = points.device
    if out is None:
        out = torch.empty((max(P, 1), 4), dtype=torch.float32, device=dev)
    if frame_off_out is None:
        frame_off_out = torch.empty((B + 1,), dtype=torch.int32, device=dev)
    _cuda(out, torch.float32, "out"); _cuda(frame_off_out, torch.int32, "frame_off_out")
    _rows16("prep_frustum_compact", points, out)
    ws = torch.empty((max(int(lib.sessd_prep_frustum_compact_workspace_bytes(P)), 16),), dtype=torch.uint8, device=dev)
    check(lib.sessd_prep_frustum_compact(_p(points), _p(frame_off), int(B), P, _p(planes), _p(ws), ws.numel(), _p(out), int(out.shape[0]),
                                         _p(frame_off_out), _st()), "sessd_prep_frustum_compact")
    return out, frame_off_out


def prep_box_count(points, frame_off, box_planes, box_off, counts=None):
    _cuda(points, torch.float32, "points"); _cuda(frame_off, torch.int32, "frame_off"); _cuda(box_planes, torch.float64, "box_planes")
    _cuda(box_off, torch.int32, "box_off")
    B = frame_off.numel() - 1
    K = int(box_planes.shape[0])
    if B < 1 or points.dim() != 2 or points.shape[1] != 4 or tuple(box_planes.shape[1:]) != (6, 4) or box_off.numel() != B + 1:
        raise ValueError("prep_box_count: points [P, 4], frame_off [B+1], box_planes [K, 6, 4], box_off [B+1]")
    if counts is None:
        counts = torch.empty((max(K, 1),), dtype=torch.int32, device=points.device)
    _cuda(counts, torch.int32, "counts")
    _rows16("prep_box_count", points)
    check(lib.sessd_prep_box_count(_p(points), _p(frame_off), int(B), int(points.shape[0]), _p(box_planes), _p(box_off), K, _p(counts),
                                   _st()), "sessd_prep_box_count")
    return counts[:K]


def prep_box_gather(points, frame_off, box_planes, centres, box_off, counts, num_rows, out=None, obj_off=None):
    _cuda(points, torch.float32, "points"); _cuda(frame_off, torch.int32, "frame_off"); _cuda(box_planes, torch.float64, "box_planes")
    _cuda(centres, torch.float64, "centres"); _cuda(box_off, torch.int32, "box_off"); _cuda(counts, torch.int32, "counts")
    B = frame_off.numel() - 1
    K = int(box_planes.shape[0])
    if (B < 1 or points.dim() != 2 or points.shape[1] != 4 or tuple(box_planes.shape[1:]) != (6, 4) or tuple(centres.shape) != (K, 3)
            or box_off.numel() != B + 1 or counts.numel() < K):
        raise ValueError("prep_box_gather: shape mismatch")
    dev = points.device
    if out is None:
        out = torch.empty((max(int(num_rows), 1), 4), dtype=torch.float32, device=dev)
    if obj_off is None:
        obj_off = torch.empty((K + 1,), dtype=torch.int32, device=dev)
    _cuda(out, torch.float32, "out"); _cuda(obj_off, torch.int32, "obj_off")
    _rows16("prep_box_gather", points, out)
    ws = torch.empty((max(int(lib.sessd_prep_box_gather_workspace_bytes(K)), 16),), dtype=torch.uint8, device=dev)
    check(lib.sessd_prep_box_gather(_p(points), _p(frame_off), int(B), int(points.shape[0]), _p(box_planes), _p(centres), _p(box_off), K,
                                    _p(counts), int(num_rows), _p(ws), ws.numel(), _p(out), int(out.shape[0]), _p(obj_off), _st()),
          "sessd_prep_box_gather")
    return out[:int(num_rows)], obj_off
```

### se-ssd_b200/sessd_b200/runners.py

```python
import itertools
import math

import torch
from sessd_data.layers import SPMIDDLE_LAYERS
from sessd_data.layers import SSFA_LAUNCHES, ssfa_extents

from . import ops

BN_EPS = 1e-3

def conv_out_shape(shape, ksize, stride, padding):
    return tuple((int(i) + 2 * p - k) // s + 1 for i, k, s, p in zip(shape, ksize, stride, padding))


def fold_bn(gamma, beta, mean, var, eps=BN_EPS):
    scale = gamma.float() / torch.sqrt(var.float() + eps)
    shift = beta.float() - mean.float() * scale
    return scale.contiguous(), shift.contiguous()


def sparse_impl(cin, use_tc=True):
    if not use_tc:
        return "simt"
    return "rows" if cin <= 16 else "cg"


def plane_width(channels):
    return 32 if channels <= 32 else 64


def spmiddle_plan(use_tc=True, keep_f32=False, cin0=4):
    plan, cin, lvl = [], cin0, 0
    for kind, cout, ks, st, pd, key in SPMIDDLE_LAYERS:
        lout = lvl if kind == "subm" else lvl + 1
        rb = key if kind == "subm" else "sp%d" % lout
        impl = sparse_impl(cin, use_tc)
        plan.append(dict(kind=kind, key=key, ks=ks, st=st, pd=pd, cin=cin, cout=cout, lin=lvl, lout=lout, rb=rb,
                         build_rb=all(p["rb"] != rb for p in plan), impl=impl, cp_in=plane_width(cin) if impl == "cg" else None))
        cin, lvl = cout, lout
    nxt = {}
    for p in reversed(plan):
        p["tile_lists"] = p["build_rb"] and any(q["impl"] == "cg" for q in plan if q["rb"] == p["rb"])
        p["cp_out"] = nxt.get("cp_in")
        p["out_f32"] = keep_f32 or p["cp_out"] is None
        p["out_info"] = p["impl"] == "cg" or p["cp_out"] is not None or (nxt.get("impl") == "rows" and nxt["cp_out"] is not None)
        nxt = p
    return plan


class SpMiddleRunner:

    GROWTH = (1.0, 4.0, 6.0, 5.0, 3.0)

    def __init__(self, batch, max_voxels_total, input_shape_xyz=(1408, 1600, 40), num_input_features=4, device="cuda",
                 growth=None, use_tc=True, keep_f32=False):
        self.batch, self.device = batch, torch.device(device)
        self.use_tc, self.keep_f32 = bool(use_tc), bool(keep_f32)
        shape = (int(input_shape_xyz[2]) + 1, int(input_shape_xyz[1]), int(input_shape_xyz[0]))
        growth = growth or self.GROWTH
        self.levels = []
        self._add_level(shape, int(max_voxels_total), hash_index=True)
        self.plan = spmiddle_plan(self.use_tc, self.keep_f32, num_input_features)
        rulebooks = {}
        for p in self.plan:
            if p["kind"] != "subm":
                oshape = conv_out_shape(self.levels[p["lin"]]["shape"], p["ks"], p["st"], p["pd"])
                cells = batch * oshape[0] * oshape[1] * oshape[2]
                self._add_level(oshape, min(cells, int(math.ceil(max_voxels_total * growth[p["lout"]]))), hash_index=False)
            if p["build_rb"]:
                cap, kvol = self.levels[p["lout"]]["cap"], p["ks"][0] * p["ks"][1] * p["ks"][2]
                rulebooks[p["rb"]] = (torch.empty((cap, kvol), dtype=torch.int32, device=self.device),
                                      ops.alloc_tile_lists(cap, kvol, self.device) if p["tile_lists"] else None)
            p["nbr"], p["tiles"] = rulebooks[p["rb"]]
        caps = [self.levels[p["lout"]]["cap"] for p in self.plan]
        self.feats = [torch.zeros((cap, p["cout"]), dtype=torch.float32, device=self.device) if p["out_f32"] else None
                      for p, cap in zip(self.plan, caps)]
        self.planes = [ops.alloc_planes(cap, p["cp_out"], self.device) if p["cp_out"] else None for p, cap in zip(self.plan, caps)]
        assert all(pl is None or pl.shape[0] <= (1 << 25) for pl in self.planes)
        last = self.levels[-1]
        self.out_channels = self.plan[-1]["cout"] * last["shape"][0]
        self.dense = torch.zeros((batch, last["shape"][1], last["shape"][2], self.out_channels), dtype=torch.float32,
                                 device=self.device)
        self.status = torch.zeros((1,), dtype=torch.int32, device=self.device)
        self.weights = None
        self.info = torch.zeros((len(self.plan), 2), dtype=torch.float32, device=self.device)

    def layer_output(self, li):
        p = self.plan[li]
        if p["out_f32"]:
            return self.feats[li]
        return ops.sparse_planes_to_float(self.planes[li][:-1], self.info[li], p["cout"])

    def _add_level(self, shape, cap, hash_index):
        grid = ops.make_grid(self.batch, shape)
        lv = dict(shape=shape, cap=cap, grid=grid, n=torch.zeros((1,), dtype=torch.int32, device=self.device))
        if hash_index:
            lv["index_kind"] = 0
            lv["index"] = torch.empty((ops.hash_capacity(cap),), dtype=torch.int64, device=self.device)
            lv["coors"] = None
        else:
            lv["index_kind"] = 1
            lv["index"], lv["scratch"] = ops.bitmap_alloc(grid, self.device)
            lv["coors"] = torch.zeros((cap, 4), dtype=torch.int32, device=self.device)
        self.levels.append(lv)

    def load_weights(self, layers):
        assert len(layers) == len(self.plan)
        self.weights = []
        for p, l in zip(self.plan, layers):
            w = torch.as_tensor(l["weight"], dtype=torch.float32, device=self.device)
            assert tuple(w.shape) == (*p["ks"], p["cin"], p["cout"]), (w.shape, p)
            sc, sh = fold_bn(*[torch.as_tensor(l[k], device=self.device) for k in ("gamma", "beta", "mean", "var")], eps=float(l.get("eps", BN_EPS)))
            wp = w.reshape(-1, p["cin"], p["cout"]).contiguous()
            p["gain"], p["shift_max"] = ops.conv_gain(wp, sc), float(sh.abs().max())
            if p["impl"] == "cg":
                tiles, inv = ops.pack_weight_sp_h2(wp, p["cp_in"])
                self.weights.append((tiles, (sc * inv).contiguous(), sh))
            else:
                self.weights.append((wp, sc, sh))

    def forward(self, feat0, coors0, n0, mark=None, dense_planes=None):
        mark = mark or (lambda label: None)
        assert self.weights is not None, "load_weights first"
        L0 = self.levels[0]
        cap0 = min(coors0.shape[0], L0["cap"])
        L0["coors"], L0["n_ext"] = coors0, n0
        ops.hash_build(coors0, n0, cap0, L0["grid"], L0["index"])
        mark("hash_build")
        if self.use_tc:
            self.info.zero_()
        x = feat0
        for li, p in enumerate(self.plan):
            lin, lout = self.levels[p["lin"]], self.levels[p["lout"]]
            n_in = lin["n_ext"] if p["lin"] == 0 else lin["n"]
            cap_in = cap0 if p["lin"] == 0 else lin["cap"]
            n_out, cap_out = (n_in, cap_in) if p["kind"] == "subm" else (lout["n"], lout["cap"])
            if p["build_rb"]:
                if p["kind"] == "subm":
                    ops.subm_rulebook(lin["coors"], n_in, cap_in, lin["grid"], p["ks"], lin["index_kind"], lin["index"], p["nbr"])
                else:
                    ops.strided_rulebook(lin["coors"], n_in, cap_in, lin["grid"], lin["index_kind"], lin["index"], p["ks"], p["st"],
                                         p["pd"], lout["grid"], lout["index"], lout["scratch"], lout["coors"], lout["n"], lout["cap"],
                                         p["nbr"], self.status)
                if p["tiles"] is not None:
                    ops.rulebook_tile_lists(p["nbr"], n_out, cap_out, p["tiles"])
                mark("rulebook:" + p["rb"])
            w, sc, sh = self.weights[li]
            out = self.feats[li]
            if p["impl"] == "rows" and p["cp_out"]:
                ops.spconv_forward_rows_planes(x, p["nbr"], n_out, cap_out, w, sc, sh, True, self.info[li - 1, 0:1], p["gain"], p["shift_max"],
                                               out, self.planes[li], self.info[li])
            elif p["impl"] == "rows":
                ops.spconv_forward_rows(x, p["nbr"], n_out, cap_out, w, sc, sh, True, out, self.info[li, 0:1] if p["out_info"] else None)
            elif p["impl"] == "cg":
                ops.spconv_forward_cg(self.planes[li - 1], self.info[li - 1], p["tiles"], n_out, cap_out, w, sc, sh, True, p["gain"],
                                      p["shift_max"], out, self.planes[li], self.info[li])
            else:
                ops.spconv_forward(x, p["nbr"], n_out, cap_out, w, sc, sh, True, out)
            mark("conv:%d" % li)
            x = out
        last = self.levels[-1]
        if dense_planes is not None:
            assert self.plan[-1]["out_info"], "the planes' scale needs the last layer's abs-max (use_tc)"
            out = ops.sparse_to_dense_planes(x, last["index"], last["grid"], self.info[-1, 0:1], dense_planes[1], dense_planes[0])
        else:
            out = ops.sparse_to_dense_indexed(x, last["index"], last["grid"], self.dense)
        mark("dense")
        return out


class RunnerCache:

    def __init__(self):
        self.runner = self.key = self.weights = None

    def get(self, module, key, build, load):
        if self.runner is None or key != self.key:
            self.runner, self.key, self.weights = build(), key, None
        weights = tuple((t.data_ptr(), t._version) for t in itertools.chain(module.parameters(), module.buffers()))
        if weights != self.weights:
            load(self.runner)
            self.weights = weights
        return self.runner


_SSFA = {L.name: L for L in SSFA_LAUNCHES}


def conv_taps(k):
    return [(dy - k // 2, dx - k // 2) for dy in range(k) for dx in range(k)]


def _pack_conv(w):
    cout, cin, kh, kw = w.shape
    packed = w.permute(2, 3, 1, 0).reshape(kh * kw, cin, cout).contiguous()
    return packed, [(ky, kx) for ky in range(kh) for kx in range(kw)]


def launch_weight(L, w):
    if L.kind == "deconv":
        return w.permute(2, 3, 0, 1).reshape(9, L.cin, L.cout).contiguous(), None
    return _pack_conv(w)[0], conv_taps(L.k)


def launch_desc(L, batch, in_hw, out_hw, taps, relu=None):
    return ops.conv_desc(batch, in_hw, L.cin, out_hw, L.cout, out_hw, taps, in_stride=L.stride, relu=L.relu if relu is None else relu)


def head_weight(param):
    w, b = (torch.cat([param(c + s) for c in ("conv_box", "conv_cls", "conv_dir", "conv_iou")], 0) for s in (".weight", ".bias"))
    pad = _SSFA["head"].cout - w.shape[0]
    return torch.cat([w, w.new_zeros((pad,) + tuple(w.shape[1:]))], 0), torch.cat([b, b.new_zeros((pad,))], 0)


def pack_head(head_sd, prefix, device):
    return head_weight(lambda name: head_sd[prefix + name].to(device, torch.float32))


def fold_ssfa_bn(sd, conv_name, device, eps=BN_EPS):
    blk, idx = conv_name.rsplit(".", 1)
    b = "%s.%d." % (blk, int(idx) + 1)
    return fold_bn(*(sd[b + k].to(device, torch.float32) for k in ("weight", "bias", "running_mean", "running_var")), eps=eps)


def pack_h2(wp, taps, scale, shift):
    planes, inv = ops.pack_weight_h2(wp, _cout_pad(wp.shape[2]))
    scale = torch.ones(wp.shape[2], device=wp.device) if scale is None else scale
    return dict(w=planes, scale=(scale * inv[:scale.numel()]).contiguous(), shift=shift.contiguous(), gain=ops.conv_gain(wp, scale),
                shift_max=float(shift.abs().max()), taps=taps)


def _cout_pad(cout):
    n_tile = 32 if cout <= 32 else 128
    return -(-cout // n_tile) * n_tile


def ssfa_weights(ssfa_sd, head_sd, head_prefix, device, bn_eps=BN_EPS):
    for L in SSFA_LAUNCHES:
        if L.name != "head":
            wp, taps = launch_weight(L, ssfa_sd[L.name + ".weight"].to(device, torch.float32))
            yield (L, wp, taps) + fold_ssfa_bn(ssfa_sd, L.name, device, bn_eps)
        elif head_sd is not None:
            w, bias = pack_head(head_sd, head_prefix, device)
            yield (L, *launch_weight(L, w), None, bias)


def ssfa_fuse_weights(ssfa_sd, device, bn_eps=BN_EPS):
    out = {}
    for name in ("w_0.0", "w_1.0"):
        sc, sh = fold_ssfa_bn(ssfa_sd, name, device, bn_eps)
        out[name] = (ssfa_sd[name + ".weight"].to(device, torch.float32).reshape(-1).contiguous(), float(sc[0]), float(sh[0]))
    return out


SSFA_SLOT = {n: i for i, n in enumerate(["x"] + [L.dst for L in SSFA_LAUNCHES if not L.f32] + ["out"] + [L.dst for L in SSFA_LAUNCHES if L.f32])}


class SSFAPlanesRunner:

    HEAD_STRIDE = 24
    SLOT = SSFA_SLOT
    SKIP_LAUNCHES = tuple(L.name for L in SSFA_LAUNCHES)

    def __init__(self, batch, hw=(200, 176), device="cuda", skip_constant=False):
        self.batch, self.h, self.w, self.device = batch, int(hw[0]), int(hw[1]), torch.device(device)
        pl = lambda hw_, c: ops.alloc_bev_planes(batch, hw_[0], hw_[1], c, self.device)
        z = lambda hw_, c: torch.zeros((batch,) + hw_ + (c,), dtype=torch.float32, device=self.device)
        H, ext = (self.h, self.w), lambda L: ssfa_extents(L, self.h, self.w)[1]
        self.planes = dict(x=pl(H, 128), **{L.dst: pl(ext(L), L.cout) for L in SSFA_LAUNCHES if not L.f32}, out=pl(H, 128))
        self.buf = dict(**{L.dst: z(ext(L), L.cout) for L in SSFA_LAUNCHES[:-1] if L.f32}, out=z(H, 128), head=z(H, self.HEAD_STRIDE))
        self.info = torch.zeros((16, 2), dtype=torch.float32, device=self.device)
        self.params = None
        self.skip_constant = bool(skip_constant)
        self.skip = ops.BevSkipPlan(batch, self.h, self.w, self.device) if self.skip_constant else None

    def _info(self, name):
        return self.info[self.SLOT[name]]

    def load_state(self, ssfa_sd, head_sd=None, head_prefix="tasks.0.", bn_eps=BN_EPS):
        P = ssfa_fuse_weights(ssfa_sd, self.device, bn_eps)
        for L, *weight in ssfa_weights(ssfa_sd, head_sd, head_prefix, self.device, bn_eps):
            P[L.name] = pack_h2(*weight)
        self.params = P

    def _split(self, x, name):
        self.info.zero_()
        ops.absmax(x, self._info(name)[0:1])
        ops.bev_split_planes(x, self._info(name), self.planes[name])

    def _launch(self, L, skip=False):
        q = self.params[L.name]
        out_f32, out_planes = (self.buf[L.dst], None) if L.f32 else (None, self.planes[L.dst])
        resid, resid_info = (self.buf[L.residual], self._info(L.residual)) if L.residual else (None, None)
        i = self.SKIP_LAUNCHES.index(L.name)
        rec = self.skip.record(i) if skip else None
        if L.kind == "conv":
            d = launch_desc(L, self.batch, *ssfa_extents(L, self.h, self.w), q["taps"])
            ops.bev_conv_p2(self.planes[L.src], self._info(L.src), q["w"], q["scale"], q["shift"], resid, resid_info, q["gain"],
                            q["shift_max"], out_f32, out_planes, self._info(L.dst), d, items=rec)
        else:
            ops.bev_deconv_p2(self.planes[L.src], self._info(L.src), q["w"], q["scale"], q["shift"], resid, resid_info, q["gain"],
                              q["shift_max"], out_f32, out_planes, self._info(L.dst), L.relu, items=rec)
        if skip:
            self.skip.fill(i, out_f32, out_planes, L.cout)

    def forward(self, x=None, mark=None, occupancy=None):
        assert self.params is not None, "load_state first"
        mark = mark or (lambda label: None)
        if x is not None:
            self._split(x, "x")
        skip = self.skip_constant and occupancy is not None
        if skip:
            index, grid = occupancy
            assert (grid.batch, grid.shape[1], grid.shape[2]) == (self.batch, self.h, self.w), "occupancy of another map"
            self.skip.build(index, grid)
            mark("neck:skip_plan")
        for L in SSFA_LAUNCHES[:-1]:
            self._launch(L, skip)
            mark("neck:" + L.name)
        w0, s0, t0 = self.params["w_0.0"]
        w1, s1, t1 = self.params["w_1.0"]
        ops.ssfa_fuse_planes(self.buf["o0"], self.buf["o1"], w0, w1, s0, t0, s1, t1, self.buf["out"], self._info("o0"), self._info("o1"),
                             self._info("out"), self.planes["out"])
        if "head" not in self.params:
            mark("neck:fuse+head")
            return self.buf["out"], None
        self.head(skip=skip)
        mark("neck:fuse+head")
        return self.buf["out"], self.buf["head"]

    def head(self, skip=False):
        self._launch(SSFA_LAUNCHES[-1], skip)
        return self.buf["head"]

    def activation(self, name):
        if name in self.buf:
            return self.buf[name]
        return ops.planes_to_float(self.planes[name], self._info(name))

    def bench_layer(self, name="bottom_up_block_0.4"):

        def launch():
            self._launch(_SSFA[name]._replace(src="x0", dst="b0b"))

        return launch, "bev_conv_p2_kernel (fp16 wgmma from pre-split fp16 planes, two-term split)"


class HeadRunner(SSFAPlanesRunner):

    def __init__(self, batch, hw, device="cuda"):
        self.batch, self.h, self.w, self.device = batch, int(hw[0]), int(hw[1]), torch.device(device)
        self.planes = dict(out=ops.alloc_bev_planes(batch, self.h, self.w, 128, self.device))
        self.buf = dict(head=torch.zeros((batch, self.h, self.w, self.HEAD_STRIDE), dtype=torch.float32, device=self.device))
        self.info = torch.zeros((len(self.SLOT), 2), dtype=torch.float32, device=self.device)
        self.params = None

    def load_state(self, head_sd, prefix=""):
        w, bias = pack_head(head_sd, prefix, self.device)
        self.params = {"head": pack_h2(*launch_weight(_SSFA["head"], w), None, bias)}

    def forward(self, x):
        self._split(x, "out")
        return self.head()
```

Before: 1549.

## Fuse SSFA attention blend into head convolution prologue

Adds a fused mode to the p2 tensor-core conv kernel. It TMA-loads the two f32 SSFA branch outputs, computes the softmax-weighted blend per pixel in shared memory, and splits the result into hi/lo half planes before the wgmma taps. The standalone ssfa_fuse kernel and the 'out' fp32 and plane buffers are dropped when fused_head is enabled, which the engine now sets by default. This removes one kernel launch and a full-map write and read round trip, but the head kernel now carries extra per-tile prologue work and synchronisation, and the engine no longer returns the fused neck output tensor.

```diff
diff --git a/include/sessd_b200.h b/include/sessd_b200.h
--- a/include/sessd_b200.h
+++ b/include/sessd_b200.h
@@ -114,6 +114,10 @@
                         const float *d_shift, const float *d_residual, const float *d_resid_info, float gain, float shift_max,
                         float *d_out_f32, void *d_out_planes, float *d_out_info, int batch, int in_h, int in_w, int cin, int cout,
                         int relu, const int *d_items, void *stream);
+int sessd_bev_conv_p2_ssfa(const float *d_x0, const float *d_x1, const float *d_info0, const float *d_info1, const float *d_w0,
+                           const float *d_w1, float s0, float t0, float s1, float t1, float *d_fused_info, const void *d_weight_h2,
+                           int cout_pad, const float *d_scale, const float *d_shift, float gain, float shift_max, float *d_out_f32,
+                           float *d_out_info, const sessd_conv_desc *desc, const int *d_items, void *stream);
 long long sessd_bev_skip_plan_words(int batch, int h, int w, int *offsets);
 int sessd_bev_skip_plan(const void *d_bitmap_index, sessd_grid grid, int *d_plan, void *stream);
 int sessd_bev_skip_fill(const int *d_record, float *d_out_f32, void *d_out_planes, int cout, void *stream);
diff --git a/se-ssd_b200/csrc/bevconv.cu b/se-ssd_b200/csrc/bevconv.cu
--- a/se-ssd_b200/csrc/bevconv.cu
+++ b/se-ssd_b200/csrc/bevconv.cu
@@ -1,6 +1,7 @@
 #include <cuda_fp16.h>
 
 #include "common.cuh"
+#include "ssfa_fuse.cuh"
 
 namespace sessd {
 
@@ -21,31 +22,19 @@
             const float4 b = *reinterpret_cast<const float4 *>(x1 + (size_t)p * C + c);
             const float4 u = *reinterpret_cast<const float4 *>(w0 + c);
             const float4 v = *reinterpret_cast<const float4 *>(w1 + c);
-            d0 += a.x * u.x + a.y * u.y + a.z * u.z + a.w * u.w;
-            d1 += b.x * v.x + b.y * v.y + b.z * v.z + b.w * v.w;
+            d0 = __fadd_rn(d0, ssfa_dot4(a, u));
+            d1 = __fadd_rn(d1, ssfa_dot4(b, v));
         }
-#pragma unroll
-        for (int o = 16; o > 0; o >>= 1) { d0 += __shfl_xor_sync(0xffffffffu, d0, o); d1 += __shfl_xor_sync(0xffffffffu, d1, o); }
-        const float l0 = fmaf(d0, s0, t0), l1 = fmaf(d1, s1, t1);
-        const float mx = fmaxf(l0, l1);
-        const float e0 = expf(l0 - mx), e1 = expf(l1 - mx);
-        const float inv = 1.0f / (e0 + e1);
-        const float a0 = e0 * inv, a1 = e1 * inv;
+        const float2 aw = ssfa_pair_weights(ssfa_warp_sum(d0), ssfa_warp_sum(d1), s0, t0, s1, t1);
         for (int c = lane * 4; c < C; c += 128) {
             const float4 a = *reinterpret_cast<const float4 *>(x0 + (size_t)p * C + c);
             const float4 b = *reinterpret_cast<const float4 *>(x1 + (size_t)p * C + c);
-            float4 r;
-            r.x = a.x * a0 + b.x * a1; r.y = a.y * a0 + b.y * a1; r.z = a.z * a0 + b.z * a1; r.w = a.w * a0 + b.w * a1;
+            const float4 r = ssfa_mix4(a, b, aw);
             if (out) *reinterpret_cast<float4 *>(out + (size_t)p * C + c) = r;
-            const float q[4] = {r.x * sp, r.y * sp, r.z * sp, r.w * sp};
-            __align__(8) __half hi[4], lo[4];
-#pragma unroll
-            for (int e = 0; e < 4; ++e) {
-                hi[e] = __float2half_rn(q[e]);
-                lo[e] = __float2half_rn(q[e] - __half2float(hi[e]));
-            }
-            *reinterpret_cast<uint2 *>(planes + (size_t)p * C + c) = *reinterpret_cast<const uint2 *>(hi);
-            *reinterpret_cast<uint2 *>(planes + plane_stride + (size_t)p * C + c) = *reinterpret_cast<const uint2 *>(lo);
+            uint2 hi, lo;
+            ssfa_split4(r, sp, hi, lo);
+            *reinterpret_cast<uint2 *>(planes + (size_t)p * C + c) = hi;
+            *reinterpret_cast<uint2 *>(planes + plane_stride + (size_t)p * C + c) = lo;
         }
     }
 }
diff --git a/se-ssd_b200/csrc/bevconv_p2.cu b/se-ssd_b200/csrc/bevconv_p2.cu
--- a/se-ssd_b200/csrc/bevconv_p2.cu
+++ b/se-ssd_b200/csrc/bevconv_p2.cu
@@ -32,6 +32,21 @@
                               d_out_f32, d_out_planes, d_out_info, desc, stream, d_items);
 }
 
+extern "C" int sessd_bev_conv_p2_ssfa(const float *d_x0, const float *d_x1, const float *d_info0, const float *d_info1, const float *d_w0,
+                                      const float *d_w1, float s0, float t0, float s1, float t1, float *d_fused_info, const void *d_weight_h2,
+                                      int cout_pad, const float *d_scale, const float *d_shift, float gain, float shift_max, float *d_out_f32,
+                                      float *d_out_info, const sessd_conv_desc *desc, const int *d_items, void *stream) {
+    if (!desc || !d_w0 || !d_w1 || (((uintptr_t)d_w0 | (uintptr_t)d_w1) & 15)) return SESSD_EINVAL;
+    P2Params p;
+    P2Taps t;
+    if (p2_conv_params(*desc, p, t)) return SESSD_EINVAL;
+    p.items = d_items;
+    p.fuse_w0 = d_w0; p.fuse_w1 = d_w1; p.fuse_info1 = d_info1; p.fuse_out_info = d_fused_info;
+    p.fuse_s0 = s0; p.fuse_t0 = t0; p.fuse_s1 = s1; p.fuse_t1 = t1;
+    return launch_p2<kP2FuseF32>(d_x0, desc->in_h, desc->in_w, d_info0, d_weight_h2, desc->ntaps, cout_pad, d_scale, d_shift, nullptr, nullptr,
+                                 gain, shift_max, d_out_f32, nullptr, d_out_info, p, &t, 1, desc->grid_h, desc->grid_w, false, stream, d_x1);
+}
+
 extern "C" int sessd_bev_deconv_p2(const void *d_in_planes, const float *d_in_info, const void *d_weight_h2, int cout_pad, const float *d_scale,
                                    const float *d_shift, const float *d_residual, const float *d_resid_info, float gain, float shift_max,
                                    float *d_out_f32, void *d_out_planes, float *d_out_info, int batch, int in_h, int in_w, int cin, int cout,
diff --git a/se-ssd_b200/csrc/bevconv_p2.cuh b/se-ssd_b200/csrc/bevconv_p2.cuh
--- a/se-ssd_b200/csrc/bevconv_p2.cuh
+++ b/se-ssd_b200/csrc/bevconv_p2.cuh
@@ -1,6 +1,7 @@
 #pragma once
 #include <cuda_fp16.h>
 
+#include "ssfa_fuse.cuh"
 #include "tc_common.cuh"
 
 namespace sessd {
@@ -16,7 +17,8 @@
 constexpr int kP2MaxSmem = 227 * 1024;
 constexpr int kP2Chunk = 32;
 constexpr int kP2ItemsHeader = 32;
-enum { kP2Planes = 0, kP2SplitF16 = 1 };
+enum { kP2Planes = 0, kP2SplitF16 = 1, kP2FuseF32 = 2 };
+constexpr int kP2FuseGroups = 4, kP2FuseRows = kP2TileU * kP2TileV / kP2FuseGroups;
 enum { kP2NoProbe = 0, kP2ProbeClocks = 1, kP2ProbeLoads = 2 };
 
 struct P2Params {
@@ -46,6 +48,9 @@
     long long out_plane_stride;
     const int *items;
     long long *prof;
+    const float *fuse_w0, *fuse_w1, *fuse_info1;
+    float fuse_s0, fuse_t0, fuse_s1, fuse_t1;
+    float *fuse_out_info;
 };
 
 enum P2Prof {
@@ -135,8 +140,35 @@
     asm volatile("bar.sync 1, %0;\n" ::"n"(kP2MmaWarps * 32) : "memory");
 }
 
+__device__ __forceinline__ void p2_fuse_patch(const P2Params &p, const unsigned char *staging, unsigned char *planes, uint64_t *full,
+                                              uint64_t *empty, uint32_t phase, float s_in, float4 w0, float4 w1, int wg, int wq, int lane) {
+    asm volatile("bar.sync %0, 128;\n" ::"r"(2 + wg) : "memory");
+    const int j = (lane >> 1) & 3;
+    unsigned char *dst = planes + 2 * (lane >> 3) * p.copy_bytes + (lane & 1) * 8;
+    for (int g = 2 * wg; g < 2 * wg + 2; ++g) {
+        mbar_wait(&full[g], phase);
+        const float4 *x0 = reinterpret_cast<const float4 *>(staging + g * p.load_bytes), *x1 = x0 + kP2FuseRows * 32;
+#pragma unroll 4
+        for (int i = 0; i < kP2FuseRows / 4; ++i) {
+            const int lr = 4 * i + wq, r = g * kP2FuseRows + lr;
+            const float4 a = x0[lr * 32 + lane], b = x1[lr * 32 + lane];
+            const float d0 = ssfa_warp_sum(__fadd_rn(0.f, ssfa_dot4(a, w0))), d1 = ssfa_warp_sum(__fadd_rn(0.f, ssfa_dot4(b, w1)));
+            uint2 hi, lo;
+            ssfa_split4(ssfa_mix4(a, b, ssfa_pair_weights(d0, d1, p.fuse_s0, p.fuse_t0, p.fuse_s1, p.fuse_t1)), s_in, hi, lo);
+            unsigned char *o = dst + r * 64 + ((j ^ ((r >> 1) & 3)) << 4);
+            *reinterpret_cast<uint2 *>(o) = hi;
+            *reinterpret_cast<uint2 *>(o + p.copy_bytes) = lo;
+        }
+        __syncwarp();
+        if (lane == 0) mbar_arrive(&empty[g]);
+    }
+    asm volatile("fence.proxy.async.shared::cta;\n" ::: "memory");
+    asm volatile("bar.sync %0, 128;\n" ::"r"(2 + wg) : "memory");
+}
+
 template <int NT, int MODE, bool REGA = false, int PROBE = kP2NoProbe>
 __global__ void __launch_bounds__(REGA ? kP2ThreadsRegA : kP2Threads, 1) bev_conv_p2_kernel(const __grid_constant__ CUtensorMap map_a,
+                                                                   const __grid_constant__ CUtensorMap map_a1,
                                                                    const __grid_constant__ CUtensorMap map_b,
                                                                    const float *__restrict__ scale, const float *__restrict__ shift,
                                                                    const float *__restrict__ resid, float *__restrict__ out_f32,
@@ -148,19 +180,24 @@
     unsigned char *patches = tiles + p.bring_bytes;
     unsigned char *staging = patches + p.npatch * p.patch_bytes;
     uint64_t *bars = (uint64_t *)(staging + p.npatch * p.staging_bytes);
-    uint64_t *patch_full = bars, *patch_empty = bars + 2, *b_full = bars + 4, *b_empty = bars + 4 + kP2MaxBStages;
+    uint64_t *patch_full = bars, *patch_empty = bars + kP2FuseGroups, *b_full = bars + 2 * kP2FuseGroups;
+    uint64_t *b_empty = b_full + kP2MaxBStages;
     uint32_t *s_aoff = (uint32_t *)(b_empty + kP2MaxBStages);
     float *s_scale = (float *)(((uintptr_t)(s_aoff + 4 * 9) + 15) & ~(uintptr_t)15), *s_shift = s_scale + p.cout;
 
     const int warp = threadIdx.x >> 5, lane = threadIdx.x & 31;
     if (threadIdx.x == kP2PatchWarp * 32) prefetch_tensormap(&map_a);
+    if (MODE == kP2FuseF32 && threadIdx.x == kP2PatchWarp * 32) prefetch_tensormap(&map_a1);
     if (threadIdx.x == kP2WeightWarp * 32) prefetch_tensormap(&map_b);
     const int nchunks = p.cin / kP2Chunk;
     const int nitems = p2_item_count(p);
     const uint32_t b_plane_bytes = (uint32_t)p.n_tile * 64u;
 
     if (threadIdx.x == 0) {
-        for (int s = 0; s < 2; ++s) { mbar_init(&patch_full[s], 1); mbar_init(&patch_empty[s], kP2MmaWarps); }
+        for (int s = 0; s < (MODE == kP2FuseF32 ? kP2FuseGroups : 2); ++s) {
+            mbar_init(&patch_full[s], 1);
+            mbar_init(&patch_empty[s], MODE == kP2FuseF32 ? kP2MmaWarps / 2 : kP2MmaWarps);
+        }
         for (int s = 0; s < p.bstages; ++s) { mbar_init(&b_full[s], 1); mbar_init(&b_empty[s], kP2MmaWarps); }
         asm volatile("fence.mbarrier_init.release.cluster;\n" ::: "memory");
     }
@@ -183,13 +220,16 @@
             int pb = 0;
             uint32_t pph = 0;
             const uint32_t patches_u32 = smem_u32(patches);
+            constexpr bool kFuse = MODE == kP2FuseF32;
+            const int nloads = kFuse ? kP2FuseGroups : nchunks;
             for (int k = blockIdx.x; k < nitems; k += gridDim.x) {
                 const P2Item it = p2_decode(p, p2_item(p, k));
                 const int bu = it.u0 * p.in_stride, bv = it.v0 * p.in_stride;
-                for (int cc = 0; cc < nchunks; ++cc) {
-                    { const long long t0 = p2_tick<PROFILE>(); mbar_wait<REGA>(&patch_empty[pb], pph ^ 1u); p2_tock<PROFILE>(clk[kProfPatchEmpty], t0); }
+                for (int cc = 0; cc < nloads; ++cc) {
+                    const int bi = kFuse ? cc : pb;
+                    { const long long t0 = p2_tick<PROFILE>(); mbar_wait<REGA>(&patch_empty[bi], pph ^ 1u); p2_tock<PROFILE>(clk[kProfPatchEmpty], t0); }
                     if (elect_one()) {
-                        mbar_expect_tx(&patch_full[pb], (uint32_t)p.load_bytes);
+                        mbar_expect_tx(&patch_full[bi], (uint32_t)p.load_bytes);
                         if constexpr (MODE == kP2Planes) {
                             uint32_t dst = patches_u32 + (uint32_t)(pb * p.patch_bytes);
                             for (int c = 0; c < p.ncopies; ++c, dst += 2u * (uint32_t)p.copy_bytes) {
@@ -197,6 +237,11 @@
                                 tma_load_5d(dst, &map_a, &patch_full[pb], cc * kP2Chunk, cu, cv, it.b, 0);
                                 tma_load_5d(dst + (uint32_t)p.copy_bytes, &map_a, &patch_full[pb], cc * kP2Chunk, cu, cv, it.b, 1);
                             }
+                        } else if constexpr (kFuse) {
+                            const uint32_t dst = smem_u32(staging) + (uint32_t)(bi * p.load_bytes);
+                            const int gu = bu + p.copy_u[0], gv = bv + p.copy_v[0] + cc * (kP2FuseRows / kP2TileU);
+                            tma_load_5d(dst, &map_a, &patch_full[bi], 0, gu, gv, it.b, 0);
+                            tma_load_5d(dst + (uint32_t)(p.load_bytes / 2), &map_a1, &patch_full[bi], 0, gu, gv, it.b, 0);
                         } else {
                             const uint32_t copy_in = (uint32_t)(p.staging_bytes / p.ncopies);
                             uint32_t dst = smem_u32(staging) + (uint32_t)(pb * p.staging_bytes);
@@ -205,7 +250,7 @@
                         }
                     }
                     __syncwarp();
-                    if (++pb == p.npatch) { pb = 0; pph ^= 1u; }
+                    if ((!kFuse || cc == nloads - 1) && ++pb == p.npatch) { pb = 0; pph ^= 1u; }
                 }
             }
             if constexpr (PROFILE)
@@ -252,6 +297,13 @@
         float amax_in = 0.f, s_in = 1.f;
         if constexpr (MODE == kP2Planes) { amax_in = __ldg(p.in_info); s_in = __ldg(p.in_info + 1); }
         if constexpr (MODE == kP2SplitF16) if (p.in_amax) { amax_in = __ldg(p.in_amax); s_in = pow2_scale_for_bound(amax_in); }
+        float4 fw0 = {}, fw1 = {};
+        if constexpr (MODE == kP2FuseF32) {
+            amax_in = fmaxf(__ldg(p.in_info), __ldg(p.fuse_info1)); s_in = pow2_scale_for_bound(amax_in);
+            if (blockIdx.x == 0 && threadIdx.x == 0) { p.fuse_out_info[0] = amax_in; p.fuse_out_info[1] = s_in; }
+            fw0 = __ldg(reinterpret_cast<const float4 *>(p.fuse_w0) + lane);
+            fw1 = __ldg(reinterpret_cast<const float4 *>(p.fuse_w1) + lane);
+        }
         const float inv_sa = 1.f / s_in;
         float bound = amax_in * p.gain + p.shift_max;
         if (p.resid_info) bound += __ldg(p.resid_info);
@@ -326,10 +378,15 @@
                 if (nsteps & 1) step_ra(frag[0], frag[1], false);
             } else {
                 for (int cc = 0; cc < nchunks; ++cc) {
-                    { const long long t0 = p2_tick<PROFILE>(); mbar_wait(&patch_full[pb], pph); p2_tock<PROFILE>(clk[kProfPatchFull], t0); }
+                    constexpr bool kFuse = MODE == kP2FuseF32;
+                    if (!kFuse) {
+                        { const long long t0 = p2_tick<PROFILE>(); mbar_wait(&patch_full[pb], pph); p2_tock<PROFILE>(clk[kProfPatchFull], t0); }
+                    }
                     if constexpr (MODE == kP2SplitF16)
                         p2_split_patch(p, staging + pb * p.staging_bytes, patches + pb * p.patch_bytes, s_in, threadIdx.x);
-                    const uint32_t pbase = patch_lo + (uint32_t)pb * patch_sz;
+                    if constexpr (kFuse)
+                        if (cc == 0) p2_fuse_patch(p, staging, patches, patch_full, patch_empty, pph, s_in, fw0, fw1, wg, wq, lane);
+                    const uint32_t pbase = patch_lo + (uint32_t)pb * patch_sz + (kFuse ? (uint32_t)cc * 2u * copy_lo : 0u);
 #pragma unroll 1
                     for (int tap = 0; tap < ntaps; ++tap) {
                         { const long long t0 = p2_tick<PROFILE>(); mbar_wait(&b_full[S], bph); p2_tock<PROFILE>(clk[kProfBFull], t0); }
@@ -340,7 +397,7 @@
                             const uint64_t db_hi = db_lo + (uint64_t)plane_lo;
                             const uint32_t accum = first ? 0u : 1u;
                             wgmma_fence();
-                            if constexpr (MODE == kP2Planes) {
+                            if constexpr (MODE != kP2SplitF16) {
                                 p2_wgmma<2 * NT>(acc, da_hi, db_lo, accum);
                                 p2_wgmma<2 * NT>(acc, da_hi + 2, db_lo + 2, 1u);
                             } else {
@@ -361,10 +418,10 @@
                             if (prev_pb >= 0) mbar_arrive(&patch_empty[prev_pb]);
                         }
                         prevS = S;
-                        prev_pb = (tap == ntaps - 1) ? pb : -1;
+                        prev_pb = (!kFuse && tap == ntaps - 1) ? pb : -1;
                         if (++S == p.bstages) { S = 0; bph ^= 1u; }
                     }
-                    if (p.npatch == 1) {
+                    if (!kFuse && p.npatch == 1) {
                         { const long long t0 = p2_tick<PROFILE>(); wgmma_wait<0>(); p2_tock<PROFILE>(clk[kProfMmaWait], t0); }
                         if (lane == 0) {
                             mbar_arrive(&b_empty[prevS]);
@@ -372,7 +429,7 @@
                         }
                         prevS = prev_pb = -1;
                     }
-                    if (++pb == p.npatch) { pb = 0; pph ^= 1u; }
+                    if ((!kFuse || cc == nchunks - 1) && ++pb == p.npatch) { pb = 0; pph ^= 1u; }
                 }
             }
             { const long long t0 = p2_tick<PROFILE>(); wgmma_wait<0>(); p2_tock<PROFILE>(clk[kProfMmaWait], t0); }
@@ -538,6 +595,8 @@
 static int p2_plan(P2Params &p, const P2Taps *cls, int nclass, int grid_h, int grid_w, int cout_pad, int mode, bool reg_a, int *smem) {
     if (reg_a && (mode != kP2Planes || p.in_stride != 1)) return SESSD_EINVAL;
     if (p.cin < 64 || p.cin % 64) return SESSD_EINVAL;
+    if (mode == kP2FuseF32 && (reg_a || p.in_stride != 1 || p.cin != 128 || nclass != 1 || cls[0].n != 1 || p2_n_tile(p.cout) != 32))
+        return SESSD_EINVAL;
     P2Geometry g;
     if (p2_geometry(g, p.batch, grid_h, grid_w, p.cout, cout_pad, cls, nclass)) return SESSD_EINVAL;
     p.u_is_x = g.u_is_x; p.grid_u = g.grid_u; p.grid_v = g.grid_v;
@@ -592,9 +651,11 @@
         }
     }
     p.copy_bytes = (p.rows_v * p.pitch_u * 64 + 511) & ~511;
-    p.patch_bytes = p.ncopies * 2 * p.copy_bytes;
-    p.staging_bytes = mode == kP2Planes ? 0 : p.ncopies * p.rows_v * kP2TileU * kP2Chunk * 4;
-    p.load_bytes = mode == kP2Planes ? p.ncopies * 2 * p.rows_v * p.pitch_u * 64 : p.staging_bytes;
+    p.patch_bytes = (mode == kP2FuseF32 ? p.cin / kP2Chunk : 1) * p.ncopies * 2 * p.copy_bytes;
+    p.staging_bytes = mode == kP2Planes    ? 0
+                      : mode == kP2FuseF32 ? 2 * p.rows_v * kP2TileU * p.cin * 4
+                                           : p.ncopies * p.rows_v * kP2TileU * kP2Chunk * 4;
+    p.load_bytes = mode == kP2Planes ? p.ncopies * 2 * p.rows_v * p.pitch_u * 64 : mode == kP2FuseF32 ? p.staging_bytes / kP2FuseGroups : p.staging_bytes;
     const int per_buf = p.patch_bytes + p.staging_bytes, bstage = 2 * p.n_tile * 64;
     const int tail = 1536 + 16 + 2 * 4 * p.cout;
     p.npatch = (kP2BStages * bstage + tail + 2 * per_buf <= kP2MaxSmem) ? 2 : 1;
@@ -610,9 +671,10 @@
 static int launch_p2(const void *d_in_planes, int in_h, int in_w, const float *d_in_info, const void *d_w, int w_taps, int cout_pad,
                      const float *d_scale, const float *d_shift, const float *d_residual, const float *d_resid_info, float gain,
                      float shift_max, float *d_out_f32, void *d_out_planes, float *d_out_info, P2Params &p, const P2Taps *cls, int nclass,
-                     int grid_h, int grid_w, bool reg_a, void *stream) {
+                     int grid_h, int grid_w, bool reg_a, void *stream, const void *d_in1 = nullptr) {
     if (!d_in_planes || !d_w || (!d_out_f32 && !d_out_planes)) return SESSD_EINVAL;
-    if (MODE == kP2Planes && (!d_in_info || !d_scale)) return SESSD_EINVAL;
+    if (MODE != kP2SplitF16 && (!d_in_info || !d_scale)) return SESSD_EINVAL;
+    if (MODE == kP2FuseF32 && (!d_in1 || !p.fuse_w0 || !p.fuse_w1 || !p.fuse_info1 || !p.fuse_out_info)) return SESSD_EINVAL;
     if (MODE != kP2Planes && d_out_planes) return SESSD_EINVAL;
     if (((uintptr_t)d_scale | (uintptr_t)d_shift | (uintptr_t)d_residual | (uintptr_t)d_out_f32 | (uintptr_t)d_out_planes) & 15)
         return SESSD_EINVAL;
@@ -620,16 +682,19 @@
     if (p2_plan(p, cls, nclass, grid_h, grid_w, cout_pad, MODE, reg_a, &smem)) return SESSD_EINVAL;
     if (p.items && cout_pad != div_up(p.cout, p.n_tile) * p.n_tile) return SESSD_EINVAL;
     const int s = p.in_stride;
-    CUtensorMap map_a, map_b;
+    CUtensorMap map_a, map_a1, map_b;
     if (MODE != kP2Planes) {
         const cuuint64_t row_w = (cuuint64_t)p.cin * 4, row_h = (cuuint64_t)in_w * p.cin * 4;
         const cuuint64_t dims[5] = {(cuuint64_t)p.cin, (cuuint64_t)(p.u_is_x ? in_w : in_h), (cuuint64_t)(p.u_is_x ? in_h : in_w),
                                     (cuuint64_t)p.batch, 1};
         const cuuint64_t strides[4] = {p.u_is_x ? row_w : row_h, p.u_is_x ? row_h : row_w, (cuuint64_t)in_h * in_w * p.cin * 4,
                                        (cuuint64_t)p.batch * in_h * in_w * p.cin * 4};
-        const cuuint32_t box[5] = {(cuuint32_t)kP2Chunk, (cuuint32_t)(kP2TileU * s), (cuuint32_t)(p.rows_v * s), 1, 1};
+        const cuuint32_t box[5] = {(cuuint32_t)(MODE == kP2FuseF32 ? p.cin : kP2Chunk), (cuuint32_t)(kP2TileU * s),
+                                   (cuuint32_t)(MODE == kP2FuseF32 ? kP2FuseRows / kP2TileU : p.rows_v * s), 1, 1};
         const cuuint32_t estr[5] = {1, (cuuint32_t)s, (cuuint32_t)s, 1, 1};
         int rc = encode_map_nd(&map_a, d_in_planes, 5, dims, strides, box, estr, CU_TENSOR_MAP_SWIZZLE_NONE, CU_TENSOR_MAP_DATA_TYPE_FLOAT32);
+        if (!rc && MODE == kP2FuseF32)
+            rc = encode_map_nd(&map_a1, d_in1, 5, dims, strides, box, estr, CU_TENSOR_MAP_SWIZZLE_NONE, CU_TENSOR_MAP_DATA_TYPE_FLOAT32);
         if (rc) return rc;
     } else {
         const cuuint64_t row_w = (cuuint64_t)p.cin * 2, row_h = (cuuint64_t)in_w * p.cin * 2;
@@ -651,20 +716,22 @@
         if (rc) return rc;
     }
     constexpr bool kRegA = MODE == kP2Planes;
-    auto kernel = bev_conv_p2_kernel<128, MODE, false, PROBE>;
-    if (p.n_tile == 32) kernel = reg_a ? bev_conv_p2_kernel<32, MODE, kRegA, PROBE> : bev_conv_p2_kernel<32, MODE, false, PROBE>;
-    else if (reg_a) kernel = bev_conv_p2_kernel<128, MODE, kRegA, PROBE>;
+    auto kernel = bev_conv_p2_kernel<MODE == kP2FuseF32 ? 32 : 128, MODE, false, PROBE>;
+    if constexpr (MODE != kP2FuseF32) {
+        if (p.n_tile == 32) kernel = reg_a ? bev_conv_p2_kernel<32, MODE, kRegA, PROBE> : bev_conv_p2_kernel<32, MODE, false, PROBE>;
+        else if (reg_a) kernel = bev_conv_p2_kernel<128, MODE, kRegA, PROBE>;
+    }
     static bool attr_done[2][2] = {};
     if (!attr_done[p.n_tile == 32][reg_a]) {
         SESSD_CUDA_TRY(cudaFuncSetAttribute(kernel, cudaFuncAttributeMaxDynamicSharedMemorySize, kP2MaxSmem));
         attr_done[p.n_tile == 32][reg_a] = true;
     }
-    p.in_info = MODE == kP2Planes ? d_in_info : nullptr;
+    p.in_info = MODE != kP2SplitF16 ? d_in_info : nullptr;
     p.in_amax = MODE == kP2SplitF16 ? d_in_info : nullptr;
     p.resid_info = d_residual ? d_resid_info : nullptr;
     if (d_residual && d_out_planes && !d_resid_info) return SESSD_EINVAL;
     p.gain = gain; p.shift_max = shift_max; p.out_info = d_out_info;
-    p.out_info_scale = MODE == kP2Planes ? 1 : 0;
+    p.out_info_scale = MODE != kP2SplitF16 ? 1 : 0;
     if (d_out_planes && !d_out_info) return SESSD_EINVAL;
     p.out_plane_stride = (long long)p.batch * p.out_h * p.out_w * p.cout;
     static int num_sms = 0;
@@ -674,8 +741,9 @@
         SESSD_CUDA_TRY(cudaDeviceGetAttribute(&num_sms, cudaDevAttrMultiProcessorCount, dev));
     }
     const int grid = p.total < num_sms ? p.total : num_sms;
-    SESSD_LAUNCH(kernel, grid, reg_a ? kP2ThreadsRegA : kP2Threads, smem, (cudaStream_t)stream, map_a, map_b, d_scale, d_shift, d_residual, d_out_f32,
-                 (__half *)d_out_planes, p);
+    if (MODE != kP2FuseF32) map_a1 = map_a;
+    SESSD_LAUNCH(kernel, grid, reg_a ? kP2ThreadsRegA : kP2Threads, smem, (cudaStream_t)stream, map_a, map_a1, map_b, d_scale, d_shift, d_residual,
+                 d_out_f32, (__half *)d_out_planes, p);
     return last_error();
 }
 
diff --git a/se-ssd_b200/csrc/bevconv_split.cu b/se-ssd_b200/csrc/bevconv_split.cu
--- a/se-ssd_b200/csrc/bevconv_split.cu
+++ b/se-ssd_b200/csrc/bevconv_split.cu
@@ -53,7 +53,7 @@
     P2Taps cls[4];
     if (deconv) p2_deconv_params(d.batch, d.in_h, d.in_w, d.cin, d.cout, d.relu, p, cls);
     else if (p2_conv_params(d, p, cls[0])) return SESSD_EINVAL;
-    const int mode = split ? kP2SplitF16 : kP2Planes;
+    const int mode = split == 2 ? kP2FuseF32 : split ? kP2SplitF16 : kP2Planes;
     const bool reg_a = mode == kP2Planes && (deconv || (d.in_stride == 1 && !smem_a));
     int smem = 0;
     if (p2_plan(p, cls, deconv ? 4 : 1, deconv ? d.in_h : d.grid_h, deconv ? d.in_w : d.grid_w, cout_pad, mode, reg_a, &smem))
diff --git a/se-ssd_b200/csrc/ssfa_fuse.cuh b/se-ssd_b200/csrc/ssfa_fuse.cuh
--- /dev/null
+++ b/se-ssd_b200/csrc/ssfa_fuse.cuh
@@ -0,0 +1,44 @@
+#pragma once
+#include <cuda_fp16.h>
+
+namespace sessd {
+
+__device__ __forceinline__ float ssfa_dot4(float4 x, float4 w) {
+    float d = __fmul_rn(x.y, w.y);
+    d = __fmaf_rn(x.x, w.x, d);
+    d = __fmaf_rn(x.z, w.z, d);
+    return __fmaf_rn(x.w, w.w, d);
+}
+
+__device__ __forceinline__ float ssfa_warp_sum(float d) {
+#pragma unroll
+    for (int o = 16; o > 0; o >>= 1) d = __fadd_rn(d, __shfl_xor_sync(0xffffffffu, d, o));
+    return d;
+}
+
+__device__ __forceinline__ float2 ssfa_pair_weights(float d0, float d1, float s0, float t0, float s1, float t1) {
+    const float l0 = __fmaf_rn(d0, s0, t0), l1 = __fmaf_rn(d1, s1, t1);
+    const float mx = fmaxf(l0, l1);
+    const float e0 = expf(__fsub_rn(l0, mx)), e1 = expf(__fsub_rn(l1, mx));
+    const float inv = __frcp_rn(__fadd_rn(e0, e1));
+    return make_float2(__fmul_rn(e0, inv), __fmul_rn(e1, inv));
+}
+
+__device__ __forceinline__ float4 ssfa_mix4(float4 x0, float4 x1, float2 a) {
+    return make_float4(__fmaf_rn(x0.x, a.x, __fmul_rn(x1.x, a.y)), __fmaf_rn(x0.y, a.x, __fmul_rn(x1.y, a.y)),
+                       __fmaf_rn(x0.z, a.x, __fmul_rn(x1.z, a.y)), __fmaf_rn(x0.w, a.x, __fmul_rn(x1.w, a.y)));
+}
+
+__device__ __forceinline__ void ssfa_split4(float4 r, float s, uint2 &hi, uint2 &lo) {
+    const float q[4] = {__fmul_rn(r.x, s), __fmul_rn(r.y, s), __fmul_rn(r.z, s), __fmul_rn(r.w, s)};
+    __align__(8) __half h[4], l[4];
+#pragma unroll
+    for (int e = 0; e < 4; ++e) {
+        h[e] = __float2half_rn(q[e]);
+        l[e] = __float2half_rn(__fsub_rn(q[e], __half2float(h[e])));
+    }
+    hi = *reinterpret_cast<const uint2 *>(h);
+    lo = *reinterpret_cast<const uint2 *>(l);
+}
+
+}
diff --git a/se-ssd_b200/sessd_b200/_lib.py b/se-ssd_b200/sessd_b200/_lib.py
--- a/se-ssd_b200/sessd_b200/_lib.py
+++ b/se-ssd_b200/sessd_b200/_lib.py
@@ -79,6 +79,8 @@
     "sessd_sparse_to_dense_indexed": (_i, [_vp, _i, _vp, _i, Grid, _vp, _vp]),
     "sessd_sparse_to_dense": (_i, [_vp, _vp, _vp, _i, _i, Grid, _vp, _vp]),
     "sessd_bev_conv_p2": (_i, [_vp, _vp, _vp, _i, _vp, _vp, _vp, _vp, _f, _f, _vp, _vp, _vp, C.POINTER(ConvDesc), _vp, _vp]),
+    "sessd_bev_conv_p2_ssfa": (_i, [_vp, _vp, _vp, _vp, _vp, _vp, _f, _f, _f, _f, _vp, _vp, _i, _vp, _vp, _f, _f, _vp, _vp, C.POINTER(ConvDesc), _vp,
+                                    _vp]),
     "sessd_bev_deconv_p2": (_i, [_vp, _vp, _vp, _i, _vp, _vp, _vp, _vp, _f, _f, _vp, _vp, _vp, _i, _i, _i, _i, _i, _i, _vp, _vp]),
     "sessd_bev_skip_plan_words": (_ll, [_i, _i, _i, _I3]),
     "sessd_bev_skip_plan": (_i, [_vp, Grid, _vp, _vp]),
diff --git a/se-ssd_b200/sessd_b200/engine.py b/se-ssd_b200/sessd_b200/engine.py
--- a/se-ssd_b200/sessd_b200/engine.py
+++ b/se-ssd_b200/sessd_b200/engine.py
@@ -19,7 +19,8 @@
         self.d_off = torch.zeros((self.batch + 1,), dtype=torch.int32, device=dev)
         self.vox = ops.VoxelBuffers(self.vcfg, self.batch, self.max_points, dev, with_mean=True)
         self.middle = SpMiddleRunner(self.batch, self.batch * max_voxels, self.grid_xyz, 4, dev, growth=growth)
-        self.neck = SSFAPlanesRunner(self.batch, (self.grid_xyz[1] // 8, self.grid_xyz[0] // 8), dev, skip_constant=skip_constant)
+        self.neck = SSFAPlanesRunner(self.batch, (self.grid_xyz[1] // 8, self.grid_xyz[0] // 8), dev, skip_constant=skip_constant,
+                                     fused_head=True)
         self.anchors = None
         pk = dict(batch=self.batch, head_stride=SSFAPlanesRunner.HEAD_STRIDE)
         pk.update(post_kwargs or {})
diff --git a/se-ssd_b200/sessd_b200/ops.py b/se-ssd_b200/sessd_b200/ops.py
--- a/se-ssd_b200/sessd_b200/ops.py
+++ b/se-ssd_b200/sessd_b200/ops.py
@@ -324,6 +324,13 @@
     check(lib.sessd_bev_conv_p2(_p(in_planes), _p(in_info), _p(weight_h2), int(weight_h2.shape[2]), _p(scale), _p(shift), _p(residual),
                                 _p(resid_info), float(gain), float(shift_max), _p(out_f32), _p(out_planes), _p(out_info), C.byref(desc),
                                 _p(items), _st()), "sessd_bev_conv_p2")
+
+
+def bev_conv_p2_ssfa(x0, x1, info0, info1, w0, w1, s0, t0, s1, t1, fused_info, weight_h2, scale, shift, gain, shift_max, out_f32, out_info,
+                     desc, items=None):
+    check(lib.sessd_bev_conv_p2_ssfa(_p(x0), _p(x1), _p(info0), _p(info1), _p(w0), _p(w1), float(s0), float(t0), float(s1), float(t1),
+                                     _p(fused_info), _p(weight_h2), int(weight_h2.shape[2]), _p(scale), _p(shift), float(gain),
+                                     float(shift_max), _p(out_f32), _p(out_info), C.byref(desc), _p(items), _st()), "sessd_bev_conv_p2_ssfa")
 
 
 def bev_deconv_p2(in_planes, in_info, weight_h2, scale, shift, residual, resid_info, gain, shift_max, out_f32, out_planes, out_info, relu=True,
diff --git a/se-ssd_b200/sessd_b200/runners.py b/se-ssd_b200/sessd_b200/runners.py
--- a/se-ssd_b200/sessd_b200/runners.py
+++ b/se-ssd_b200/sessd_b200/runners.py
@@ -259,16 +259,20 @@
 class SSFAPlanesRunner:
 
     HEAD_STRIDE = 24
+    fused_head = False
     SLOT = SSFA_SLOT
     SKIP_LAUNCHES = tuple(L.name for L in SSFA_LAUNCHES)
 
-    def __init__(self, batch, hw=(200, 176), device="cuda", skip_constant=False):
+    def __init__(self, batch, hw=(200, 176), device="cuda", skip_constant=False, fused_head=False):
         self.batch, self.h, self.w, self.device = batch, int(hw[0]), int(hw[1]), torch.device(device)
         pl = lambda hw_, c: ops.alloc_bev_planes(batch, hw_[0], hw_[1], c, self.device)
         z = lambda hw_, c: torch.zeros((batch,) + hw_ + (c,), dtype=torch.float32, device=self.device)
         H, ext = (self.h, self.w), lambda L: ssfa_extents(L, self.h, self.w)[1]
-        self.planes = dict(x=pl(H, 128), **{L.dst: pl(ext(L), L.cout) for L in SSFA_LAUNCHES if not L.f32}, out=pl(H, 128))
-        self.buf = dict(**{L.dst: z(ext(L), L.cout) for L in SSFA_LAUNCHES[:-1] if L.f32}, out=z(H, 128), head=z(H, self.HEAD_STRIDE))
+        self.fused_head = bool(fused_head)
+        self.planes = dict(x=pl(H, 128), **{L.dst: pl(ext(L), L.cout) for L in SSFA_LAUNCHES if not L.f32})
+        self.buf = dict(**{L.dst: z(ext(L), L.cout) for L in SSFA_LAUNCHES[:-1] if L.f32}, head=z(H, self.HEAD_STRIDE))
+        if not self.fused_head:
+            self.planes["out"], self.buf["out"] = pl(H, 128), z(H, 128)
         self.info = torch.zeros((16, 2), dtype=torch.float32, device=self.device)
         self.params = None
         self.skip_constant = bool(skip_constant)
@@ -294,7 +298,12 @@
         resid, resid_info = (self.buf[L.residual], self._info(L.residual)) if L.residual else (None, None)
         i = self.SKIP_LAUNCHES.index(L.name)
         rec = self.skip.record(i) if skip else None
-        if L.kind == "conv":
+        if L.name == "head" and self.fused_head:
+            (w0, s0, t0), (w1, s1, t1) = self.params["w_0.0"], self.params["w_1.0"]
+            d = launch_desc(L, self.batch, *ssfa_extents(L, self.h, self.w), q["taps"])
+            ops.bev_conv_p2_ssfa(self.buf["o0"], self.buf["o1"], self._info("o0"), self._info("o1"), w0, w1, s0, t0, s1, t1, self._info(L.src),
+                                 q["w"], q["scale"], q["shift"], q["gain"], q["shift_max"], out_f32, self._info(L.dst), d, items=rec)
+        elif L.kind == "conv":
             d = launch_desc(L, self.batch, *ssfa_extents(L, self.h, self.w), q["taps"])
             ops.bev_conv_p2(self.planes[L.src], self._info(L.src), q["w"], q["scale"], q["shift"], resid, resid_info, q["gain"],
                             q["shift_max"], out_f32, out_planes, self._info(L.dst), d, items=rec)
@@ -318,6 +327,10 @@
         for L in SSFA_LAUNCHES[:-1]:
             self._launch(L, skip)
             mark("neck:" + L.name)
+        if self.fused_head:
+            self.head(skip=skip)
+            mark("neck:fuse+head")
+            return None, self.buf["head"]
         w0, s0, t0 = self.params["w_0.0"]
         w1, s1, t1 = self.params["w_1.0"]
         ops.ssfa_fuse_planes(self.buf["o0"], self.buf["o1"], w0, w1, s0, t0, s1, t1, self.buf["out"], self._info("o0"), self._info("o1"),
```

After: 1593 (median of 6 runs). 1.03x the previous value.
